# ComputationalRobotics/cuADMM

Measured on NVIDIA B200. Metric: ADMM iterations/s, higher is better.
Workload: dtype f64

## Files before the change

cuadmm_b200/csrc/common.cpp:

```cpp
#include "common.h"
#include <mutex>

namespace cuadmm {
static thread_local std::string g_last_error;
void set_last_error(const std::string& msg) { g_last_error = msg; }
}

extern "C" {
const char* cuadmm_last_error(void) { return cuadmm::g_last_error.c_str(); }
const char* cuadmm_version(void) { return "cuadmm_b200 0.1 (sm_100a)"; }
int cuadmm_device_count(void) {
    int n = 0;
    if (cudaGetDeviceCount(&n) != cudaSuccess) { cudaGetLastError(); return 0; }
    return n;
}
}
```

cuadmm_b200/csrc/common.h:

```cpp
#pragma once
#include <cuda_runtime.h>
#include <stdint.h>
#include <stdio.h>
#include <string>
#include <vector>
#include <memory>
#include <stdexcept>
#include "../../include/cuadmm_b200.h"

namespace cuadmm {

void set_last_error(const std::string& msg);

struct Error : public std::runtime_error {
    int code;
    Error(int c, const std::string& m) : std::runtime_error(m), code(c) {}
};

#define CUADMM_CUDA(call)                                                                   \
    do {                                                                                    \
        cudaError_t e__ = (call);                                                           \
        if (e__ != cudaSuccess) {                                                           \
            char buf__[512];                                                                \
            snprintf(buf__, sizeof buf__, "CUDA error %s at %s:%d: %s", cudaGetErrorName(e__), \
                     __FILE__, __LINE__, cudaGetErrorString(e__));                          \
            throw ::cuadmm::Error(e__ == cudaErrorMemoryAllocation ? CUADMM_ENOMEM :        \
                                  (e__ == cudaErrorNoDevice || e__ == cudaErrorInsufficientDriver) ? CUADMM_ENODEVICE : CUADMM_ECUDA, buf__); \
        }                                                                                   \
    } while (0)

#define CUADMM_REQUIRE(cond, msg)                                                           \
    do { if (!(cond)) throw ::cuadmm::Error(CUADMM_EINVAL, std::string("invalid argument: ") + (msg)); } while (0)

template <class F>
static inline int guarded(F&& f) {
    try { f(); return CUADMM_OK; }
    catch (const Error& e) { set_last_error(e.what()); return e.code; }
    catch (const std::bad_alloc&) { set_last_error("host out of memory"); return CUADMM_ENOMEM; }
    catch (const std::exception& e) { set_last_error(e.what()); return CUADMM_EINVAL; }
}

template <class T>
struct DevBuf {
    T* p = nullptr;
    int64_t n = 0;
    bool owned = true;
    DevBuf() {}
    explicit DevBuf(int64_t n_) { alloc(n_); }
    DevBuf(const DevBuf&) = delete;
    DevBuf& operator=(const DevBuf&) = delete;
    DevBuf(DevBuf&& o) noexcept : p(o.p), n(o.n), owned(o.owned) { o.p = nullptr; o.n = 0; }
    DevBuf& operator=(DevBuf&& o) noexcept { if (this != &o) { release(); p = o.p; n = o.n; owned = o.owned; o.p = nullptr; o.n = 0; } return *this; }
    ~DevBuf() { release(); }
    void release() { if (p && owned) cudaFree(p); p = nullptr; n = 0; owned = true; }
    void adopt(T* ptr, int64_t n_) { release(); p = ptr; n = n_; owned = false; }
    void alloc(int64_t n_) {
        release();
        n = n_;
        if (n_ > 0) CUADMM_CUDA(cudaMalloc((void**)&p, sizeof(T) * (size_t)n_));
    }
    void zero(cudaStream_t s = 0) { if (n) CUADMM_CUDA(cudaMemsetAsync(p, 0, sizeof(T) * (size_t)n, s)); }
    void upload(const T* h, int64_t cnt, cudaStream_t s = 0) {
        if (cnt) CUADMM_CUDA(cudaMemcpyAsync(p, h, sizeof(T) * (size_t)cnt, cudaMemcpyHostToDevice, s));
    }
    void upload(const std::vector<T>& h, cudaStream_t s = 0) {
        if ((int64_t)h.size() != n) alloc((int64_t)h.size());
        upload(h.data(), n, s);
    }
    void download(T* h, int64_t cnt, cudaStream_t s = 0) const {
        if (cnt) CUADMM_CUDA(cudaMemcpyAsync(h, p, sizeof(T) * (size_t)cnt, cudaMemcpyDeviceToHost, s));
    }
};

struct DeviceGuard {
    int prev = -1;
    explicit DeviceGuard(int dev) {
        if (dev >= 0) { cudaGetDevice(&prev); CUADMM_CUDA(cudaSetDevice(dev)); }
    }
    ~DeviceGuard() { if (prev >= 0) cudaSetDevice(prev); }
};

static inline int64_t tri(int64_t n) { return n * (n + 1) / 2; }

}
```

cuadmm_b200/csrc/debug_api.cpp:

```cpp
#include "chol_host.h"
#include "common.h"
#include <algorithm>
#include <cmath>

using namespace cuadmm;

extern "C" {

int cuadmm_debug_chol_solve(int64_t m, int64_t ncols, const int32_t* rowptr, const int32_t* colind, const double* val,
                            double eps, double n_lead_frac, const double* rhs, double* y, int32_t* perm_out,
                            int64_t* stats ) {
    return guarded([&] {
        SymCsc M = form_aat(m, ncols, rowptr, colind, val, eps);
        std::vector<int32_t> perm = min_degree_order(M);
        perm = postorder_perm(M, perm);
        CholFactor F; SymCsc C;
        chol_symbolic(M, perm, F, &C);
        const int64_t n_lead = std::max<int64_t>(0, std::min<int64_t>(m, (int64_t)(n_lead_frac * (double)m)));
        chol_numeric(C, F, n_lead);
        const int64_t r = m - n_lead;
        std::vector<double> S((size_t)(r * r), 0.0);
        for (int64_t j = n_lead; j < m; ++j)
            for (int64_t p = C.p[j]; p < C.p[j + 1]; ++p) S[(C.i[p] - n_lead) + (j - n_lead) * r] = C.x[p];
        for (int64_t j = 0; j < n_lead; ++j)
            for (int64_t p = F.Lp[j] + 1; p < F.Lp[j + 1]; ++p) if (F.Li[p] >= n_lead)
                for (int64_t q = p; q < F.Lp[j + 1]; ++q)
                    S[(F.Li[q] - n_lead) + (F.Li[p] - n_lead) * r] -= F.Lx[q] * F.Lx[p];
        for (int64_t k = 0; k < r; ++k) {
            double d = S[k + k * r];
            d = (d > 1e-11) ? std::sqrt(d) : INFINITY; S[k + k * r] = d;
            for (int64_t i = k + 1; i < r; ++i) S[i + k * r] /= d;
            for (int64_t j = k + 1; j < r; ++j)
                for (int64_t i = j; i < r; ++i) S[i + j * r] -= S[i + k * r] * S[j + k * r];
        }
        std::vector<double> z(m);
        for (int64_t k = 0; k < m; ++k) z[k] = rhs[F.perm[k]];
        for (int64_t j = 0; j < n_lead; ++j) {
            z[j] /= F.Lx[F.Lp[j]];
            for (int64_t p = F.Lp[j] + 1; p < F.Lp[j + 1]; ++p) z[F.Li[p]] -= F.Lx[p] * z[j];
        }
        for (int64_t j = 0; j < r; ++j) {
            z[n_lead + j] /= S[j + j * r];
            for (int64_t i = j + 1; i < r; ++i) z[n_lead + i] -= S[i + j * r] * z[n_lead + j];
        }
        for (int64_t j = r - 1; j >= 0; --j) {
            for (int64_t i = j + 1; i < r; ++i) z[n_lead + j] -= S[i + j * r] * z[n_lead + i];
            z[n_lead + j] /= S[j + j * r];
        }
        for (int64_t j = n_lead - 1; j >= 0; --j) {
            for (int64_t p = F.Lp[j] + 1; p < F.Lp[j + 1]; ++p) z[j] -= F.Lx[p] * z[F.Li[p]];
            z[j] /= F.Lx[F.Lp[j]];
        }
        for (int64_t k = 0; k < m; ++k) y[F.perm[k]] = z[k];
        if (perm_out) std::copy(F.perm.begin(), F.perm.end(), perm_out);
        if (stats) {
            stats[0] = M.p[m]; stats[1] = F.nnz(); stats[2] = F.n_deficient;
            std::vector<int32_t> lev(m, 0);
            int32_t depth = 0;
            for (int64_t j = 0; j < m; ++j) {
                for (int64_t p = F.Lp[j] + 1; p < F.Lp[j + 1]; ++p) lev[F.Li[p]] = std::max(lev[F.Li[p]], lev[j] + 1);
                depth = std::max(depth, lev[j] + 1);
            }
            stats[3] = depth;
            std::vector<int64_t> cnt(depth + 1, 0);
            for (int64_t j = 0; j < m; ++j) cnt[lev[j]]++;
            int64_t narrow = 0;
            for (int32_t l = 0; l < depth; ++l) if (cnt[l] < 8) narrow += cnt[l];
            stats[4] = narrow;
            std::vector<int64_t> sn = find_supernodes(F, 256);
            const int64_t nsn = (int64_t)sn.size() - 1;
            std::vector<int32_t> snof(m, 0), slev(std::max<int64_t>(nsn, 1), 0);
            for (int64_t s = 0; s < nsn; ++s) for (int64_t j = sn[s]; j < sn[s + 1]; ++j) snof[j] = (int32_t)s;
            int32_t sdepth = 0;
            for (int64_t s = 0; s < nsn; ++s) {
                for (int64_t j = sn[s]; j < sn[s + 1]; ++j)
                    for (int64_t p = F.Lp[j] + 1; p < F.Lp[j + 1]; ++p) {
                        const int32_t t = snof[F.Li[p]];
                        if (t != s) slev[t] = std::max(slev[t], slev[s] + 1);
                    }
                sdepth = std::max(sdepth, slev[s] + 1);
            }
            stats[5] = nsn; stats[6] = sdepth;
            std::vector<int64_t> scnt(sdepth + 1, 0);
            for (int64_t s = 0; s < nsn; ++s) scnt[slev[s]] += sn[s + 1] - sn[s];
            int64_t deep_rows = 0;
            for (int32_t l = 48; l < sdepth; ++l) deep_rows += scnt[l];
            stats[7] = deep_rows;
        }
    });
}

}
```

cuadmm_b200/csrc/plan.h:

```cpp
#pragma once
#include "common.h"
#include "blocks.h"
#include "project_jacobi.cuh"

namespace cuadmm { struct DensePart; }
cuadmm::DensePart* dense_part_create(int device, const std::vector<int32_t>& blk, const std::vector<int64_t>& svec_off,
                                     const std::vector<int64_t>& which);
void dense_part_destroy(cuadmm::DensePart* p);
int dense_part_project(cuadmm::DensePart* D, const double* Xb, double* Xproj, cudaStream_t st,
                       const cuadmm::ProjEpilogue* epi, const int* done_flag);

namespace cuadmm {
struct LinChunk {
    int64_t off;
    int32_t len;
    int32_t cone;
};
constexpr int kLinearChunk = 4096;
std::vector<LinChunk> linear_chunks(const BlockLayout& layout);
int linear_project(const LinChunk* d_chunks, int64_t nchunks, const double* Xb, double* Xproj, cudaStream_t st,
                   const ProjEpilogue* epi, const int* done_flag);
}

struct cuadmm_plan {
    int device = -1;
    cuadmm::BlockLayout layout;

    struct Class {
        int kind;
        int nmax;
        int32_t count;
        int64_t first;
        size_t smem;
        int grid;
    };
    std::vector<Class> classes;
    std::vector<cuadmm::BlkDesc> h_desc;
    cuadmm::DevBuf<cuadmm::BlkDesc> d_desc;
    cuadmm::DevBuf<double> d_scratch;
    cuadmm::DevBuf<double> d_eig;
    cuadmm::DevBuf<int32_t> d_sweeps;
    cuadmm::DevBuf<double> d_in, d_out;
    cuadmm::DevBuf<int64_t> d_svec_off, d_mat_off;
    cuadmm::DevBuf<int32_t> d_blk;
    cuadmm::DevBuf<uint8_t> d_pool;

    cuadmm::DevBuf<double> d_Q;
    bool warm_start = true;
    void reset_warm_start();
    double threshold = 1e-11;
    int max_sweeps = 40;
    bool force_global = false;
    std::unique_ptr<cuadmm_plan> eig_plan;
    int rank_limit = 0;
    cudaEvent_t ev0 = nullptr, ev1 = nullptr;
    std::vector<cudaStream_t> side_streams;
    std::vector<cudaEvent_t> side_events;
    cudaEvent_t fork_event = nullptr;
    cuadmm::DensePart* dense = nullptr;
    std::vector<cuadmm::LinChunk> h_lin;
    cuadmm::DevBuf<cuadmm::LinChunk> d_lin;
    cudaStream_t lin_stream = nullptr;
    cudaEvent_t lin_event = nullptr;
    int64_t eig_len = 0;
    const int* done_flag = nullptr;
    double last_ms = 0.0;
    int64_t last_launches = 0;

    ~cuadmm_plan();
    void build_device();
    int project(const double* d_Xb, double* d_Xproj, cudaStream_t stream,
                const cuadmm::ProjEpilogue* epi, bool want_eig);
};
```

cuadmm_b200/csrc/project.cu:

```cuda
#include "plan.h"
#include <algorithm>
#include <limits>
#include <type_traits>
#include <numeric>
#include <stdlib.h>

namespace cuadmm {

template <bool WARP>
__device__ __forceinline__ void mat_sync() {
    if (WARP) __syncwarp(); else __syncthreads();
}

template <int NT, bool WARP>
__device__ __forceinline__ double mat_sum(double v, double* red, int tid) {
#pragma unroll
    for (int o = 16; o > 0; o >>= 1) v += __shfl_xor_sync(0xffffffffu, v, o);
    if (WARP) return v;
    const int wid = tid >> 5;
    __syncthreads();
    if ((tid & 31) == 0) red[wid] = v;
    __syncthreads();
    double t = 0.0;
#pragma unroll 1
    for (int i = 0; i < NT / 32; ++i) t += red[i];
    return t;
}

template <int NT, bool WARP>
__device__ __forceinline__ double mat_max(double v, double* red, int tid) {
#pragma unroll
    for (int o = 16; o > 0; o >>= 1) v = fmax(v, __shfl_xor_sync(0xffffffffu, v, o));
    if (WARP) return v;
    const int wid = tid >> 5;
    __syncthreads();
    if ((tid & 31) == 0) red[wid] = v;
    __syncthreads();
    double t = 0.0;
#pragma unroll 1
    for (int i = 0; i < NT / 32; ++i) t = fmax(t, red[i]);
    return t;
}

__host__ __device__ __forceinline__ int jacobi_ld(int n, int L) {
    if (L >= 16) return n | 1;
    int ld = n;
    while ((ld & 15) != (L & 15)) ++ld;
    return ld;
}
__host__ __device__ __forceinline__ size_t jacobi_per_mat(int nmax, int L) {
    return (((size_t)jacobi_ld(nmax, L) * nmax + nmax + (nmax + 2) / 2 + 1 + 34) + 1) & ~(size_t)1;
}

__device__ __forceinline__ void jacobi_cs2(double alpha, double beta, double gamma, double& c, double& s,
                                           double& alpha_new, double& beta_new) {
    const double d = beta - alpha;
    const double g2 = gamma + gamma;
    const double rh = rsqrt(fma(d, d, g2 * g2));
    const double c2 = fabs(d) * rh;
    const double s2 = (d < 0.0 ? -g2 : g2) * rh;
    const double cc = fma(0.5, c2, 0.5);
    const double rc = rsqrt(cc);
    c = cc * rc;
    s = 0.5 * s2 * rc;
    const double ss = 1.0 - cc;
    const double x = s2 * gamma;
    alpha_new = fma(cc, alpha, fma(ss, beta, -x));
    beta_new = fma(ss, alpha, fma(cc, beta, x));
}

__device__ __forceinline__ void jacobi_dmma(double& c0, double& c1, double a, double b) {
    asm volatile("mma.sync.aligned.m8n8k4.row.col.f64.f64.f64.f64 {%0,%1}, {%2}, {%3}, {%0,%1};"
                 : "+d"(c0), "+d"(c1) : "d"(a), "d"(b));
}

template <int NT, bool WARP>
__device__ __forceinline__ bool jacobi_gram_converged(const double* G, const double* w, int n, int ld, double thr2, int tid) {
    const int lane = tid & 31;
    const int wid = WARP ? 0 : (tid >> 5);
    constexpr int NW = WARP ? 1 : NT / 32;
    const int nt = (n + 7) >> 3;
    const int kr = lane & 3, cq = lane >> 2;
    int flag = 0;
    for (int P = wid; P < nt; P += NW) {
        const int pcol = P * 8 + cq;
        const double* Gp = G + (size_t)min(pcol, n - 1) * ld;
        const bool pv = pcol < n;
        const int row = P * 8 + cq;
        const double wr = (row < n) ? w[row] : 0.0;
        for (int Q0 = P; Q0 < nt; Q0 += 4) {
            double c[4][2];
            const double* Gq[4];
            bool qv[4];
#pragma unroll
            for (int u = 0; u < 4; ++u) {
                const int qcol = (Q0 + u) * 8 + cq;
                qv[u] = (Q0 + u < nt) && qcol < n;
                Gq[u] = G + (size_t)min(qcol, n - 1) * ld;
                c[u][0] = 0.0; c[u][1] = 0.0;
            }
            for (int r0 = 0; r0 < n; r0 += 4) {
                const int r = r0 + kr;
                const bool rv = r < n;
                const double av = (pv && rv) ? Gp[r] : 0.0;
                double bv[4];
#pragma unroll
                for (int u = 0; u < 4; ++u) bv[u] = (qv[u] && rv) ? Gq[u][r] : 0.0;
#pragma unroll
                for (int u = 0; u < 4; ++u) jacobi_dmma(c[u][0], c[u][1], av, bv[u]);
            }
            if (row < n) {
#pragma unroll
                for (int u = 0; u < 4; ++u) {
                    const int col0 = (Q0 + u) * 8 + 2 * kr;
                    if (Q0 + u < nt) {
                        if (col0 < n && col0 != row) { const double g2 = c[u][0] * c[u][0]; if (g2 > thr2 * wr * w[col0] && g2 > 1e-30) flag = 1; }
                        if (col0 + 1 < n && col0 + 1 != row) { const double g2 = c[u][1] * c[u][1]; if (g2 > thr2 * wr * w[col0 + 1] && g2 > 1e-30) flag = 1; }
                    }
                }
            }
        }
    }
    const int any = WARP ? __any_sync(0xffffffffu, flag) : __syncthreads_or(flag);
    return !any;
}

constexpr int jacobi_min_ctas(int T) { return T <= 64 ? 8 : T <= 128 ? 4 : T <= 256 ? 2 : 1; }

template <int T, int L, int RPL, bool WARP>
__global__ void __launch_bounds__(T, jacobi_min_ctas(T)) proj_jacobi_kernel(ProjArgs a, int nmax) {
    extern __shared__ double smem[];
    constexpr int NT = WARP ? 32 : T;
    constexpr int NG = NT / L;
    constexpr int MPC = WARP ? T / 32 : 1;
    const int tid = WARP ? (threadIdx.x & 31) : threadIdx.x;
    const int mat_in_cta = WARP ? (threadIdx.x >> 5) : 0;
    const int bi = blockIdx.x * MPC + mat_in_cta;
    if (bi >= a.nblk) return;
    if (a.done_flag && *a.done_flag) return;

    const size_t per_mat = jacobi_per_mat(nmax, L);
    double* G = smem + per_mat * mat_in_cta;
    double* w = G + (size_t)jacobi_ld(nmax, L) * nmax;
    int* pos = (int*)(w + nmax);
    double* red = w + nmax + (nmax + 2) / 2 + 1;

    const BlkDesc d = a.desc[bi];
    const int n = d.n;
    const int ld = jacobi_ld(n, L);
    const int ntri = n * (n + 1) / 2;
    const double* __restrict__ xin = a.Xb + d.svec_off;
    double* __restrict__ xout = a.Xproj + d.svec_off;

    double amax = 0.0;
    for (int idx0 = tid; idx0 < ntri; idx0 += NT * 8) {
        double v[8];
#pragma unroll
        for (int u = 0; u < 8; ++u) { const int idx = idx0 + u * NT; v[u] = (idx < ntri) ? __ldg(xin + idx) : 0.0; }
#pragma unroll
        for (int u = 0; u < 8; ++u) {
            const int idx = idx0 + u * NT;
            if (idx < ntri) {
                int r, c;
                tri_unrank(idx, r, c);
                amax = fmax(amax, fabs(v[u]));
                const double v2 = (r == c) ? v[u] : v[u] * CUADMM_SQRT2INV;
                G[r + c * ld] = v2;
                G[c + r * ld] = v2;
            }
        }
    }
    amax = mat_max<NT, WARP>(amax, red, tid);
    int ex = 0;
    if (amax > 0.0 && amax < 1.7e308) frexp(amax, &ex);
    mat_sync<WARP>();
    double f2 = 0.0;
    const int e_dc = NT / n, e_dr = NT - e_dc * n;
    const int e_c0 = tid / n, e_r0 = tid - e_c0 * n;
    for (int c = e_c0, r = e_r0; c < n;) {
        const double v = ldexp(G[r + c * ld], -ex);
        G[r + c * ld] = v;
        f2 = fma(v, v, f2);
        r += e_dr; c += e_dc;
        if (r >= n) { r -= n; ++c; }
    }
    f2 = mat_sum<NT, WARP>(f2, red, tid);
    const double sp = sqrt(f2);
    if (!(sp > 0.0) || !(sp < 1.7e308)) {
        const double fill = (sp == 0.0) ? 0.0 : (sp - sp);
        for (int idx = tid; idx < ntri; idx += NT) {
            xout[idx] = fill;
            if (a.epi.X) {
                const int64_t gi = d.svec_off + idx;
                const double sig = *a.epi.sig_ptr;
                const double Sv = (fill - a.epi.X[gi]) / sig - a.epi.Rd1[gi];
                a.epi.S[gi] = Sv;
                a.epi.SmC[gi] = Sv - a.epi.Cd[gi];
            }
        }
        if (tid == 0 && a.sweeps_out) a.sweeps_out[d.index] = 0;
        if (a.eig_out) for (int j = tid; j < n; j += NT) a.eig_out[d.w_off + j] = fill;
        return;
    }
    const double inv_s = 1.0 / sp;
    for (int c = e_c0, r = e_r0; c < n;) {
        const double v = G[r + c * ld] * inv_s;
        G[r + c * ld] = (r == c) ? v + 1.0 : v;
        r += e_dr; c += e_dc;
        if (r >= n) { r -= n; ++c; }
    }
    mat_sync<WARP>();

    const int m = n + (n & 1);
    const int half = m >> 1;
    const int grp = tid / L, lane = tid % L;
    const unsigned gmask = (L == 32) ? 0xffffffffu : (((1u << L) - 1u) << ((tid & 31) / L * L));

    double* Qb = a.Q ? a.Q + d.q_off : nullptr;
    if (Qb) {
        constexpr int KF = (((L * RPL) > 168 ? 168 : (L * RPL)) + 3) / 4;
        constexpr int NWARP = WARP ? 1 : NT / 32;
        const int wid = WARP ? 0 : (tid >> 5);
        const int l32 = tid & 31;
        const int fr = l32 >> 2, fk = l32 & 3;
        const int nk = (n + 3) >> 2;
        for (int r0 = wid * 8; r0 < n; r0 += NWARP * 8) {
            const int row = r0 + fr;
            double af[KF];
#pragma unroll
            for (int kk = 0; kk < KF; ++kk) {
                const int k = kk * 4 + fk;
                af[kk] = (kk < nk && row < n && k < n) ? G[row + k * ld] : 0.0;
            }
            __syncwarp();
            for (int j0 = 0; j0 < n; j0 += 16) {
                constexpr int KC = KF < 16 ? KF : 16;
                const int col0 = j0 + fr, col1 = j0 + 8 + fr;
                const double* __restrict__ q0 = Qb + (size_t)min(col0, n - 1) * n;
                const double* __restrict__ q1 = Qb + (size_t)min(col1, n - 1) * n;
                double c00 = 0.0, c01 = 0.0, c10 = 0.0, c11 = 0.0;
#pragma unroll
                for (int kb = 0; kb < KF; kb += KC) {
                    if (kb < nk) {
                        double b0[KC], b1[KC];
#pragma unroll
                        for (int kk = 0; kk < KC; ++kk) {
                            const int k = (kb + kk) * 4 + fk;
                            const bool kv = kb + kk < nk && k < n;
                            b0[kk] = (kv && col0 < n) ? __ldg(q0 + k) : 0.0;
                            b1[kk] = (kv && col1 < n) ? __ldg(q1 + k) : 0.0;
                        }
#pragma unroll
                        for (int kk = 0; kk < KC; ++kk) {
                            if (kb + kk < KF && kb + kk < nk) {
                                jacobi_dmma(c00, c01, af[kb + kk], b0[kk]);
                                jacobi_dmma(c10, c11, af[kb + kk], b1[kk]);
                            }
                        }
                    }
                }
                if (row < n) {
                    const int cc = j0 + 2 * fk;
                    if (cc < n) G[row + cc * ld] = c00;
                    if (cc + 1 < n) G[row + (cc + 1) * ld] = c01;
                    if (cc + 8 < n) G[row + (cc + 8) * ld] = c10;
                    if (cc + 9 < n) G[row + (cc + 9) * ld] = c11;
                }
            }
        }
        mat_sync<WARP>();
    }

    const double thr2 = a.threshold * a.threshold;
    const double tiny2 = 1.2325951644078309e-32;
    int sweeps = 0;
    bool converged = false;
    while (true) {
        for (int j = grp; j < n; j += NG) {
            const double* Gj = G + j * ld;
            double al = 0.0;
            for (int r = lane; r < n; r += L) al = fma(Gj[r], Gj[r], al);
#pragma unroll
            for (int o = L / 2; o > 0; o >>= 1) al += __shfl_xor_sync(gmask, al, o);
            if (lane == 0) w[j] = al;
        }
        mat_sync<WARP>();
        if (jacobi_gram_converged<NT, WARP>(G, w, n, ld, thr2, tid)) { converged = true; break; }
        if (sweeps >= a.max_sweeps) break;
        auto run_steps = [&](auto nit_c) {
            constexpr int NIT = decltype(nit_c)::value;
// ... 303 lines not shown
    int nmax;
    int threads;
    int L;
    int mats_per_cta;
    void (*fn)(ProjArgs, int);
};

#define CUADMM_CLASS(NMAX, T, L, RPL, WARP) {NMAX, T, L, (WARP) ? (T) / 32 : 1, proj_jacobi_kernel<T, L, RPL, WARP>}
static const SizeClass kSizeClasses[] = {
    CUADMM_CLASS(16, 128, 4, 4, true),
    CUADMM_CLASS(32, 64, 4, 8, false),
    CUADMM_CLASS(64, 128, 4, 16, false),
    CUADMM_CLASS(96, 192, 4, 24, false),
    CUADMM_CLASS(128, 512, 8, 16, false),
    CUADMM_CLASS(168, 352, 8, 21, false),
};
static const int kNumSizeClasses = (int)(sizeof(kSizeClasses) / sizeof(kSizeClasses[0]));
static const int kGlobalKind = -1;

static size_t smem_bytes(int nmax, const SizeClass& sc) {
    return jacobi_per_mat(nmax, sc.L) * sizeof(double) * sc.mats_per_cta;
}

}

using namespace cuadmm;

cuadmm_plan::~cuadmm_plan() {
    if (device >= 0) {
        cudaSetDevice(device);
        if (ev0) cudaEventDestroy(ev0);
        if (ev1) cudaEventDestroy(ev1);
        if (fork_event) cudaEventDestroy(fork_event);
        if (lin_stream) cudaStreamDestroy(lin_stream);
        if (lin_event) cudaEventDestroy(lin_event);
        for (auto s : side_streams) cudaStreamDestroy(s);
        for (auto e : side_events) cudaEventDestroy(e);
        if (dense) dense_part_destroy(dense);
    }
}

void cuadmm_plan::build_device() {
    const int64_t nblk = (int64_t)layout.blk.size();
    std::vector<int64_t> w_off(nblk + 1, 0);
    for (int64_t k = 0; k < nblk; ++k) w_off[k + 1] = w_off[k] + (layout.types[k] == 's' ? layout.blk[k] : 0);
    eig_len = w_off[nblk];
    h_lin = linear_chunks(layout);

    std::vector<std::vector<int64_t>> members(kNumSizeClasses + 1);
    std::vector<int64_t> dense_blocks;
    for (int64_t k = 0; k < nblk; ++k) {
        if (layout.types[k] != 's') continue;
        const int n = layout.blk[k];
        int ci = kNumSizeClasses;
        for (int c = 0; c < kNumSizeClasses; ++c) if (n <= kSizeClasses[c].nmax) { ci = c; break; }
        if (ci == kNumSizeClasses && !force_global) { dense_blocks.push_back(k); continue; }
        members[ci].push_back(k);
    }
    if (dense) { dense_part_destroy(dense); dense = nullptr; }
    if (!dense_blocks.empty()) dense = dense_part_create(device, layout.blk, layout.svec_off, dense_blocks);
    h_desc.clear(); classes.clear();
    int64_t scratch = 0, q_total = 0;
    for (int ci = kNumSizeClasses; ci >= 0; --ci) {
        auto& mem = members[ci];
        if (mem.empty()) continue;
        std::stable_sort(mem.begin(), mem.end(), [&](int64_t a, int64_t b) { return layout.blk[a] > layout.blk[b]; });
        Class cl;
        cl.kind = (ci == kNumSizeClasses) ? kGlobalKind : ci;
        cl.nmax = layout.blk[mem[0]];
        cl.count = (int32_t)mem.size();
        cl.first = (int64_t)h_desc.size();
        if (cl.kind == kGlobalKind) {
            cl.smem = 0;
            cl.grid = cl.count;
        } else {
            const SizeClass& sc = kSizeClasses[cl.kind];
            cl.smem = smem_bytes(cl.nmax, sc);
            cl.grid = (cl.count + sc.mats_per_cta - 1) / sc.mats_per_cta;
        }
        for (int64_t k : mem) {
            BlkDesc d;
            d.svec_off = layout.svec_off[k];
            d.w_off = w_off[k];
            d.n = layout.blk[k];
            d.index = (int32_t)k;
            d.scratch_off = 0;
            d.q_off = 0;
            if (cl.kind != kGlobalKind) { d.q_off = q_total; q_total += (int64_t)d.n * d.n; }
            else { d.scratch_off = scratch; scratch += (int64_t)d.n * d.n; }
            h_desc.push_back(d);
        }
        classes.push_back(cl);
    }
    if (device < 0) return;

    DeviceGuard g(device);
    d_desc.upload(h_desc);
    if (!h_lin.empty()) {
        d_lin.upload(h_lin);
        CUADMM_CUDA(cudaStreamCreateWithFlags(&lin_stream, cudaStreamNonBlocking));
        CUADMM_CUDA(cudaEventCreateWithFlags(&lin_event, cudaEventDisableTiming));
    }
    if (scratch) d_scratch.alloc(scratch);
    d_eig.alloc(std::max<int64_t>(w_off[nblk], 1));
    d_sweeps.alloc(std::max<int64_t>(nblk, 1));
    warm_start = true;
    if (const char* e = getenv("CUADMM_JACOBI_WARM")) warm_start = atoi(e) != 0;
    if (const char* e = getenv("CUADMM_JACOBI_THR")) { const double v = atof(e); if (v > 0.0 && v < 1e-3) threshold = v; }
    if (warm_start && q_total > 0) {
        d_Q.alloc(q_total);
        reset_warm_start();
    }
    d_svec_off.upload(layout.svec_off);
    d_mat_off.upload(layout.mat_off);
    d_blk.upload(layout.blk);
    d_pool.upload(layout.pool);
    CUADMM_CUDA(cudaEventCreate(&ev0));
    CUADMM_CUDA(cudaEventCreate(&ev1));
    CUADMM_CUDA(cudaEventCreateWithFlags(&fork_event, cudaEventDisableTiming));
    for (size_t i = 0; i < classes.size(); ++i) {
        cudaStream_t s; cudaEvent_t e;
        CUADMM_CUDA(cudaStreamCreateWithFlags(&s, cudaStreamNonBlocking));
        CUADMM_CUDA(cudaEventCreateWithFlags(&e, cudaEventDisableTiming));
        side_streams.push_back(s); side_events.push_back(e);
    }
    for (const Class& cl : classes) {
        if (cl.kind == kGlobalKind) continue;
        const SizeClass& sc = kSizeClasses[cl.kind];
        CUADMM_CUDA(cudaFuncSetAttribute((const void*)sc.fn, cudaFuncAttributeMaxDynamicSharedMemorySize, (int)smem_bytes(sc.nmax, sc)));
    }
    CUADMM_CUDA(cudaDeviceSynchronize());
}

__global__ void init_basis_kernel(const BlkDesc* __restrict__ desc, int nblk, double* Q) {
    const int b = blockIdx.x;
    if (b >= nblk) return;
    const int n = desc[b].n;
    double* q = Q + desc[b].q_off;
    for (int e = threadIdx.x; e < n * n; e += blockDim.x) q[e] = (e / n == e % n) ? 1.0 : 0.0;
}

void cuadmm_plan::reset_warm_start() {
    if (d_Q.n == 0) return;
    DeviceGuard g(device);
    for (const Class& cl : classes) {
        if (cl.kind == kGlobalKind) continue;
        init_basis_kernel<<<cl.count, 256>>>(d_desc.p + cl.first, cl.count, d_Q.p);
    }
    CUADMM_CUDA(cudaGetLastError());
    CUADMM_CUDA(cudaDeviceSynchronize());
}

int cuadmm_plan::project(const double* d_Xb, double* d_Xproj, cudaStream_t stream,
                         const ProjEpilogue* epi, bool want_eig) {
    if (device < 0) throw Error(CUADMM_ENODEVICE, "plan was built without a CUDA device; there is no CPU fallback");
    int launches = 0;
    if (want_eig) {
        CUADMM_CUDA(cudaMemsetAsync(d_eig.p, 0xFF, sizeof(double) * (size_t)d_eig.n, stream));
        CUADMM_CUDA(cudaMemsetAsync(d_sweeps.p, 0, sizeof(int32_t) * (size_t)d_sweeps.n, stream));
    }
    const bool has_dense = dense != nullptr;
    const bool has_lin = !h_lin.empty();
    const bool lin_side = has_lin && (has_dense || !classes.empty());
    if (rank_limit > 0) {
        if (has_dense) throw Error(CUADMM_EINVAL, "fixed-rank projection is only available for blocks n <= 168 (the sign iteration of larger blocks has no eigenvalues to rank)");
    }
    if (classes.size() > 1 || (has_dense && !classes.empty()) || lin_side) CUADMM_CUDA(cudaEventRecord(fork_event, stream));
    for (size_t i = 0; i < classes.size(); ++i) {
        const Class& cl = classes[i];
        cudaStream_t st = stream;
        const bool side = has_dense || i > 0;
        if (side) {
            st = side_streams[i];
            CUADMM_CUDA(cudaStreamWaitEvent(st, fork_event, 0));
        }
        ProjArgs a;
        a.Xb = d_Xb; a.Xproj = d_Xproj;
        a.desc = d_desc.p + cl.first;
        a.nblk = cl.count;
        a.threshold = threshold;
        a.max_sweeps = max_sweeps;
        a.eig_out = want_eig ? d_eig.p : nullptr;
        a.sweeps_out = want_eig ? d_sweeps.p : nullptr;
        a.scratch = d_scratch.p;
        a.done_flag = done_flag;
        a.rank_limit = rank_limit;
        a.Q = (warm_start && cl.kind != kGlobalKind && d_Q.n > 0) ? d_Q.p : nullptr;
        if (epi) a.epi = *epi; else { a.epi.X = nullptr; a.epi.Rd1 = nullptr; a.epi.Cd = nullptr; a.epi.S = nullptr; a.epi.SmC = nullptr; a.epi.sig_ptr = nullptr; }
        if (cl.kind == kGlobalKind) {
            proj_jacobi_global_kernel<<<cl.grid, 1024, 0, st>>>(a);
        } else {
            kSizeClasses[cl.kind].fn<<<cl.grid, kSizeClasses[cl.kind].threads, cl.smem, st>>>(a, cl.nmax);
        }
        CUADMM_CUDA(cudaGetLastError());
        ++launches;
        if (side) CUADMM_CUDA(cudaEventRecord(side_events[i], st));
    }
    if (has_lin) {
        cudaStream_t st = stream;
        if (lin_side) {
            st = lin_stream;
            CUADMM_CUDA(cudaStreamWaitEvent(st, fork_event, 0));
        }
        launches += linear_project(d_lin.p, d_lin.n, d_Xb, d_Xproj, st, epi, done_flag);
        if (lin_side) CUADMM_CUDA(cudaEventRecord(lin_event, st));
    }
    if (has_dense) launches += dense_part_project(dense, d_Xb, d_Xproj, stream, epi, done_flag);
    for (size_t i = 0; i < classes.size(); ++i)
        if (has_dense || i > 0) CUADMM_CUDA(cudaStreamWaitEvent(stream, side_events[i], 0));
    if (lin_side) CUADMM_CUDA(cudaStreamWaitEvent(stream, lin_event, 0));
    return launches;
}

extern "C" {

int cuadmm_plan_create(const int32_t* blk, int64_t nblk, int device, cuadmm_plan** out) {
    return cuadmm_plan_create_typed(nullptr, blk, nblk, device, out);
}

int cuadmm_plan_create_typed(const char* types, const int32_t* blk, int64_t nblk, int device, cuadmm_plan** out) {
    return guarded([&] {
        CUADMM_REQUIRE(out != nullptr, "out is null");
        CUADMM_REQUIRE(blk != nullptr || nblk == 0, "blk is null");
        *out = nullptr;
        std::unique_ptr<cuadmm_plan> p(new cuadmm_plan());
        p->layout.init(blk, nblk, types);
        if (device >= 0) {
            int cnt = 0;
            cudaError_t e = cudaGetDeviceCount(&cnt);
            if (e != cudaSuccess || cnt == 0) {
                cudaGetLastError();
                throw Error(CUADMM_ENODEVICE, "no CUDA device available (pass device=-1 for a host-only plan; compute has no CPU fallback)");
            }
            CUADMM_REQUIRE(device < cnt, "device index out of range");
        }
        p->device = device;
        p->build_device();
        *out = p.release();
    });
}

void cuadmm_plan_destroy(cuadmm_plan* plan) { delete plan; }
int64_t cuadmm_plan_vec_len(const cuadmm_plan* plan) { return plan ? plan->layout.vec_len : -1; }
int64_t cuadmm_plan_nblk(const cuadmm_plan* plan) { return plan ? (int64_t)plan->layout.blk.size() : -1; }
int64_t cuadmm_plan_num_sizes(const cuadmm_plan* plan) { return plan ? (int64_t)plan->layout.sizes.size() : -1; }

int cuadmm_plan_sizes(const cuadmm_plan* plan, int32_t* sizes, int32_t* nums, int32_t* is_large) {
    return guarded([&] {
        CUADMM_REQUIRE(plan, "plan is null");
        plan->layout.require_all_psd("cuadmm_plan_sizes");
        for (size_t i = 0; i < plan->layout.sizes.size(); ++i) {
            if (sizes) sizes[i] = plan->layout.sizes[i];
            if (nums) nums[i] = plan->layout.nums[i];
            if (is_large) is_large[i] = plan->layout.large[i];
        }
    });
}

int cuadmm_plan_totals(const cuadmm_plan* plan, int64_t out[6]) {
    return guarded([&] {
        CUADMM_REQUIRE(plan && out, "null argument");
        const BlockLayout& l = plan->layout;
        l.require_all_psd("cuadmm_plan_totals");
        out[0] = l.large_mat_num; out[1] = l.sum_large_mat_size; out[2] = l.total_large_mat_size;
        out[3] = l.small_mat_num; out[4] = l.sum_small_mat_size; out[5] = l.total_small_mat_size;
    });
}

int64_t cuadmm_plan_start_indices(const cuadmm_plan* plan, int which, int64_t* out) {
    if (!plan) return -1;
    const BlockLayout& l = plan->layout;
    if (!l.all_psd()) return guarded([&] { l.require_all_psd("cuadmm_plan_start_indices"); });
    const std::vector<int64_t>* v = nullptr;
    switch (which) {
        case 0: v = &l.large_mat_start; break;
        case 1: v = &l.large_W_start; break;
        case 2: v = &l.small_mat_start; break;
        case 3: v = &l.small_W_start; break;
        default: return -1;
    }
    if (out) std::copy(v->begin(), v->end(), out);
    return (int64_t)v->size();
}

int cuadmm_plan_maps(const cuadmm_plan* plan, int32_t* map_B, int32_t* map_M1, int32_t* map_M2) {
    return guarded([&] {
        CUADMM_REQUIRE(plan && map_B && map_M1 && map_M2, "null argument");
        plan->layout.maps(map_B, map_M1, map_M2);
    });
}

int cuadmm_plan_partition(const cuadmm_plan* plan, int nparts, int32_t* owner, double* part_cost) {
    return guarded([&] {
        CUADMM_REQUIRE(plan && owner, "null argument");
        plan->layout.partition(nparts, owner, part_cost);
    });
}

int cuadmm_plan_set_rank_limit(cuadmm_plan* plan, int eig_rank) {
    return guarded([&] {
        CUADMM_REQUIRE(plan, "plan is null");
        CUADMM_REQUIRE(eig_rank >= 0, "eig_rank < 0");
        plan->rank_limit = eig_rank;
    });
}

int cuadmm_eig_rank_mask(int32_t* mask, int64_t batch_size, int64_t mat_size, int64_t eig_rank) {
    return guarded([&] {
        CUADMM_REQUIRE(mask || batch_size * mat_size == 0, "mask is null");
        CUADMM_REQUIRE(batch_size >= 0 && mat_size >= 0 && eig_rank >= 0 && eig_rank <= mat_size, "bad sizes");
        for (int64_t i = 0; i < batch_size * mat_size; ++i) mask[i] = 0;
        for (int64_t i = 0; i < batch_size; ++i)
            for (int64_t j = 0; j < eig_rank; ++j) mask[i * mat_size + (mat_size - 1 - j)] = 1;
    });
}

int cuadmm_plan_set_warm_start(cuadmm_plan* plan, int enable) {
    return guarded([&] {
        CUADMM_REQUIRE(plan, "plan is null");
        if (plan->device < 0) return;
        plan->reset_warm_start();
        plan->warm_start = enable != 0 && plan->d_Q.n > 0;
    });
}

int cuadmm_plan_set_jacobi(cuadmm_plan* plan, double threshold, int max_sweeps) {
    return guarded([&] {
        CUADMM_REQUIRE(plan, "plan is null");
        CUADMM_REQUIRE(threshold > 0 && max_sweeps > 0, "threshold and max_sweeps must be positive");
        plan->threshold = threshold;
        plan->max_sweeps = max_sweeps;
    });
}

double cuadmm_plan_last_ms(const cuadmm_plan* plan) { return plan ? plan->last_ms : -1.0; }
int64_t cuadmm_plan_last_launches(const cuadmm_plan* plan) { return plan ? plan->last_launches : -1; }

int cuadmm_project_psd(cuadmm_plan* plan, const double* d_Xb, double* d_Xproj, void* stream) {
    return guarded([&] {
        CUADMM_REQUIRE(plan && d_Xb && d_Xproj, "null argument");
        DeviceGuard g(plan->device);
        plan->last_launches = plan->project(d_Xb, d_Xproj, (cudaStream_t)stream, nullptr, false);
    });
}

int cuadmm_project_epilogue(cuadmm_plan* plan, const double* d_Xb, double* d_Xproj, const double* d_X, const double* d_Rd1,
                            const double* d_C, double* d_S, double* d_SmC, const double* d_sig, void* stream) {
    return guarded([&] {
        CUADMM_REQUIRE(plan && d_Xb && d_Xproj && d_X && d_Rd1 && d_C && d_S && d_SmC && d_sig, "null argument");
        DeviceGuard g(plan->device);
        ProjEpilogue pe;
        pe.X = d_X; pe.Rd1 = d_Rd1; pe.Cd = d_C; pe.S = d_S; pe.SmC = d_SmC; pe.sig_ptr = d_sig;
        plan->last_launches = plan->project(d_Xb, d_Xproj, (cudaStream_t)stream, &pe, false);
    });
}

static void project_host_impl(cuadmm_plan* plan, const double* h_Xb, double* h_Xproj,
                              double* h_eig, int32_t* h_sweeps) {
    CUADMM_REQUIRE(plan && h_Xb && h_Xproj, "null argument");
    if (plan->device < 0) throw Error(CUADMM_ENODEVICE, "plan was built without a CUDA device; there is no CPU fallback");
    DeviceGuard g(plan->device);
    const int64_t L = plan->layout.vec_len;
    if (plan->d_in.n != L) { plan->d_in.alloc(L); plan->d_out.alloc(L); }
// ... 105 lines not shown
```

cuadmm_b200/csrc/solver.cu:

```cuda
#include "solver.h"
#include <algorithm>
#include <chrono>
#include <cmath>
#include <string>
#include <string.h>
#include <stdlib.h>

namespace cuadmm {

void spmv_set_done_flag(cuadmm_spmv_s& A, const int* flag);

static constexpr int kEwThreads = 256;
static constexpr int64_t kHistRing = 4096;

__global__ void __launch_bounds__(kEwThreads) x_update_kernel(int64_t n, const double* __restrict__ Rd1,
        const double* __restrict__ S, const double* __restrict__ Cd, double* Rd, double* X,
        const DevState* st, double* partial) {
    if (st->done) return;
    __shared__ double red[2][kEwThreads / 32];
    const double ts = st->tau * st->sig;
    double a0 = 0.0, a1 = 0.0;
    for (int64_t i = (int64_t)blockIdx.x * kEwThreads + threadIdx.x; i < n; i += (int64_t)gridDim.x * kEwThreads) {
        const double rd = Rd1[i] + S[i];
        Rd[i] = rd;
        const double xn = X[i] + ts * rd;
        X[i] = xn;
        a0 = fma(rd, rd, a0);
        a1 = fma(Cd[i], xn, a1);
    }
#pragma unroll
    for (int o = 16; o > 0; o >>= 1) { a0 += __shfl_xor_sync(0xffffffffu, a0, o); a1 += __shfl_xor_sync(0xffffffffu, a1, o); }
    if ((threadIdx.x & 31) == 0) { red[0][threadIdx.x >> 5] = a0; red[1][threadIdx.x >> 5] = a1; }
    __syncthreads();
    if (threadIdx.x == 0) {
        double s0 = 0.0, s1 = 0.0;
        for (int k = 0; k < kEwThreads / 32; ++k) { s0 += red[0][k]; s1 += red[1][k]; }
        partial[2 * blockIdx.x] = s0; partial[2 * blockIdx.x + 1] = s1;
    }
}

__global__ void __launch_bounds__(256) scalar_update_kernel(DevState* st, const double* __restrict__ part_rd, int n_rd,
        const double* __restrict__ part_rp, int n_rp, double* hist, int64_t hist_cap) {
    if (st->done) return;
    __shared__ double sm[4][256];
    double v[4] = {0.0, 0.0, 0.0, 0.0};
    for (int i = threadIdx.x; i < n_rd; i += 256) { v[0] += part_rd[2 * i]; v[1] += part_rd[2 * i + 1]; }
    for (int i = threadIdx.x; i < n_rp; i += 256) { v[2] += part_rp[2 * i]; v[3] += part_rp[2 * i + 1]; }
    for (int q = 0; q < 4; ++q) sm[q][threadIdx.x] = v[q];
    __syncthreads();
    for (int o = 128; o > 0; o >>= 1) {
        if (threadIdx.x < o) for (int q = 0; q < 4; ++q) sm[q][threadIdx.x] += sm[q][threadIdx.x + o];
        __syncthreads();
    }
    if (threadIdx.x != 0) return;
    const double sumRd = sm[0][0], sumCX = sm[1][0], sumRp = sm[2][0], sumby = sm[3][0];
    const int iter = st->iter;
    const double errRp = st->bscale * sqrt(sumRp) / st->norm_borg;
    const double pobj = sumCX * st->objscale;
    const double errRd = st->Cscale * sqrt(sumRd) / st->norm_Corg;
    const double dobj = sumby * st->objscale;
    const double maxfeas = fmax(errRp, errRd);
    const double relgap = fabs(pobj - dobj) / (1 + fabs(pobj) + fabs(dobj));
    const double feasratio = st->ratioconst * errRp / errRd;
    if (feasratio < 1) st->prim_win += 1; else st->dual_win += 1;
    double sig = st->sig;
    if (((iter <= st->sig_update_threshold) && ((iter % st->sig_update_stage_1) == 1)) ||
        ((iter > st->sig_update_threshold) && ((iter % st->sig_update_stage_2) == 1))) {
        if (st->prim_win > 1.2 * st->dual_win) {
            st->prim_win = 0;
            sig = fmin(st->sigmax, sig * st->sigscale);
        } else if (st->dual_win > 1.2 * st->prim_win) {
            st->dual_win = 0;
            sig = fmax(st->sigmin, sig / st->sigscale);
        }
    }
    st->sig = sig;
    st->errRp = errRp; st->errRd = errRd; st->pobj = pobj; st->dobj = dobj;
    st->maxfeas = maxfeas; st->relgap = relgap; st->feasratio = feasratio;
    {
        const int64_t k = (int64_t)(iter - 1) % hist_cap;
        hist[0 * hist_cap + k] = pobj;  hist[1 * hist_cap + k] = dobj;
        hist[2 * hist_cap + k] = errRp; hist[3 * hist_cap + k] = errRd;
        hist[4 * hist_cap + k] = relgap; hist[5 * hist_cap + k] = sig;
        hist[6 * hist_cap + k] = st->bscale; hist[7 * hist_cap + k] = st->Cscale;
    }
    const int next = iter + 1;
    st->iter = next;
    double tau = (next < st->switch_admm) ? 1.95 : 1.618;
    if (errRd < st->stop_tol) tau = fmax(1.618, tau / 1.1);
    st->tau = tau;
    if (fmax(maxfeas, relgap) < st->stop_tol) { st->done = 1; st->stop_reason = 1; }
    if (next > st->max_iter) { st->done = 1; st->stop_reason = 2; }
}

__global__ void switch_kernel(DevState* st) {
    if (st->done) return;
    st->sig_update_stage_2 = st->sig_update_stage_2 / 2;
    st->sigscale = st->sigscale * 1.23;
    st->sgs_KKT = fmax(st->maxfeas, st->relgap);
    st->best_KKT = st->sgs_KKT;
}

__global__ void best_decide_kernel(DevState* st) {
    if (st->done) { st->pad_ = 0; return; }
    const double cur = fmax(st->maxfeas, st->relgap);
    if (st->best_KKT > cur) { st->best_KKT = cur; st->pad_ = 1; } else st->pad_ = 0;
}
__global__ void best_copy_kernel(const DevState* st, int64_t n, const double* __restrict__ src, double* dst) {
    if (!st->pad_) return;
    for (int64_t i = (int64_t)blockIdx.x * blockDim.x + threadIdx.x; i < n; i += (int64_t)gridDim.x * blockDim.x) dst[i] = src[i];
}

__global__ void scale_kernel(int64_t n, double* x, double s) {
    for (int64_t i = (int64_t)blockIdx.x * blockDim.x + threadIdx.x; i < n; i += (int64_t)gridDim.x * blockDim.x) x[i] *= s;
}
__global__ void scale_vec_kernel(int64_t n, double* y, const double* __restrict__ d, double s, int divide) {
    for (int64_t i = (int64_t)blockIdx.x * blockDim.x + threadIdx.x; i < n; i += (int64_t)gridDim.x * blockDim.x)
        y[i] = divide ? y[i] / d[i] * s : y[i] * d[i] * s;
}
__global__ void sub_kernel(int64_t n, const double* __restrict__ a, const double* __restrict__ b, double* out) {
    for (int64_t i = (int64_t)blockIdx.x * blockDim.x + threadIdx.x; i < n; i += (int64_t)gridDim.x * blockDim.x) out[i] = a[i] - b[i];
}

__global__ void rhsy_kernel(int64_t m, const double* __restrict__ Rp, const double* __restrict__ buf, double* rhsy, const DevState* st) {
    if (st->done) return;
    const double sig = st->sig;
    for (int64_t i = (int64_t)blockIdx.x * blockDim.x + threadIdx.x; i < m; i += (int64_t)gridDim.x * blockDim.x) rhsy[i] = Rp[i] / sig + buf[i];
}
__global__ void __launch_bounds__(256) fold_partials_kernel(const double* __restrict__ part, int n, double* out2, const DevState* st) {
    if (st->done) return;
    __shared__ double sm[2][256];
    double a = 0.0, b = 0.0;
    for (int i = threadIdx.x; i < n; i += 256) { a += part[2 * i]; b += part[2 * i + 1]; }
    sm[0][threadIdx.x] = a; sm[1][threadIdx.x] = b;
    __syncthreads();
    for (int o = 128; o > 0; o >>= 1) {
        if (threadIdx.x < o) { sm[0][threadIdx.x] += sm[0][threadIdx.x + o]; sm[1][threadIdx.x] += sm[1][threadIdx.x + o]; }
        __syncthreads();
    }
    if (threadIdx.x == 0) { out2[0] = sm[0][0]; out2[1] = sm[1][0]; }
}
__global__ void __launch_bounds__(kEwThreads) rp_kernel(int64_t m, const double* __restrict__ b, const double* __restrict__ buf,
        const double* __restrict__ normA, const double* __restrict__ y, double* Rp, const DevState* st, double* partial) {
    if (st->done) return;
    __shared__ double red[2][kEwThreads / 32];
    double a0 = 0.0, a1 = 0.0;
    for (int64_t i = (int64_t)blockIdx.x * kEwThreads + threadIdx.x; i < m; i += (int64_t)gridDim.x * kEwThreads) {
        const double rp = b[i] - buf[i];
        Rp[i] = rp;
        const double t = normA[i] * rp;
        a0 = fma(t, t, a0);
        a1 = fma(b[i], y[i], a1);
    }
#pragma unroll
    for (int o = 16; o > 0; o >>= 1) { a0 += __shfl_xor_sync(0xffffffffu, a0, o); a1 += __shfl_xor_sync(0xffffffffu, a1, o); }
    if ((threadIdx.x & 31) == 0) { red[0][threadIdx.x >> 5] = a0; red[1][threadIdx.x >> 5] = a1; }
    __syncthreads();
    if (threadIdx.x == 0) {
        double s0 = 0.0, s1 = 0.0;
        for (int k = 0; k < kEwThreads / 32; ++k) { s0 += red[0][k]; s1 += red[1][k]; }
        partial[2 * blockIdx.x] = s0; partial[2 * blockIdx.x + 1] = s1;
    }
}
__global__ void scatter_full_kernel(int64_t nloc, const double* __restrict__ local, const int64_t* __restrict__ loc2glob, double* full) {
    for (int64_t i = (int64_t)blockIdx.x * blockDim.x + threadIdx.x; i < nloc; i += (int64_t)gridDim.x * blockDim.x) full[loc2glob[i]] = local[i];
}

static int ew_grid(int64_t n, int device) {
    int sms = 148;
    cudaDeviceGetAttribute(&sms, cudaDevAttrMultiProcessorCount, device);
    return (int)std::max<int64_t>(1, std::min<int64_t>((n + kEwThreads - 1) / kEwThreads, (int64_t)sms * 8));
}

static double host_norm2(const std::vector<double>& v) {
    double scale = 0.0, ssq = 1.0;
    for (double x : v) {
        if (x != 0.0) {
            const double a = std::fabs(x);
            if (scale < a) { ssq = 1.0 + ssq * (scale / a) * (scale / a); scale = a; }
            else ssq += (a / scale) * (a / scale);
        }
    }
    return scale * std::sqrt(ssq);
}

}

using namespace cuadmm;

cuadmm_solver::~cuadmm_solver() {
    cudaSetDevice(device);
    delete A; delete At; delete ys;
    if (h_st) cudaFreeHost(h_st);
    if (ev_start) cudaEventDestroy(ev_start);
    if (ev_now) cudaEventDestroy(ev_now);
    for (auto e : prof_ev) cudaEventDestroy(e);
    if (graph_sgs) cudaGraphExecDestroy(graph_sgs);
    if (graph_admm) cudaGraphExecDestroy(graph_admm);
    if (stream) cudaStreamDestroy(stream);
}

void cuadmm_solver::init(int , int , int64_t vec_len_, int64_t con_num_,
                         const int32_t* At_col_ptrs, const int32_t* At_row_ids, const double* At_vals, int64_t At_nnz,
                         const int32_t* b_idx, const double* b_val, int64_t b_nnz,
                         const int32_t* C_idx, const double* C_val, int64_t C_nnz,
                         const int32_t* blk, int64_t mat_num, const double* X0, const double* y0, const double* S0, double sig) {
    CUADMM_REQUIRE(!initialised, "solver already initialised (one instance per problem, like SDPSolver)");
    CUADMM_REQUIRE(vec_len_ >= 0 && con_num_ >= 0 && At_nnz >= 0, "negative dimension");
    CUADMM_REQUIRE(At_col_ptrs && blk, "null argument");
    CUADMM_REQUIRE(At_col_ptrs[0] == 0 && At_col_ptrs[con_num_] == At_nnz, "At_csc_col_ptrs does not span At_nnz");
    int cnt = 0;
    if (cudaGetDeviceCount(&cnt) != cudaSuccess || cnt == 0) {
        cudaGetLastError();
        throw Error(CUADMM_ENODEVICE, "no CUDA device available; the solver has no CPU fallback");
    }
    if (!device_set) {
        if (const char* e = getenv("CUADMM_DEVICE")) device = atoi(e);
        else { int cur = 0; if (cudaGetDevice(&cur) == cudaSuccess) device = cur; else cudaGetLastError(); }
    }
    if (const char* e = getenv("CUADMM_NO_GRAPH")) use_graphs = atoi(e) == 0;
    CUADMM_REQUIRE(device >= 0 && device < cnt, "device index out of range");
    CUADMM_CUDA(cudaSetDevice(device));
    vec_len = vec_len_; con_num = con_num_;
    CUADMM_CUDA(cudaStreamCreateWithFlags(&stream, cudaStreamNonBlocking));
    CUADMM_CUDA(cudaEventCreate(&ev_start));
    CUADMM_CUDA(cudaEventCreate(&ev_now));
    CUADMM_CUDA(cudaEventRecord(ev_start, stream));
    const auto t0 = std::chrono::steady_clock::now();

    {
        CUADMM_REQUIRE(blk_types.empty() || (int64_t)blk_types.size() == mat_num, "block types were set for a different block count");
        BlockLayout full_layout;
        full_layout.init(blk, mat_num, blk_types.empty() ? nullptr : blk_types.data());
        CUADMM_REQUIRE(full_layout.vec_len == vec_len, "vec_len does not match the block sizes");
        shard.build(full_layout, world, rank);
        nloc = shard.vec_len_local;
        plan.reset(new cuadmm_plan());
        plan->layout.init(shard.local_blk.data(), (int64_t)shard.local_blk.size(), shard.local_types.data());
        plan->device = device;
        plan->build_device();
        if (world > 1) {
            d_loc2glob.upload(shard.loc2glob);
            if (const char* c = getenv("CUADMM_COMM")) use_peer = strcmp(c, "nccl") != 0;
        }
    }
    std::vector<double> vals(At_vals, At_vals + At_nnz);
    h_normA.assign(con_num, 1.0);
    for (int64_t p = 0; p < At_nnz; ++p) CUADMM_REQUIRE(At_row_ids[p] >= 0 && At_row_ids[p] < vec_len, "At row index out of range");
    for (int64_t i = 0; i < con_num; ++i) {
        double norm = 0.0;
        for (int p = At_col_ptrs[i]; p < At_col_ptrs[i + 1]; ++p) norm += vals[p] * vals[p];
        norm = std::max(1.0, std::sqrt(norm));
        h_normA[i] = norm;
        for (int p = At_col_ptrs[i]; p < At_col_ptrs[i + 1]; ++p) vals[p] /= norm;
    }
    {
        std::vector<int32_t> l_cp, l_ri; std::vector<double> l_v;
        const int32_t* cp = At_col_ptrs; const int32_t* ri = At_row_ids; const double* vv = vals.data();
        int64_t l_nnz = At_nnz;
        if (world > 1) {
            shard.slice_csc(con_num, At_col_ptrs, At_row_ids, vals.data(), l_cp, l_ri, l_v);
            l_ri.push_back(0); l_v.push_back(0.0);
            cp = l_cp.data(); ri = l_ri.data(); vv = l_v.data(); l_nnz = l_cp[con_num];
        }
        A = spmv_create(con_num, nloc, l_nnz, cp, ri, vv, device);
        std::vector<int32_t> t_rp(nloc + 1), t_ci(std::max<int64_t>(l_nnz, 1));
        std::vector<double> t_v(std::max<int64_t>(l_nnz, 1));
        if (cuadmm_csc_to_csr_host(nloc, con_num, l_nnz, cp, ri, vv, t_rp.data(), t_ci.data(), t_v.data()) != 0)
            throw Error(CUADMM_EINVAL, cuadmm_last_error());
        At = spmv_create(nloc, con_num, l_nnz, t_rp.data(), t_ci.data(), t_v.data(), device);
    }
    ys = ysolve_create(con_num, vec_len, At_nnz, At_col_ptrs, At_row_ids, vals.data(), 1e-15, device);
    if (world > 1) {
        if (use_peer) {
            CUADMM_REQUIRE(con_num < (int64_t)0xffffffffll, "sharded solver: con_num exceeds 32 bits");
            slice = (((con_num + world - 1) / world) + 1) & ~(int64_t)1;
            const int64_t mm = std::max<int64_t>(con_num, 1);
            const size_t need = sizeof(double) * (size_t)(world * slice + 4 * mm + std::max<int64_t>(ys->n_tail, 1) + std::max<int64_t>(vec_len, 1)) + 16 * 256;
            peer.reset(new PeerComm());
            peer->init(rank, world, nccl_id, device, need);
            const size_t o_stage = peer->alloc(sizeof(double) * world * slice);
            const size_t o_asmc = peer->alloc(sizeof(double) * mm), o_Rp = peer->alloc(sizeof(double) * mm), o_y = peer->alloc(sizeof(double) * mm);
            const size_t o_x = peer->alloc(sizeof(double) * mm), o_tmp = peer->alloc(sizeof(double) * std::max<int64_t>(ys->n_tail, 1));
            const size_t o_full = peer->alloc(sizeof(double) * std::max<int64_t>(vec_len, 1));
            stage = peer->local<double>(o_stage);
            p_stage = peer->ptrs(o_stage); p_asmc = peer->ptrs(o_asmc); p_Rp = peer->ptrs(o_Rp); p_full = peer->ptrs(o_full);
            asmc.adopt(peer->local<double>(o_asmc), mm); Rp.adopt(peer->local<double>(o_Rp), mm); y.adopt(peer->local<double>(o_y), mm);
            full_buf.adopt(peer->local<double>(o_full), std::max<int64_t>(vec_len, 1));
            ys->enable_peer(peer.get(), o_tmp, o_x);
            cta_part.alloc(2 * (int64_t)peer_reduce_grid(*peer, slice) + 2);
        } else {
            comm.reset(new NcclComm());
            comm->init(rank, world, nccl_id, device);
            red_buf.alloc(con_num + 2);
            asmc_part.alloc(std::max<int64_t>(con_num, 1));
            asmc_part.zero(stream);
        }
    }

    std::vector<double> hb(con_num, 0.0), hC(vec_len, 0.0), hX(vec_len, 0.0), hy(con_num, 0.0), hS(vec_len, 0.0);
    for (int64_t k = 0; k < b_nnz; ++k) { CUADMM_REQUIRE(b_idx[k] >= 0 && b_idx[k] < con_num, "b index out of range"); hb[b_idx[k]] = b_val[k]; }
    for (int64_t k = 0; k < C_nnz; ++k) { CUADMM_REQUIRE(C_idx[k] >= 0 && C_idx[k] < vec_len, "C index out of range"); hC[C_idx[k]] = C_val[k]; }
    if (X0) std::copy(X0, X0 + vec_len, hX.begin());
    if (y0) std::copy(y0, y0 + con_num, hy.begin());
    if (S0) std::copy(S0, S0 + vec_len, hS.begin());
    norm_borg = 1 + host_norm2(hb);
    norm_Corg = 1 + host_norm2(hC);
    for (int64_t i = 0; i < con_num; ++i) { hb[i] /= h_normA[i]; hy[i] *= h_normA[i]; }
    bscale = 1 + host_norm2(hb);
    Cscale = 1 + host_norm2(hC);
    objscale = bscale * Cscale;
    for (auto& v : hb) v /= bscale;
    for (auto& v : hC) v /= Cscale;
    for (auto& v : hX) v /= bscale;
    for (auto& v : hS) v /= Cscale;
    for (auto& v : hy) v /= Cscale;

    std::vector<double> hRp(con_num), hSmC(vec_len), hRd(vec_len, 0.0);
    for (int64_t i = 0; i < con_num; ++i) {
        double acc = 0.0;
        for (int p = At_col_ptrs[i]; p < At_col_ptrs[i + 1]; ++p) acc += vals[p] * hX[At_row_ids[p]];
        hRp[i] = hb[i] - acc;
    }
    for (int64_t i = 0; i < con_num; ++i)
        for (int p = At_col_ptrs[i]; p < At_col_ptrs[i + 1]; ++p) hRd[At_row_ids[p]] += vals[p] * hy[i];
    double sRp = 0, sRd = 0, cx = 0, by = 0;
    {
        std::vector<double> tmp(con_num);
        for (int64_t i = 0; i < con_num; ++i) tmp[i] = h_normA[i] * hRp[i] * bscale;
        sRp = host_norm2(tmp);
        for (int64_t i = 0; i < vec_len; ++i) { hSmC[i] = hS[i] - hC[i]; hRd[i] = (hRd[i] + hSmC[i]) * Cscale; cx += hC[i] * hX[i]; }
        sRd = host_norm2(hRd);
        for (int64_t i = 0; i < con_num; ++i) by += hb[i] * hy[i];
    }

    auto up = [&](DevBuf<double>& d, const std::vector<double>& h) {
        if (d.owned || !d.p) d.alloc(std::max<int64_t>((int64_t)h.size(), 1));
        d.upload(h.data(), (int64_t)h.size(), stream);
    };
    if (world > 1) {
        std::vector<double> t;
        shard.slice_vec(hX.data(), t); hX.swap(t);
        shard.slice_vec(hS.data(), t); hS.swap(t);
        shard.slice_vec(hSmC.data(), t); hSmC.swap(t);
        shard.slice_vec(hC.data(), t); hC.swap(t);
    }
    up(X, hX); up(S, hS); up(y, hy); up(Rp, hRp); up(SmC, hSmC); up(Cd, hC); up(bd, hb); up(normA, h_normA);
    Rd1.alloc(std::max<int64_t>(nloc, 1)); Rd.alloc(std::max<int64_t>(nloc, 1)); Xb.alloc(std::max<int64_t>(nloc, 1));
    Xproj.alloc(std::max<int64_t>(nloc, 1)); rhsy.alloc(std::max<int64_t>(con_num, 1)); if (asmc.owned || !asmc.p) asmc.alloc(std::max<int64_t>(con_num, 1)); asmc_valid = false;
    Rd1.zero(stream); Rd.zero(stream);
    nA_blocks = spmv_grid(*A); nAt_blocks = spmv_grid(*At); nE_blocks = ew_grid(std::max(nloc, con_num), device);
    partial.alloc(2 * (int64_t)(std::max(nAt_blocks, nE_blocks) + std::max(nA_blocks, nE_blocks)) + 4);
    partial.zero(stream);

    st.alloc(1);
    CUADMM_CUDA(cudaMallocHost((void**)&h_st, sizeof(DevState)));
    memset(h_st, 0, sizeof(DevState));
    h_st->sig = sig; h_st->tau = 1.95;
    h_st->errRp = sRp / norm_borg; h_st->errRd = sRd / norm_Corg;
    h_st->maxfeas = std::max(h_st->errRp, h_st->errRd);
    h_st->pobj = cx * objscale; h_st->dobj = by * objscale;
    h_st->relgap = std::fabs(h_st->pobj - h_st->dobj) / (1 + std::fabs(h_st->pobj) + std::fabs(h_st->dobj));
    h_st->bscale = bscale; h_st->Cscale = Cscale; h_st->objscale = objscale;
    h_st->norm_borg = norm_borg; h_st->norm_Corg = norm_Corg;
    h_st->sigmax = 1e3; h_st->sigmin = 1e-3; h_st->ratioconst = 1e0;
    h_st->prim_win = 0; h_st->dual_win = 0;
    CUADMM_CUDA(cudaMemcpyAsync(st.p, h_st, sizeof(DevState), cudaMemcpyHostToDevice, stream));

    const int* done_ptr = &st.p->done;
    spmv_set_done_flag(*A, done_ptr);
    spmv_set_done_flag(*At, done_ptr);
    ys->done_flag = done_ptr;
    plan->done_flag = done_ptr;
    CUADMM_CUDA(cudaStreamSynchronize(stream));
    init_time = std::chrono::duration<double>(std::chrono::steady_clock::now() - t0).count();
    initialised = true;
}

void cuadmm_solver::enqueue_iteration(int iter, int switch_admm, bool prof) {
    const double* scal = &st.p->sig;
    SpmvEpilogue e;
    auto mark = [&](int k) {
        if (!prof) return;
        cudaEvent_t ev;
        CUADMM_CUDA(cudaEventCreate(&ev));
        CUADMM_CUDA(cudaEventRecord(ev, stream));
        prof_ev.push_back(ev);
        prof_tag.push_back(k);
    };
    ys->prof_ev = prof ? &prof_ev : nullptr;
    ys->prof_tag = prof ? &prof_tag : nullptr;
    const int gm_ = ew_grid(con_num, device);
    auto k1 = [&](bool cached) {
        if (!cached) {
            if (world == 1) { e = SpmvEpilogue(); spmv_launch(*A, -1.0, SmC.p, 0.0, asmc.p, e, stream); ++launches; }
            else reduce_partial_A(false, SmC.p, -1.0, nullptr, 0, nullptr);
        }
        rhsy_kernel<<<gm_, 256, 0, stream>>>(con_num, Rp.p, asmc.p, rhsy.p, st.p); ++launches;
    };
    k1(asmc_valid);
    mark(0);
    ys->solve(rhsy.p, y.p, stream); launches += ys->launches_per_solve;
    mark(1);
    e = SpmvEpilogue(); e.mode = 2; e.aux1 = Cd.p; e.aux2 = X.p; e.out2 = Xb.p; e.scal = scal;
    spmv_launch(*At, 1.0, y.p, 0.0, Rd1.p, e, stream); ++launches;
    ProjEpilogue pe;
    pe.X = X.p; pe.Rd1 = Rd1.p; pe.Cd = Cd.p; pe.S = S.p; pe.SmC = SmC.p; pe.sig_ptr = scal;
    mark(2);
    launches += plan->project(Xb.p, Xproj.p, stream, &pe, false);
    mark(3);
    if (iter == switch_admm) {
        switch_kernel<<<1, 1, 0, stream>>>(st.p); ++launches;
        CUADMM_CUDA(cudaMemcpyAsync(X_best.p, X.p, sizeof(double) * nloc, cudaMemcpyDeviceToDevice, stream));
        CUADMM_CUDA(cudaMemcpyAsync(y_best.p, y.p, sizeof(double) * con_num, cudaMemcpyDeviceToDevice, stream));
        CUADMM_CUDA(cudaMemcpyAsync(S_best.p, S.p, sizeof(double) * nloc, cudaMemcpyDeviceToDevice, stream));
    }
    double* part_rd = partial.p;
    double* part_rp = partial.p + 2 * (int64_t)std::max(nAt_blocks, nE_blocks);
    int n_rd = 0;
    if (iter < switch_admm) {
        mark(6);
        k1(false);
        mark(7);
        mark(4);
        ys->solve(rhsy.p, y.p, stream); launches += ys->launches_per_solve;
        mark(5);
        e = SpmvEpilogue(); e.mode = 3; e.aux1 = Cd.p; e.aux2 = S.p; e.out2 = X.p; e.scal = scal; e.partial = part_rd;
        spmv_launch(*At, 1.0, y.p, 0.0, Rd.p, e, stream); ++launches;
        n_rd = nAt_blocks;
    } else {
        if (iter > switch_admm) {
            const int g = ew_grid(nloc, device);
            best_decide_kernel<<<1, 1, 0, stream>>>(st.p);
            best_copy_kernel<<<g, 256, 0, stream>>>(st.p, nloc, X.p, X_best.p);
            best_copy_kernel<<<g, 256, 0, stream>>>(st.p, con_num, y.p, y_best.p);
            best_copy_kernel<<<g, 256, 0, stream>>>(st.p, nloc, S.p, S_best.p);
            launches += 4;
        }
        mark(4); mark(5);
        x_update_kernel<<<nE_blocks, kEwThreads, 0, stream>>>(nloc, Rd1.p, S.p, Cd.p, Rd.p, X.p, st.p, part_rd); ++launches;
        n_rd = nE_blocks;
    }
    mark(8);
    if (world == 1) {
        e = SpmvEpilogue(); e.mode = 4; e.aux1 = bd.p; e.aux2 = normA.p; e.aux3 = y.p; e.partial = part_rp;
        spmv_launch(*A, 1.0, X.p, 0.0, Rp.p, e, stream); ++launches;
        scalar_update_kernel<<<1, 256, 0, stream>>>(st.p, part_rd, n_rd, part_rp, nA_blocks, hist.p, hist_cap); ++launches;
    } else {
        reduce_partial_A(true, X.p, 1.0, part_rd, n_rd, part_rp);
        if (use_peer)
            scalar_update_kernel<<<1, 256, 0, stream>>>(st.p, peer->local<double>(peer->off_scal_rd), world,
                                                        peer->local<double>(peer->off_scal_rp), world, hist.p, hist_cap);
        else
            scalar_update_kernel<<<1, 256, 0, stream>>>(st.p, red_buf.p + con_num, 1, part_rp, nE_blocks, hist.p, hist_cap);
        ++launches;
    }
    mark(9);
    ys->prof_ev = nullptr; ys->prof_tag = nullptr;
    asmc_valid = iter < switch_admm;
    CUADMM_CUDA(cudaGetLastError());
}

void cuadmm_solver::launch_iteration(int iter, int switch_admm, bool prof) {
    const bool sgs = iter < switch_admm;
    if (prof || !use_graphs || iter == switch_admm || sgs != asmc_valid) { enqueue_iteration(iter, switch_admm, prof); return; }
    cudaGraphExec_t& exec = sgs ? graph_sgs : graph_admm;
    int64_t& nl = sgs ? graph_launches_sgs : graph_launches_admm;
    if (!exec) {
        const int64_t before = launches;
        cudaGraph_t graph = nullptr;
        CUADMM_CUDA(cudaStreamBeginCapture(stream, cudaStreamCaptureModeThreadLocal));
        try {
            enqueue_iteration(iter, switch_admm, false);
        } catch (...) {
            cudaStreamEndCapture(stream, &graph);
            if (graph) cudaGraphDestroy(graph);
            throw;
        }
        CUADMM_CUDA(cudaStreamEndCapture(stream, &graph));
        CUADMM_CUDA(cudaGraphInstantiate(&exec, graph, 0));
        CUADMM_CUDA(cudaGraphDestroy(graph));
        nl = launches - before;
        launches = before;
    }
    CUADMM_CUDA(cudaGraphLaunch(exec, stream));
    launches += nl;
    asmc_valid = sgs;
}

void cuadmm_solver::reduce_partial_A(bool for_rp, const double* x_local, double alpha, const double* part_rd, int n_rd, double* part_rp) {
    SpmvEpilogue e;
    if (use_peer) {
        e.mode = 5; e.slice = (unsigned)slice; e.rank = rank;
        for (int q = 0; q < world; ++q) e.push[q] = p_stage.p[q];
        spmv_launch(*A, alpha, x_local, 0.0, stage, e, stream);
        peer_reduce_launch(*peer, for_rp ? 1 : 0, con_num, slice, stage, for_rp ? p_Rp : p_asmc, bd.p, normA.p, y.p, part_rd, n_rd,
                           cta_part.p, &st.p->done, stream);
        launches += 2;
        return;
    }
    if (!for_rp) {
        spmv_launch(*A, alpha, x_local, 0.0, asmc_part.p, e, stream);
        comm->allreduce_sum(asmc_part.p, asmc.p, con_num, stream);
        launches += 2;
        return;
    }
    spmv_launch(*A, alpha, x_local, 0.0, red_buf.p, e, stream);
    if (part_rd) fold_partials_kernel<<<1, 256, 0, stream>>>(part_rd, n_rd, red_buf.p + con_num, st.p);
    comm->allreduce_sum(red_buf.p, red_buf.p, con_num + 2, stream);
    rp_kernel<<<nE_blocks, kEwThreads, 0, stream>>>(con_num, bd.p, red_buf.p, normA.p, y.p, Rp.p, st.p, part_rp);
    launches += 4;
}

void cuadmm_solver::enqueue_half_step() {
    SpmvEpilogue e;
    if (!asmc_valid) {
        if (world == 1) { spmv_launch(*A, -1.0, SmC.p, 0.0, asmc.p, e, stream); ++launches; }
        else reduce_partial_A(false, SmC.p, -1.0, nullptr, 0, nullptr);
    }
    rhsy_kernel<<<ew_grid(con_num, device), 256, 0, stream>>>(con_num, Rp.p, asmc.p, rhsy.p, st.p); ++launches;
    ys->solve(rhsy.p, y.p, stream); launches += ys->launches_per_solve;
}

void cuadmm_solver::run_iterations(int n_iters, bool sgs, bool profile_, double out_ms[8]) {
    CUADMM_REQUIRE(initialised && hist.n > 0, "run_iterations() needs init() and one solve() first");
    CUADMM_CUDA(cudaSetDevice(device));
    CUADMM_CUDA(cudaMemcpyAsync(h_st, st.p, sizeof(DevState), cudaMemcpyDeviceToHost, stream));
    CUADMM_CUDA(cudaStreamSynchronize(stream));
    const int first = h_st->iter;
    h_st->done = 0; h_st->stop_tol = -1.0; h_st->max_iter = 0x7fffffff;
    const int sw = sgs ? 0x7fffffff : 0;
    h_st->switch_admm = sw;
    h_st->tau = sgs ? 1.95 : 1.618;
    CUADMM_CUDA(cudaMemcpyAsync(st.p, h_st, sizeof(DevState), cudaMemcpyHostToDevice, stream));
    if (!sgs && X_best.n < std::max<int64_t>(nloc, 1)) {
        X_best.alloc(std::max<int64_t>(nloc, 1)); y_best.alloc(std::max<int64_t>(con_num, 1)); S_best.alloc(std::max<int64_t>(nloc, 1));
        if (graph_admm) { cudaGraphExecDestroy(graph_admm); graph_admm = nullptr; }
    }
    for (auto e : prof_ev) cudaEventDestroy(e);
    prof_ev.clear(); prof_tag.clear();
    cudaEvent_t e0, e1;
    CUADMM_CUDA(cudaEventCreate(&e0)); CUADMM_CUDA(cudaEventCreate(&e1));
    CUADMM_CUDA(cudaEventRecord(e0, stream));
    for (int k = 0; k < n_iters; ++k) launch_iteration(first + k, sw, profile_);
    CUADMM_CUDA(cudaEventRecord(e1, stream));
    CUADMM_CUDA(cudaStreamSynchronize(stream));
    float ms = 0.f;
    cudaEventElapsedTime(&ms, e0, e1);
    out_ms[0] = ms;
    for (int k = 1; k < 8; ++k) out_ms[k] = 0.0;
    if (profile_) {
        auto span = [&](int a, int b) {
            double tot = 0.0;
            for (size_t i = 0; i < prof_ev.size(); ++i) {
                if (prof_tag[i] != a) continue;
                for (size_t j = i + 1; j < prof_ev.size(); ++j)
                    if (prof_tag[j] == b) { float t = 0.f; cudaEventElapsedTime(&t, prof_ev[i], prof_ev[j]); tot += t; break; }
            }
            return tot;
        };
        out_ms[1] = span(2, 3);
        out_ms[2] = span(0, 1) + (sgs ? span(4, 5) : 0.0);
        out_ms[3] = out_ms[0] - out_ms[1] - out_ms[2];
        out_ms[4] = span(6, 7);
        out_ms[5] = span(8, 9);
        out_ms[6] = span(20, 21);
        for (auto e : prof_ev) cudaEventDestroy(e);
        prof_ev.clear(); prof_tag.clear();
    }
    cudaEventDestroy(e0); cudaEventDestroy(e1);
    h_st->done = 1;
    CUADMM_CUDA(cudaMemcpyAsync(&st.p->done, &h_st->done, sizeof(int), cudaMemcpyHostToDevice, stream));
    CUADMM_CUDA(cudaStreamSynchronize(stream));
    if (peer) peer->check(stream);
}

void cuadmm_solver::gather_full(const DevBuf<double>& local, double* h_full) {
    CUADMM_REQUIRE(initialised && h_full, "solver not initialised");
    CUADMM_CUDA(cudaSetDevice(device));
    if (use_peer) {
        peer_scatter_full_launch(*peer, nloc, local.p, d_loc2glob.p, p_full, stream);
        full_buf.download(h_full, vec_len, stream);
        peer->check(stream);
        return;
    }
    if (full_buf.n < vec_len) full_buf.alloc(std::max<int64_t>(vec_len, 1));
    full_buf.zero(stream);
    scatter_full_kernel<<<ew_grid(nloc, device), 256, 0, stream>>>(nloc, local.p, d_loc2glob.p, full_buf.p);
    comm->allreduce_sum(full_buf.p, full_buf.p, vec_len, stream);
    full_buf.download(h_full, vec_len, stream);
    CUADMM_CUDA(cudaStreamSynchronize(stream));
}

static bool is_log_iter(int iter) { return (iter <= 200 && iter % 50 == 1) || (iter > 200 && iter % 100 == 1); }

void cuadmm_solver::solve(int max_iter, double stop_tol, int sig_update_threshold, int sig_update_stage_1,
                          int sig_update_stage_2, int switch_admm, double sigscale, bool if_first) {
    CUADMM_REQUIRE(initialised, "solve() before init()");
    CUADMM_REQUIRE(max_iter >= 0, "max_iter < 0");
    CUADMM_REQUIRE(sig_update_stage_1 >= 1 && sig_update_stage_2 >= 1, "sig_update_stage must be >= 1");
    CUADMM_CUDA(cudaSetDevice(device));
    const auto t0 = std::chrono::steady_clock::now();
    const int64_t n = nloc, m = con_num;
    const int gv = ew_grid(n, device), gm = ew_grid(m, device);
    if (X_best.n < std::max<int64_t>(n, 1)) {
        X_best.alloc(std::max<int64_t>(n, 1)); y_best.alloc(std::max<int64_t>(m, 1)); S_best.alloc(std::max<int64_t>(n, 1));
    }
    if (hist.n == 0) {
        hist_cap = kHistRing;
        hist.alloc(8 * hist_cap);
        if (graph_sgs) { cudaGraphExecDestroy(graph_sgs); graph_sgs = nullptr; }
        if (graph_admm) { cudaGraphExecDestroy(graph_admm); graph_admm = nullptr; }
    }
    info_iter_num = 0;
    for (auto& v : h_hist) v.clear();
    int64_t drained = 0;
    auto drain = [&](int64_t upto) {
        if (upto <= drained) return;
        CUADMM_REQUIRE(upto - drained <= hist_cap, "internal: history ring overrun");
        const int64_t n0 = upto - drained;
        for (int q = 0; q < 8; ++q) {
            const size_t base = h_hist[q].size();
            h_hist[q].resize(base + (size_t)n0);
            int64_t done_ = 0;
            while (done_ < n0) {
                const int64_t k = (drained + done_) % hist_cap;
                const int64_t len = std::min(n0 - done_, hist_cap - k);
                CUADMM_CUDA(cudaMemcpyAsync(h_hist[q].data() + base + done_, hist.p + q * hist_cap + k, sizeof(double) * len,
                                            cudaMemcpyDeviceToHost, stream));
                done_ += len;
            }
        }
        CUADMM_CUDA(cudaStreamSynchronize(stream));
// ... 298 lines not shown
```

cuadmm_b200/csrc/solver.h:

```cpp
#pragma once
#include "common.h"
#include "plan.h"
#include "spmv.h"
#include "ysolve.h"
#include "problem.h"
#include "shard.h"
#include "dist.h"
#include "peer.h"
#include "peer_kernels.h"

namespace cuadmm {

struct DevState {
    double sig, tau;
    double errRp, errRd, pobj, dobj, relgap, maxfeas, feasratio;
    double bscale, Cscale, objscale, norm_borg, norm_Corg;
    double sigmax, sigmin, sigscale, stop_tol, ratioconst;
    double best_KKT, sgs_KKT;
    int prim_win, dual_win;
    int iter;
    int done;
    int max_iter, sig_update_threshold, sig_update_stage_1, sig_update_stage_2, switch_admm;
    int stop_reason;
    int pad_;
};

}

struct cuadmm_solver {
    int device = 0;
    bool verbose = false;
    bool initialised = false;
    int64_t vec_len = 0, con_num = 0;
    int64_t nloc = 0;
    int rank = 0, world = 1;
    char nccl_id[128] = {0};
    cuadmm::Shard shard;
    std::vector<char> blk_types;
    bool use_peer = true;
    bool device_set = false;
    std::unique_ptr<cuadmm::PeerComm> peer;
    int64_t slice = 0;
    double* stage = nullptr;
    cuadmm::PeerPtrs p_stage, p_asmc, p_Rp, p_full;
    cuadmm::DevBuf<double> cta_part;
    std::unique_ptr<cuadmm::NcclComm> comm;
    cuadmm::DevBuf<double> red_buf;
    cuadmm::DevBuf<double> asmc_part;
    cuadmm::DevBuf<int64_t> d_loc2glob;
    cuadmm::DevBuf<double> full_buf;
    void gather_full(const cuadmm::DevBuf<double>& local, double* h_full);
    void reduce_partial_A(bool for_rp, const double* x_local, double alpha, const double* part_rd, int n_rd, double* part_rp);
    std::unique_ptr<cuadmm_plan> plan;
    cuadmm_spmv_s* A = nullptr;
    cuadmm_spmv_s* At = nullptr;
    cuadmm_ysolve_s* ys = nullptr;
    cuadmm::DevBuf<double> X, S, y, Rp, SmC, Rd1, Rd, Xb, Xproj, rhsy, Cd, bd, normA;
    cuadmm::DevBuf<double> X_best, y_best, S_best;
    cuadmm::DevBuf<double> partial;
    cuadmm::DevBuf<double> hist;
    int64_t hist_cap = 0;
    cuadmm::DevBuf<cuadmm::DevState> st;
    cuadmm::DevState* h_st = nullptr;
    cudaStream_t stream = nullptr;
    cudaEvent_t ev_start = nullptr, ev_now = nullptr;
    double bscale = 1, Cscale = 1, objscale = 1, norm_borg = 1, norm_Corg = 1;
    std::vector<double> h_normA;
    int64_t info_iter_num = 0;
    std::vector<double> h_hist[8];
    double total_time = 0, init_time = 0, solve_time = 0, proj_time = 0, ysolve_time = 0, spmv_time = 0;
    int64_t launches = 0;
    int nA_blocks = 0, nAt_blocks = 0, nE_blocks = 0;
    bool profile = false;
    std::vector<cudaEvent_t> prof_ev;
    std::vector<int> prof_tag;

    ~cuadmm_solver();
    void init(int eig_stream_num_per_gpu, int cpu_eig_thread_num, int64_t vec_len, int64_t con_num,
              const int32_t* At_col_ptrs, const int32_t* At_row_ids, const double* At_vals, int64_t At_nnz,
              const int32_t* b_idx, const double* b_val, int64_t b_nnz,
              const int32_t* C_idx, const double* C_val, int64_t C_nnz,
              const int32_t* blk, int64_t mat_num, const double* X0, const double* y0, const double* S0, double sig);
    void solve(int max_iter, double stop_tol, int sig_update_threshold, int sig_update_stage_1,
               int sig_update_stage_2, int switch_admm, double sigscale, bool if_first);
    void enqueue_iteration(int iter, int switch_admm, bool prof = false);
    void run_iterations(int n_iters, bool sgs, bool profile, double out_ms[8]);
    void enqueue_half_step();
    cudaGraphExec_t graph_sgs = nullptr, graph_admm = nullptr;
    int64_t graph_launches_sgs = 0, graph_launches_admm = 0;
    bool use_graphs = true;
    cuadmm::DevBuf<double> asmc;
    bool asmc_valid = false;
    void launch_iteration(int iter, int switch_admm, bool prof);
};
```

cuadmm_b200/csrc/spmv.cu:

```cuda
#include "spmv.h"
#include <algorithm>
#include <cstdlib>

namespace cuadmm {

static constexpr int kLongRow = 256;
static constexpr int kThreads = 256;

struct SpmvPre { double a1, a2, a3; };
template <int MODE>
__device__ __forceinline__ SpmvPre spmv_prefetch(const SpmvEpilogue& e, double beta, const double* y, int64_t i) {
    SpmvPre p = {0.0, 0.0, 0.0};
    switch (MODE) {
        case 0: if (beta != 0.0) p.a1 = y[i]; break;
        case 1: p.a1 = e.aux1[i]; break;
        case 2: p.a1 = e.aux1[i]; p.a2 = e.aux2[i]; break;
        case 3: p.a1 = e.aux1[i]; p.a2 = e.aux2[i]; p.a3 = e.out2[i]; break;
        case 4: p.a1 = e.aux1[i]; p.a2 = e.aux2[i]; p.a3 = e.aux3[i]; break;
        default: break;
    }
    return p;
}

template <int MODE>
__device__ __forceinline__ void spmv_store(const SpmvEpilogue& e, double alpha, double beta, double* y,
                                           int64_t i, double r, const SpmvPre& pre, double& acc0, double& acc1) {
    switch (MODE) {
        case 0:
            y[i] = (beta == 0.0) ? alpha * r : alpha * r + beta * pre.a1;
            break;
        case 1: {
            const double sig = e.scal[0];
            y[i] = pre.a1 / sig - r;
            break;
        }
        case 2: {
            const double sig = e.scal[0];
            const double rd1 = r - pre.a1;
            y[i] = rd1;
            e.out2[i] = pre.a2 + sig * rd1;
            break;
        }
        case 3: {
            const double sig = e.scal[0], tau = e.scal[1];
            const double c = pre.a1;
            const double rd = (r - c) + pre.a2;
            y[i] = rd;
            const double xn = pre.a3 + (tau * sig) * rd;
            e.out2[i] = xn;
            acc0 = fma(rd, rd, acc0);
            acc1 = fma(c, xn, acc1);
            break;
        }
        case 4: {
            const double b = pre.a1;
            const double rp = b - r;
            y[i] = rp;
            const double t = pre.a2 * rp;
            acc0 = fma(t, t, acc0);
            acc1 = fma(b, pre.a3, acc1);
            break;
        }
        case 5: {
            const unsigned q = (unsigned)i / e.slice;
            e.push[q][(size_t)e.rank * e.slice + ((unsigned)i - q * e.slice)] = alpha * r;
            break;
        }
    }
}

#ifndef CUADMM_SPMV_MINB
#define CUADMM_SPMV_MINB 5
#endif
template <int G, int MODE>
__global__ void __launch_bounds__(kThreads, CUADMM_SPMV_MINB) spmv_csr_kernel(
        int64_t rows, const int32_t* __restrict__ rowptr, const int32_t* __restrict__ colind,
        const double* __restrict__ val, const double* __restrict__ x, double* y, double alpha, double beta,
        SpmvEpilogue e, const int32_t* __restrict__ long_rows, int n_long, int main_blocks, int long_thr,
        const int* __restrict__ done_flag) {
    if (done_flag && *done_flag) return;
    __shared__ double red[2][kThreads / 32];
    double acc0 = 0.0, acc1 = 0.0;
    const int lane = threadIdx.x & 31;
    if ((int)blockIdx.x < main_blocks) {
        const int sub = threadIdx.x % G;
        const int64_t gid = ((int64_t)blockIdx.x * kThreads + threadIdx.x) / G;
        const int64_t ngroups = (int64_t)main_blocks * kThreads / G;
        const unsigned gmask = (G == 32) ? 0xffffffffu : (((1u << G) - 1u) << (lane / G * G));
        constexpr int U = (G == 1) ? 2 : 4;
        constexpr bool PRE = (G == 1);
        for (int64_t i0 = gid; i0 < rows; i0 += ngroups * U) {
            int p0[U], p1[U];
            bool mine[U];
            double r[U];
            SpmvPre pre[U];
#pragma unroll
            for (int u = 0; u < U; ++u) {
                const int64_t i = i0 + (int64_t)u * ngroups;
                p0[u] = 0; p1[u] = 0;
                pre[u] = SpmvPre{0.0, 0.0, 0.0};
                if (i < rows) {
                    p0[u] = rowptr[i]; p1[u] = rowptr[i + 1];
                    if (PRE && sub == 0) pre[u] = spmv_prefetch<MODE>(e, beta, y, i);
                }
            }
#pragma unroll
            for (int u = 0; u < U; ++u) {
                const int64_t i = i0 + (int64_t)u * ngroups;
                mine[u] = i < rows && p1[u] - p0[u] <= long_thr;
                if (!mine[u]) p1[u] = p0[u];
            }
#pragma unroll
            for (int u = 0; u < U; ++u) {
                const int p = p0[u] + sub;
                r[u] = 0.0;
                if (p < p1[u]) r[u] = fma(val[p], x[colind[p]], 0.0);
            }
#pragma unroll
            for (int u = 0; u < U; ++u)
                for (int p = p0[u] + sub + G; p < p1[u]; p += G) r[u] = fma(val[p], x[colind[p]], r[u]);
#pragma unroll
            for (int u = 0; u < U; ++u) {
#pragma unroll
                for (int o = G / 2; o > 0; o >>= 1) r[u] += __shfl_xor_sync(gmask, r[u], o);
            }
#pragma unroll
            for (int u = 0; u < U; ++u) {
                const int64_t i = i0 + (int64_t)u * ngroups;
                if (sub == 0 && mine[u]) {
                    if (!PRE) pre[u] = spmv_prefetch<MODE>(e, beta, y, i);
                    spmv_store<MODE>(e, alpha, beta, y, i, r[u], pre[u], acc0, acc1);
                }
            }
        }
    } else {
        const int w = ((int)blockIdx.x - main_blocks) * (kThreads / 32) + (threadIdx.x >> 5);
        const int nw = ((int)gridDim.x - main_blocks) * (kThreads / 32);
        for (int li = w; li < n_long; li += nw) {
            const int64_t i = long_rows[li];
            const int p0 = rowptr[i], p1 = rowptr[i + 1];
            SpmvPre pre = {0.0, 0.0, 0.0};
            if (lane == 0) pre = spmv_prefetch<MODE>(e, beta, y, i);
            double r = 0.0;
            for (int p = p0 + lane; p < p1; p += 32) r = fma(val[p], x[colind[p]], r);
#pragma unroll
            for (int o = 16; o > 0; o >>= 1) r += __shfl_xor_sync(0xffffffffu, r, o);
            if (lane == 0) spmv_store<MODE>(e, alpha, beta, y, i, r, pre, acc0, acc1);
        }
    }
    if ((MODE == 3 || MODE == 4) && e.partial) {
#pragma unroll
        for (int o = 16; o > 0; o >>= 1) {
            acc0 += __shfl_xor_sync(0xffffffffu, acc0, o);
            acc1 += __shfl_xor_sync(0xffffffffu, acc1, o);
        }
        if (lane == 0) { red[0][threadIdx.x >> 5] = acc0; red[1][threadIdx.x >> 5] = acc1; }
        __syncthreads();
        if (threadIdx.x == 0) {
            double s0 = 0.0, s1 = 0.0;
            for (int k = 0; k < kThreads / 32; ++k) { s0 += red[0][k]; s1 += red[1][k]; }
            e.partial[2 * blockIdx.x] = s0;
            e.partial[2 * blockIdx.x + 1] = s1;
        }
    }
}

struct SpmvAux {
    DevBuf<int32_t> long_rows;
    int n_long = 0;
    int long_thr = kLongRow;
    int main_blocks = 0, long_blocks = 0;
};

}

using namespace cuadmm;

struct cuadmm_spmv_full : cuadmm_spmv_s {
    SpmvAux aux;
    const int* done_flag = nullptr;
};

namespace cuadmm {

int spmv_grid(const cuadmm_spmv_s& A_) {
    const cuadmm_spmv_full& A = static_cast<const cuadmm_spmv_full&>(A_);
    return A.aux.main_blocks + A.aux.long_blocks;
}

void spmv_set_done_flag(cuadmm_spmv_s& A_, const int* flag) {
    static_cast<cuadmm_spmv_full&>(A_).done_flag = flag;
}

void spmv_launch(const cuadmm_spmv_s& A_, double alpha, const double* x, double beta, double* y,
                 const SpmvEpilogue& epi, cudaStream_t stream, int* grid_out) {
    const cuadmm_spmv_full& A = static_cast<const cuadmm_spmv_full&>(A_);
    const int grid = A.aux.main_blocks + A.aux.long_blocks;
    if (grid_out) *grid_out = grid;
    if (A.rows == 0 || grid == 0) return;
#define CUADMM_SPMV_LAUNCH(G, MODE)                                                                     \
    spmv_csr_kernel<G, MODE><<<grid, kThreads, 0, stream>>>(A.rows, A.rowptr.p, A.colind.p, A.val.p, x, y, \
        alpha, beta, epi, A.aux.long_rows.p, A.aux.n_long, A.aux.main_blocks, A.aux.long_thr, A.done_flag)
#define CUADMM_SPMV_CASE(G)                                                                            \
    case G:                                                                                            \
        switch (epi.mode) {                                                                            \
            case 0: CUADMM_SPMV_LAUNCH(G, 0); break;                                                   \
            case 1: CUADMM_SPMV_LAUNCH(G, 1); break;                                                   \
            case 2: CUADMM_SPMV_LAUNCH(G, 2); break;                                                   \
            case 3: CUADMM_SPMV_LAUNCH(G, 3); break;                                                   \
            case 4: CUADMM_SPMV_LAUNCH(G, 4); break;                                                   \
            case 5: CUADMM_SPMV_LAUNCH(G, 5); break;                                                   \
            default: throw Error(CUADMM_EINVAL, "bad spmv epilogue mode");                             \
        }                                                                                              \
        break;
    switch (A.group) {
        CUADMM_SPMV_CASE(1)
        CUADMM_SPMV_CASE(2)
        CUADMM_SPMV_CASE(4)
        CUADMM_SPMV_CASE(8)
        CUADMM_SPMV_CASE(16)
        CUADMM_SPMV_CASE(32)
        default: throw Error(CUADMM_EINVAL, "bad spmv group size");
    }
#undef CUADMM_SPMV_LAUNCH
#undef CUADMM_SPMV_CASE
    CUADMM_CUDA(cudaGetLastError());
}

cuadmm_spmv_s* spmv_create(int64_t rows, int64_t cols, int64_t nnz, const int32_t* h_rowptr,
                         const int32_t* h_colind, const double* h_val, int device) {
    CUADMM_REQUIRE(rows >= 0 && cols >= 0 && nnz >= 0, "negative dimension");
    CUADMM_REQUIRE(nnz <= INT32_MAX, "nnz exceeds int32 row pointers");
    CUADMM_REQUIRE(h_rowptr != nullptr, "rowptr is null");
    CUADMM_REQUIRE(h_rowptr[0] == 0 && h_rowptr[rows] == nnz, "rowptr does not span nnz");
    int cnt = 0;
    if (cudaGetDeviceCount(&cnt) != cudaSuccess || cnt == 0) {
        cudaGetLastError();
        throw Error(CUADMM_ENODEVICE, "no CUDA device available; SpMV has no CPU fallback");
    }
    CUADMM_REQUIRE(device >= 0 && device < cnt, "device index out of range");
    std::unique_ptr<cuadmm_spmv_full> A(new cuadmm_spmv_full());
    A->device = device; A->rows = rows; A->cols = cols; A->nnz = nnz;
    DeviceGuard g(device);
    A->rowptr.alloc(rows + 1); A->rowptr.upload(h_rowptr, rows + 1);
    A->colind.alloc(std::max<int64_t>(nnz, 1)); A->colind.upload(h_colind, nnz);
    A->val.alloc(std::max<int64_t>(nnz, 1)); A->val.upload(h_val, nnz);
    std::vector<int32_t> longs;
    int64_t short_nnz = 0, short_rows = 0;
    for (int64_t i = 0; i < rows; ++i) {
        CUADMM_REQUIRE(h_rowptr[i + 1] >= h_rowptr[i], "rowptr not monotone");
        const int len = h_rowptr[i + 1] - h_rowptr[i];
        if (len > 0 && len <= kLongRow) { short_nnz += len; ++short_rows; }
    }
    for (int64_t p = 0; p < nnz; ++p) CUADMM_REQUIRE(h_colind[p] >= 0 && h_colind[p] < cols, "column index out of range");
    const double mean = short_rows ? (double)short_nnz / (double)short_rows : 1.0;
    int G = 1;
    while (G < 32 && (double)G < mean) G <<= 1;
    if (mean <= 4.0 && rows >= 262144) G = 1;
    if (const char* e = getenv("CUADMM_SPMV_G")) {
        const int g = atoi(e);
        if (g >= 1 && g <= 32 && (g & (g - 1)) == 0) G = g;
    }
    A->group = G;
    int long_thr = kLongRow;
    if (G == 1 && rows >= 262144) long_thr = 16;
    if (const char* e = getenv("CUADMM_SPMV_LONG")) { const int t = atoi(e); if (t >= 1 && t <= kLongRow) long_thr = t; }
    A->aux.long_thr = long_thr;
    for (int64_t i = 0; i < rows; ++i)
        if (h_rowptr[i + 1] - h_rowptr[i] > long_thr) longs.push_back((int32_t)i);
    A->aux.n_long = (int)longs.size();
    if (!longs.empty()) { A->aux.long_rows.upload(longs); }
    int sm = 148;
    cudaDeviceGetAttribute(&sm, cudaDevAttrMultiProcessorCount, device);
    const int64_t need = (rows * G + kThreads - 1) / kThreads;
    const int cap_default = CUADMM_SPMV_MINB;
    int cap = cap_default;
    if (const char* e = getenv("CUADMM_SPMV_CAP")) { const int c = atoi(e); if (c >= 1 && c <= 32) cap = c; }
    A->aux.main_blocks = (int)std::min<int64_t>(std::max<int64_t>(need, 1), (int64_t)sm * cap);
    A->aux.long_blocks = longs.empty() ? 0 : (int)std::min<int64_t>(((int64_t)longs.size() + 7) / 8, (int64_t)sm);
    CUADMM_CUDA(cudaStreamSynchronize(0));
    return A.release();
}

}

extern "C" {

int cuadmm_spmv_create(int64_t rows, int64_t cols, int64_t nnz, const int32_t* h_rowptr, const int32_t* h_colind,
                       const double* h_val, int device, cuadmm_spmv_t** out) {
    return guarded([&] {
        CUADMM_REQUIRE(out != nullptr, "out is null");
        *out = nullptr;
        *out = spmv_create(rows, cols, nnz, h_rowptr, h_colind, h_val, device);
    });
}

void cuadmm_spmv_destroy(cuadmm_spmv_t* A) { delete static_cast<cuadmm_spmv_full*>(A); }

int cuadmm_spmv(cuadmm_spmv_t* A, double alpha, const double* d_x, double beta, double* d_y, void* stream) {
    return guarded([&] {
        CUADMM_REQUIRE(A && d_x && d_y, "null argument");
        DeviceGuard g(A->device);
        SpmvEpilogue e;
        spmv_launch(*A, alpha, d_x, beta, d_y, e, (cudaStream_t)stream);
    });
}

int cuadmm_spmv_host(cuadmm_spmv_t* A, double alpha, const double* h_x, double beta, double* h_y) {
    return guarded([&] {
        CUADMM_REQUIRE(A && h_x && h_y, "null argument");
        DeviceGuard g(A->device);
        if (A->d_x.n != A->cols) A->d_x.alloc(A->cols);
        if (A->d_y.n != A->rows) A->d_y.alloc(A->rows);
        A->d_x.upload(h_x, A->cols);
        A->d_y.upload(h_y, A->rows);
        SpmvEpilogue e;
        spmv_launch(*A, alpha, A->d_x.p, beta, A->d_y.p, e, 0);
        A->d_y.download(h_y, A->rows);
        CUADMM_CUDA(cudaStreamSynchronize(0));
    });
}

int cuadmm_normA_host(int64_t con_num, const int32_t* At_col_ptrs, double* At_vals, double* normA) {
    return guarded([&] {
        CUADMM_REQUIRE(At_col_ptrs && At_vals && normA, "null argument");
        for (int64_t i = 0; i < con_num; ++i) {
            double norm = 0.0;
            for (int p = At_col_ptrs[i]; p < At_col_ptrs[i + 1]; ++p) norm += At_vals[p] * At_vals[p];
            norm = std::max(1.0, sqrt(norm));
            normA[i] = norm;
            for (int p = At_col_ptrs[i]; p < At_col_ptrs[i + 1]; ++p) At_vals[p] /= norm;
        }
    });
}

int cuadmm_csc_to_csr_host(int64_t nrows, int64_t ncols, int64_t nnz, const int32_t* col_ptrs, const int32_t* row_ids,
                           const double* vals, int32_t* row_ptrs, int32_t* col_ids, double* out_vals) {
    return guarded([&] {
        CUADMM_REQUIRE(col_ptrs && row_ptrs, "null argument");
        std::vector<int64_t> cnt(nrows + 1, 0);
        for (int64_t p = 0; p < nnz; ++p) {
            CUADMM_REQUIRE(row_ids[p] >= 0 && row_ids[p] < nrows, "row index out of range");
            cnt[row_ids[p] + 1]++;
        }
        for (int64_t i = 0; i < nrows; ++i) cnt[i + 1] += cnt[i];
        for (int64_t i = 0; i <= nrows; ++i) row_ptrs[i] = (int32_t)cnt[i];
        std::vector<int64_t> next(cnt.begin(), cnt.end() - 1);
        for (int64_t c = 0; c < ncols; ++c)
            for (int p = col_ptrs[c]; p < col_ptrs[c + 1]; ++p) {
                const int64_t q = next[row_ids[p]]++;
                col_ids[q] = (int32_t)c;
                out_vals[q] = vals[p];
            }
    });
}
// ... 3 lines not shown
```

cuadmm_b200/csrc/spmv.h:

```cpp
#pragma once
#include "common.h"

struct cuadmm_spmv_s {
    int device = -1;
    int64_t rows = 0, cols = 0, nnz = 0;
    cuadmm::DevBuf<int32_t> rowptr, colind;
    cuadmm::DevBuf<double> val;
    int group = 1;
    cuadmm::DevBuf<double> d_x, d_y;
    int64_t alg_bytes() const { return 12 * nnz + 4 * (rows + 1) + 8 * rows + 8 * cols; }
};

namespace cuadmm {

struct SpmvEpilogue {
    int mode = 0;
    const double* aux1 = nullptr;
    const double* aux2 = nullptr;
    const double* aux3 = nullptr;
    double* out2 = nullptr;
    double* out3 = nullptr;
    const double* scal = nullptr;
    double* partial = nullptr;
    double* push[8] = {nullptr, nullptr, nullptr, nullptr, nullptr, nullptr, nullptr, nullptr};
    unsigned slice = 1;
    int rank = 0;
};

void spmv_launch(const cuadmm_spmv_s& A, double alpha, const double* x, double beta, double* y,
                 const SpmvEpilogue& epi, cudaStream_t stream, int* grid_out = nullptr);
int spmv_grid(const cuadmm_spmv_s& A);
cuadmm_spmv_s* spmv_create(int64_t rows, int64_t cols, int64_t nnz, const int32_t* h_rowptr,
                         const int32_t* h_colind, const double* h_val, int device);
void spmv_set_done_flag(cuadmm_spmv_s& A, const int* flag);

}
```

cuadmm_b200/csrc/ysolve.cu:

```cuda
#include "ysolve.h"
#include <chrono>
#include <thread>
#include <atomic>
#include "dense.h"
#include <algorithm>
#include <numeric>
#include <stdio.h>
#include <stdlib.h>

namespace cuadmm {

static constexpr int kTriThreads = 256;
static constexpr int kLongRowNnz = 24;
static constexpr int kNarrowSlots = 160;
static constexpr int kNarrowThreads = 1024;

struct SlotWork {
    static constexpr int K = 4;
    int32_t u; int is_long;
    double rv, invd;
    int64_t p, p1; int step;
    int32_t d[K]; double v[K];

    __device__ __forceinline__ void load(int64_t s, int lane, const int32_t* __restrict__ slot_rows,
            const int32_t* __restrict__ slot_info, const int64_t* __restrict__ ptr, const int32_t* __restrict__ dep,
            const double* __restrict__ val, const double* __restrict__ inv_diag, const double* __restrict__ rhs,
            const int32_t* __restrict__ rhs_gather) {
        is_long = slot_info[s] >> 30;
        u = slot_rows[8 * s + (is_long ? 0 : (lane >> 2))];
        step = is_long ? 32 : 4;
        p = 0; p1 = 0; rv = 0.0; invd = 0.0;
        if (u >= 0) {
            p = ptr[u] + (is_long ? lane : (lane & 3));
            p1 = ptr[u + 1];
            invd = inv_diag[u];
            rv = rhs_gather ? rhs[rhs_gather[u]] : rhs[u];
        }
#pragma unroll
        for (int k = 0; k < K; ++k) {
            const int64_t q = p + (int64_t)k * step;
            if (q < p1) { d[k] = dep[q]; v[k] = val[q]; } else { d[k] = -1; v[k] = 0.0; }
        }
    }
    __device__ __forceinline__ void finish(int lane, const int32_t* __restrict__ dep, const double* __restrict__ val,
                                           double* x, double* out_scatter, const int32_t* __restrict__ out_perm) {
        double acc = 0.0;
#pragma unroll
        for (int k = 0; k < K; ++k) if (d[k] >= 0) acc = fma(v[k], x[d[k]], acc);
        for (int64_t q = p + (int64_t)K * step; q < p1; q += step) acc = fma(val[q], x[dep[q]], acc);
        acc += __shfl_xor_sync(0xffffffffu, acc, 1);
        acc += __shfl_xor_sync(0xffffffffu, acc, 2);
        if (is_long) {
            acc += __shfl_xor_sync(0xffffffffu, acc, 4);
            acc += __shfl_xor_sync(0xffffffffu, acc, 8);
            acc += __shfl_xor_sync(0xffffffffu, acc, 16);
        }
        const bool writer = (u >= 0) && (is_long ? (lane == 0) : ((lane & 3) == 0));
        if (writer) {
            const double r = (rv - acc) * invd;
            x[u] = r;
            if (out_scatter) out_scatter[out_perm[u]] = r;
        }
    }
};

#define CUADMM_TRI_PARAMS                                                                                   \
    const int32_t* __restrict__ slot_rows, const int32_t* __restrict__ slot_info, const int64_t* __restrict__ ptr, \
    const int32_t* __restrict__ dep, const double* __restrict__ val, const double* __restrict__ inv_diag,   \
    const double* __restrict__ rhs, const int32_t* __restrict__ rhs_gather, double* x, double* out_scatter, \
    const int32_t* __restrict__ out_perm, const int* __restrict__ done_flag
#define CUADMM_TRI_LOAD(W, S) (W).load((S), lane, slot_rows, slot_info, ptr, dep, val, inv_diag, rhs, rhs_gather)
#define CUADMM_TRI_FINISH(W) (W).finish(lane, dep, val, x, out_scatter, out_perm)

__global__ void __launch_bounds__(kTriThreads) tri_wide_kernel(int64_t slot0, int64_t slot1, CUADMM_TRI_PARAMS) {
    if (done_flag && *done_flag) return;
    const int lane = threadIdx.x & 31;
    const int64_t s = slot0 + (((int64_t)blockIdx.x * kTriThreads + threadIdx.x) >> 5);
    if (s >= slot1) return;
    SlotWork w;
    CUADMM_TRI_LOAD(w, s);
    CUADMM_TRI_FINISH(w);
}

template <int NW>
__device__ __forceinline__ void tri_level_loop(const int64_t* __restrict__ lvl_ptr, int level0, int level1, int lane, int warp,
        CUADMM_TRI_PARAMS) {
    (void)done_flag;
    if (level0 >= level1) return;
    SlotWork w;
    int64_t s0 = lvl_ptr[level0];
    int64_t s1 = lvl_ptr[level0 + 1];
    bool have = (s0 + warp) < s1;
    if (have) CUADMM_TRI_LOAD(w, s0 + warp);
    for (int l = level0; l < level1; ++l) {
        if (have) {
            CUADMM_TRI_FINISH(w);
            for (int64_t s = s0 + warp + NW; s < s1; s += NW) { SlotWork t; CUADMM_TRI_LOAD(t, s); CUADMM_TRI_FINISH(t); }
        }
        s0 = s1;
        have = false;
        if (l + 1 < level1) {
            s1 = lvl_ptr[l + 2];
            have = (s0 + warp) < s1;
            if (have) CUADMM_TRI_LOAD(w, s0 + warp);
        }
        __syncthreads();
    }
}

__global__ void __launch_bounds__(kNarrowThreads) tri_narrow_kernel(int level0, int level1, const int64_t* __restrict__ level_ptr,
                                                                    CUADMM_TRI_PARAMS) {
    if (done_flag && *done_flag) return;
    tri_level_loop<kNarrowThreads / 32>(level_ptr, level0, level1, threadIdx.x & 31, threadIdx.x >> 5,
        slot_rows, slot_info, ptr, dep, val, inv_diag, rhs, rhs_gather, x, out_scatter, out_perm, done_flag);
}

__global__ void __launch_bounds__(kTriThreads) tri_subtree_kernel(const int64_t* __restrict__ sub_off,
        const int64_t* __restrict__ sub_lvl_ptr, CUADMM_TRI_PARAMS) {
    if (done_flag && *done_flag) return;
    const int64_t base = sub_off[blockIdx.x];
    const int nl = (int)(sub_off[blockIdx.x + 1] - base) - 1;
    tri_level_loop<kTriThreads / 32>(sub_lvl_ptr + base, 0, nl, threadIdx.x & 31, threadIdx.x >> 5,
        slot_rows, slot_info, ptr, dep, val, inv_diag, rhs, rhs_gather, x, out_scatter, out_perm, done_flag);
}

#ifndef CUADMM_PK_CHUNK
#define CUADMM_PK_CHUNK 65536
#endif
#ifndef CUADMM_PK_RING
#define CUADMM_PK_RING 2
#endif
static constexpr int kPkChunk = CUADMM_PK_CHUNK;
static constexpr int kPkRing = CUADMM_PK_RING;
#ifndef CUADMM_PK_THREADS
#define CUADMM_PK_THREADS 1024
#endif
static constexpr int kPkThreads = CUADMM_PK_THREADS;
static constexpr int kPkRecHeader = 8 + 32 + 16 + 16 + 16 + 64;
static constexpr int kPkMaxRowEntries = 768;
static constexpr int kPkMaxRows = 23000;
static constexpr int kPkChainMax = 384;

__device__ __forceinline__ uint32_t smem_u32(const void* p) { return (uint32_t)__cvta_generic_to_shared(p); }

__device__ __forceinline__ long long pk_globaltimer() {
    long long t;
    asm volatile("mov.u64 %0, %%globaltimer;" : "=l"(t));
    return t;
}

__device__ __forceinline__ void pk_fetch(unsigned char* dst, const unsigned char* src, uint64_t* bar) {
    asm volatile("mbarrier.arrive.expect_tx.shared::cta.b64 _, [%0], %1;" :: "r"(smem_u32(bar)), "r"(kPkChunk) : "memory");
    asm volatile("cp.async.bulk.shared::cluster.global.mbarrier::complete_tx::bytes [%0], [%1], %2, [%3];"
                 :: "r"(smem_u32(dst)), "l"(src), "r"(kPkChunk), "r"(smem_u32(bar)) : "memory");
}

__device__ __forceinline__ void pk_wait(uint64_t* bar, uint32_t parity) {
    uint32_t ok;
    do {
        asm volatile("{ .reg .pred p; mbarrier.try_wait.parity.shared::cta.b64 p, [%1], %2; selp.u32 %0, 1, 0, p; }"
                     : "=r"(ok) : "r"(smem_u32(bar)), "r"(parity) : "memory");
    } while (!ok);
}

__device__ __forceinline__ void pk_record(const unsigned char* rec, int lane, double* xs) {
    const int r = lane >> 2;
    const bool is_long = *reinterpret_cast<const int32_t*>(rec) != 0;
    const int ul = reinterpret_cast<const int32_t*>(rec + 8)[r];
    const int voff = reinterpret_cast<const uint16_t*>(rec + 40)[r];
    const int ioff = reinterpret_cast<const uint16_t*>(rec + 56)[r];
    const int ln = reinterpret_cast<const uint16_t*>(rec + 72)[r];
    const double invd = reinterpret_cast<const double*>(rec + 88)[r];
    const int j = is_long ? lane : (lane & 3);
    const int step = is_long ? 32 : 4;
    const double* val = reinterpret_cast<const double*>(rec) + voff;
    const uint16_t* idx = reinterpret_cast<const uint16_t*>(rec) + ioff;
    const double cur = ul >= 0 ? xs[ul] : 0.0;
    double acc = 0.0;
    for (int k = j; k < ln; k += step) acc = fma(val[k], xs[idx[k]], acc);
    acc += __shfl_xor_sync(0xffffffffu, acc, 1);
    acc += __shfl_xor_sync(0xffffffffu, acc, 2);
    if (is_long) {
        acc += __shfl_xor_sync(0xffffffffu, acc, 4);
        acc += __shfl_xor_sync(0xffffffffu, acc, 8);
        acc += __shfl_xor_sync(0xffffffffu, acc, 16);
    }
    if (ul >= 0 && j == 0) xs[ul] = (cur - acc) * invd;
}

static constexpr int kPkHeavyExt = 8;

__global__ void __launch_bounds__(256) pk_gather_kernel(int64_t n_rows, int main_blocks, const int32_t* __restrict__ heavy,
        int n_heavy, const int32_t* __restrict__ prow_src, const int64_t* __restrict__ ext_ptr,
        const int32_t* __restrict__ ext_dep, const double* __restrict__ ext_val, const double* __restrict__ rhs,
        const double* __restrict__ x, double* __restrict__ w, const int* __restrict__ done_flag) {
    if (done_flag && *done_flag) return;
    if ((int)blockIdx.x < main_blocks) {
        const int64_t g = (int64_t)blockIdx.x * 256 + threadIdx.x;
        if (g >= n_rows) return;
        const int32_t src = prow_src[g];
        double acc = src >= 0 ? rhs[src] : 0.0;
        if (ext_ptr) {
            const int64_t p0 = ext_ptr[g], p1 = ext_ptr[g + 1];
            if (p1 - p0 > kPkHeavyExt) return;
            for (int64_t p = p0; p < p1; ++p) acc = fma(-ext_val[p], x[ext_dep[p]], acc);
        }
        w[g] = acc;
    } else {
        const int lane = threadIdx.x & 31;
        const int hw = ((int)blockIdx.x - main_blocks) * 8 + (threadIdx.x >> 5);
        if (hw >= n_heavy) return;
        const int64_t g = heavy[hw];
        double acc = 0.0;
        for (int64_t p = ext_ptr[g] + lane; p < ext_ptr[g + 1]; p += 32) acc = fma(ext_val[p], x[ext_dep[p]], acc);
#pragma unroll
        for (int o = 16; o > 0; o >>= 1) acc += __shfl_xor_sync(0xffffffffu, acc, o);
        if (lane == 0) {
            const int32_t src = prow_src[g];
            w[g] = (src >= 0 ? rhs[src] : 0.0) - acc;
        }
    }
}

__device__ __forceinline__ void pk_record2(const unsigned char* recA, const unsigned char* recB, bool hasB, int lane, double* xs) {
    const int r = lane >> 2;
    const bool longA = *reinterpret_cast<const int32_t*>(recA) != 0;
    const bool longB = *reinterpret_cast<const int32_t*>(recB) != 0;
    const int ulA = reinterpret_cast<const int32_t*>(recA + 8)[r];
    const int ulB = hasB ? reinterpret_cast<const int32_t*>(recB + 8)[r] : -1;
    const int voffA = reinterpret_cast<const uint16_t*>(recA + 40)[r], voffB = reinterpret_cast<const uint16_t*>(recB + 40)[r];
    const int ioffA = reinterpret_cast<const uint16_t*>(recA + 56)[r], ioffB = reinterpret_cast<const uint16_t*>(recB + 56)[r];
    const int lnA = reinterpret_cast<const uint16_t*>(recA + 72)[r];
    const int lnB = hasB ? reinterpret_cast<const uint16_t*>(recB + 72)[r] : 0;
    const double invdA = reinterpret_cast<const double*>(recA + 88)[r], invdB = reinterpret_cast<const double*>(recB + 88)[r];
    const int jA = longA ? lane : (lane & 3), jB = longB ? lane : (lane & 3);
    const int stepA = longA ? 32 : 4, stepB = longB ? 32 : 4;
    const double* valA = reinterpret_cast<const double*>(recA) + voffA;
    const double* valB = reinterpret_cast<const double*>(recB) + voffB;
    const uint16_t* idxA = reinterpret_cast<const uint16_t*>(recA) + ioffA;
    const uint16_t* idxB = reinterpret_cast<const uint16_t*>(recB) + ioffB;
    const double curA = ulA >= 0 ? xs[ulA] : 0.0;
    const double curB = ulB >= 0 ? xs[ulB] : 0.0;
    double accA = 0.0, accB = 0.0;
    int kA = jA, kB = jB;
    while (kA < lnA || kB < lnB) {
        const bool a = kA < lnA, b = kB < lnB;
        double va = 0.0, vb = 0.0;
        int ia = 0, ib = 0;
        if (a) { va = valA[kA]; ia = idxA[kA]; }
        if (b) { vb = valB[kB]; ib = idxB[kB]; }
        const double xa = xs[ia], xb = xs[ib];
        if (a) accA = fma(va, xa, accA);
        if (b) accB = fma(vb, xb, accB);
        kA += stepA; kB += stepB;
    }
    accA += __shfl_xor_sync(0xffffffffu, accA, 1);
    accB += __shfl_xor_sync(0xffffffffu, accB, 1);
    accA += __shfl_xor_sync(0xffffffffu, accA, 2);
    accB += __shfl_xor_sync(0xffffffffu, accB, 2);
    if (longA || longB) {
        double tA = accA, tB = accB;
        tA += __shfl_xor_sync(0xffffffffu, tA, 4);  tB += __shfl_xor_sync(0xffffffffu, tB, 4);
        tA += __shfl_xor_sync(0xffffffffu, tA, 8);  tB += __shfl_xor_sync(0xffffffffu, tB, 8);
        tA += __shfl_xor_sync(0xffffffffu, tA, 16); tB += __shfl_xor_sync(0xffffffffu, tB, 16);
        if (longA) accA = tA;
        if (longB) accB = tB;
    }
    if (ulA >= 0 && jA == 0) xs[ulA] = (curA - accA) * invdA;
    if (ulB >= 0 && jB == 0) xs[ulB] = (curB - accB) * invdB;
}

template <int NW, bool WARP>
__device__ __forceinline__ void pk_chunk(const unsigned char* chunk, int lane, int warp, double* xs) {
    const uint16_t* dir = reinterpret_cast<const uint16_t*>(chunk);
    const int nseg = dir[0];
    const uint16_t* seg_end = dir + 2;
    const uint16_t* rec_off = seg_end + nseg;
    int sb = 0;
    for (int g = 0; g < nseg; ++g) {
        const int se = seg_end[g];
        int sl = sb + warp;
        if constexpr (!WARP) {
            for (; sl + NW < se; sl += 2 * NW)
                pk_record2(chunk + 8 * (int)rec_off[sl], chunk + 8 * (int)rec_off[sl + NW], true, lane, xs);
        }
        for (; sl < se; sl += NW) pk_record(chunk + 8 * (int)rec_off[sl], lane, xs);
        if constexpr (WARP) __syncwarp(); else __syncthreads();
        sb = se;
    }
}

__global__ void __launch_bounds__(kPkThreads, 1) tri_packed_kernel(const int64_t* __restrict__ chunk_off,
        const int64_t* __restrict__ row_off, const unsigned char* __restrict__ stream, const int32_t* __restrict__ prow_u,
        const int32_t* __restrict__ prow_out, const double* __restrict__ w, double* x, double* out_scatter,
        const int* __restrict__ done_flag, long long* __restrict__ timeline) {
    if (done_flag && *done_flag) return;
    if (timeline && threadIdx.x == 0) timeline[4 * blockIdx.x + 0] = pk_globaltimer();
    extern __shared__ __align__(128) unsigned char pk_smem[];
    unsigned char* ring = pk_smem;
    uint64_t* bars = reinterpret_cast<uint64_t*>(pk_smem + kPkRing * kPkChunk);
    double* xs = reinterpret_cast<double*>(pk_smem + kPkRing * kPkChunk + 64);
    const int tid = threadIdx.x, lane = tid & 31, warp = tid >> 5;
    const int64_t c0 = chunk_off[blockIdx.x];
    const int nc = (int)(chunk_off[blockIdx.x + 1] - c0);
    const int64_t r0 = row_off[blockIdx.x];
    const int nr = (int)(row_off[blockIdx.x + 1] - r0);
    const unsigned char* src = stream + c0 * kPkChunk;
    if (tid == 0) {
        for (int i = 0; i < kPkRing; ++i)
            asm volatile("mbarrier.init.shared::cta.b64 [%0], 1;" :: "r"(smem_u32(bars + i)) : "memory");
        asm volatile("fence.mbarrier_init.release.cluster;" ::: "memory");
        asm volatile("fence.proxy.async.shared::cta;" ::: "memory");
        for (int i = 0; i < kPkRing && i < nc; ++i) pk_fetch(ring + i * kPkChunk, src + (int64_t)i * kPkChunk, bars + i);
    }
#pragma unroll 4
    for (int loc = tid; loc < nr; loc += kPkThreads) xs[loc] = w[r0 + loc];
    __syncthreads();
    if (timeline && tid == 0) timeline[4 * blockIdx.x + 1] = pk_globaltimer();
    for (int c = 0; c < nc; ++c) {
        const int b = c % kPkRing;
        pk_wait(bars + b, (uint32_t)((c / kPkRing) & 1));
        pk_chunk<kPkThreads / 32, false>(ring + b * kPkChunk, lane, warp, xs);
        if (tid == 0 && c + kPkRing < nc) pk_fetch(ring + b * kPkChunk, src + (int64_t)(c + kPkRing) * kPkChunk, bars + b);
    }
    if (timeline && tid == 0) timeline[4 * blockIdx.x + 2] = pk_globaltimer();
#pragma unroll 4
    for (int loc = tid; loc < nr; loc += kPkThreads) {
        const int32_t u = prow_u[r0 + loc];
        if (u < 0) continue;
        const double r = xs[loc];
        x[u] = r;
        if (out_scatter) out_scatter[prow_out[r0 + loc]] = r;
    }
    if (timeline && tid == 0) timeline[4 * blockIdx.x + 3] = pk_globaltimer();
}

static constexpr int kPkWarpBlob = 2048;
static constexpr int kPkWarpRows = 32;
static constexpr int kPkWarpThreads = 256;

__global__ void __launch_bounds__(kPkWarpThreads, 5) tri_packed_warp_kernel(int64_t count, const int64_t* __restrict__ blob_off,
        const int64_t* __restrict__ row_off, const uint4* __restrict__ blobs, const int32_t* __restrict__ prow_u,
        const int32_t* __restrict__ prow_out, const double* __restrict__ w, double* x, double* out_scatter,
        const int* __restrict__ done_flag) {
    if (done_flag && *done_flag) return;
    __shared__ __align__(16) unsigned char slices[kPkWarpThreads / 32][kPkWarpBlob];
    __shared__ double xs_all[kPkWarpThreads / 32][kPkWarpRows];
    const int lane = threadIdx.x & 31, warp = threadIdx.x >> 5;
    const int64_t t = (int64_t)blockIdx.x * (kPkWarpThreads / 32) + warp;
    if (t >= count) return;
    const int64_t b0 = blob_off[t];
    const int nb = (int)(blob_off[t + 1] - b0);
    const int64_t r0 = row_off[t];
    const int nr = (int)(row_off[t + 1] - r0);
    uint4* slice = reinterpret_cast<uint4*>(slices[warp]);
    double* xs = xs_all[warp];
    for (int i = lane; i < nb; i += 32) slice[i] = blobs[b0 + i];
    int32_t u = -1, po = -1;
    if (lane < nr) {
        xs[lane] = w[r0 + lane];
        u = prow_u[r0 + lane];
        if (out_scatter) po = prow_out[r0 + lane];
    }
    __syncwarp();
    pk_chunk<1, true>(slices[warp], lane, 0, xs);
    if (lane < nr && u >= 0) {
        const double r = xs[lane];
        x[u] = r;
        if (out_scatter) out_scatter[po] = r;
    }
}

__global__ void __launch_bounds__(256) tail_gemv_row_kernel(int64_t r, const double* __restrict__ T, const double* __restrict__ in,
                                                        double* out, const int32_t* __restrict__ tile_ptr,
                                                        const int32_t* __restrict__ tile_col, double* out_scatter,
                                                        const int32_t* __restrict__ out_perm, int64_t perm_base,
                                                        const int* __restrict__ done_flag, int longest_last) {
    if (done_flag && *done_flag) return;
    const int lane = threadIdx.x & 31;
    const int64_t cta = longest_last ? (int64_t)gridDim.x - 1 - blockIdx.x : blockIdx.x;
    const int64_t row = cta * (blockDim.x >> 5) + (threadIdx.x >> 5);
    if (row >= r) return;
    const double* Ti = T + row * r;
    const int I = (int)(row >> 6);
    double acc0 = 0.0, acc1 = 0.0;
    const bool vec = (r & 1) == 0 && (reinterpret_cast<uintptr_t>(T) & 15) == 0;
    const bool in_al = (reinterpret_cast<uintptr_t>(in) & 15) == 0;
    for (int t = tile_ptr[I]; t < tile_ptr[I + 1]; ++t) {
        const int64_t j0 = tile_col[2 * t];
        const int64_t j1 = min((int64_t)tile_col[2 * t + 1], r);
        if (vec) {
            const int64_t jv = j0 + ((j1 - j0) & ~(int64_t)1);
#pragma unroll 4
            for (int64_t j = j0 + 2 * lane; j < jv; j += 64) {
                const double2 a = __ldcs(reinterpret_cast<const double2*>(Ti + j));
                const double2 b = in_al ? *reinterpret_cast<const double2*>(in + j) : make_double2(in[j], in[j + 1]);
                acc0 = fma(a.x, b.x, acc0);
                acc1 = fma(a.y, b.y, acc1);
            }
            if (lane == 0 && jv < j1) acc0 = fma(Ti[jv], in[jv], acc0);
        } else {
#pragma unroll 4
            for (int64_t j = j0 + lane; j < j1; j += 32) acc0 = fma(Ti[j], in[j], acc0);
        }
    }
    double acc = acc0 + acc1;
#pragma unroll
    for (int o = 16; o > 0; o >>= 1) acc += __shfl_xor_sync(0xffffffffu, acc, o);
    if (lane == 0) {
        out[row] = acc;
        if (out_scatter) out_scatter[out_perm[perm_base + row]] = acc;
    }
}

__global__ void __launch_bounds__(256) tail_gemv_kernel(int64_t r, const double* __restrict__ T, const double* in,
                                                        double* out, const int32_t* __restrict__ tile_ptr,
                                                        const int32_t* __restrict__ tile_col, double* out_scatter,
                                                        const int32_t* __restrict__ out_perm, int64_t perm_base,
                                                        const int* __restrict__ done_flag, int longest_last,
                                                        int64_t row0, int64_t nrows, int npush, PeerView pv,
                                                        PeerPtrs outp, PeerPtrs scatp, int splits, double* split_part,
                                                        unsigned int* split_count) {
    if (done_flag && *done_flag) return;
    __shared__ double part[8][9];
    __shared__ int s_final;
    const int lane = threadIdx.x & 31, w = threadIdx.x >> 5;
    unsigned long long ep = 0;
    if (npush) ep = peer_epoch(pv);
    const int sp = (int)(blockIdx.x % (unsigned)splits);
    const int64_t rb = blockIdx.x / (unsigned)splits, nrb = gridDim.x / (unsigned)splits;
    const int64_t cta = longest_last ? nrb - 1 - rb : rb;
    const int64_t base = row0 + cta * 8;
    const int nr = (int)max((int64_t)0, min((int64_t)8, row0 + nrows - base));
    double acc[8];
#pragma unroll
    for (int q = 0; q < 8; ++q) acc[q] = 0.0;
    if (nr > 0) {
        const int I = (int)(base >> 6);
        const bool vec = (r & 1) == 0 && (reinterpret_cast<uintptr_t>(T) & 15) == 0 && (reinterpret_cast<uintptr_t>(in) & 15) == 0;
        const double* Tb = T + base * r;
        int g = 0;
        for (int t = tile_ptr[I]; t < tile_ptr[I + 1]; ++t) {
            const int64_t j0 = tile_col[2 * t];
            const int64_t j1 = min((int64_t)tile_col[2 * t + 1], r);
            const int nch = (int)((j1 - j0 + 63) >> 6);
            const int g0 = g;
            int c = (w - (g & 7)) & 7;
            g += nch;
            for (; c < nch; c += 8) {
                if (splits > 1 && (((g0 + c) >> 3) % splits) != sp) continue;
                const int64_t j = j0 + ((int64_t)c << 6) + 2 * lane;
                if (vec) {
                    if (j + 1 < j1) {
                        const double2 b = *reinterpret_cast<const double2*>(in + j);
#pragma unroll
                        for (int q = 0; q < 8; ++q) {
                            if (q < nr) {
                                const double2 a = __ldcs(reinterpret_cast<const double2*>(Tb + q * r + j));
                                acc[q] = fma(a.x, b.x, fma(a.y, b.y, acc[q]));
                            }
                        }
                    } else if (j < j1) {
                        const double b = in[j];
#pragma unroll
                        for (int q = 0; q < 8; ++q) if (q < nr) acc[q] = fma(Tb[q * r + j], b, acc[q]);
                    }
                } else {
#pragma unroll
                    for (int h = 0; h < 2; ++h) {
                        const int64_t jj = j0 + ((int64_t)c << 6) + lane + 32 * h;
                        if (jj < j1) {
                            const double b = in[jj];
#pragma unroll
                            for (int q = 0; q < 8; ++q) if (q < nr) acc[q] = fma(Tb[q * r + jj], b, acc[q]);
                        }
                    }
                }
            }
        }
    }
#pragma unroll
    for (int q = 0; q < 8; ++q) {
#pragma unroll
        for (int o = 16; o > 0; o >>= 1) acc[q] += __shfl_xor_sync(0xffffffffu, acc[q], o);
    }
    if (lane == 0) {
#pragma unroll
        for (int q = 0; q < 8; ++q) part[w][q] = acc[q];
    }
    __syncthreads();
    const int t = threadIdx.x;
    bool final_cta = true;
    if (splits > 1) {
        if (t < 8) {
            double v = 0.0;
#pragma unroll
            for (int k = 0; k < 8; ++k) v += part[k][t];
            split_part[(rb * splits + sp) * 8 + t] = v;
        }
        __syncthreads();
        if (t == 0) {
            __threadfence();
            const unsigned old = atomicAdd(split_count + rb, 1u);
            s_final = (old == (unsigned)splits - 1u) ? 1 : 0;
            if (s_final) { split_count[rb] = 0u; __threadfence(); }
        }
        __syncthreads();
        final_cta = s_final != 0;
    }
    if (final_cta && t < 8 * max(npush, 1)) {
        const int q = t >> 3, rr = t & 7;
        if (rr < nr) {
            double v = 0.0;
            if (splits > 1) {
                for (int k = 0; k < splits; ++k) v += __ldcg(split_part + (rb * splits + k) * 8 + rr);
            } else {
#pragma unroll
                for (int k = 0; k < 8; ++k) v += part[k][rr];
            }
            if (npush == 0) {
                out[base + rr] = v;
                if (out_scatter) out_scatter[out_perm[perm_base + base + rr]] = v;
            } else {
                outp.p[q][base + rr] = v;
            }
        }
    }
    if (npush) peer_leave(pv, ep);
}

__global__ void __launch_bounds__(256) tail_scatter_kernel(int64_t r, const double* __restrict__ xt, const int32_t* __restrict__ perm,
                                                           int64_t base, double* y, const int* __restrict__ done_flag) {
    if (done_flag && *done_flag) return;
    const int64_t i = (int64_t)blockIdx.x * 256 + threadIdx.x;
    if (i < r) y[perm[base + i]] = xt[i];
}

static int launch_subtrees(const TriSweep& S, const double* rhs, const int32_t* gather, double* x, double* out_scatter,
                           const int32_t* out_perm, const int* done, cudaStream_t st, const SweepStreams& ss) {
    int launches = 0;
    if (S.pk_rows > 0) {
        const int main_blocks = (int)((S.pk_rows + 255) / 256);
        pk_gather_kernel<<<(unsigned)(main_blocks + (S.pk_n_heavy + 7) / 8), 256, 0, st>>>(S.pk_rows, main_blocks, S.pk_heavy.p,
            (int)S.pk_n_heavy, S.pk_prow_src.p, S.pk_has_ext ? S.pk_ext_ptr.p : nullptr, S.pk_ext_dep.p, S.pk_ext_val.p, rhs, x,
            S.pk_w.p, done);
        ++launches;
    }
    const bool fork = S.n_sub_warp > 0 && (S.n_sub_pack > 0 || S.n_sub_cta > 0);
    cudaStream_t wst = st;
    if (fork) {
        CUADMM_CUDA(cudaEventRecord(ss.fork, st));
        CUADMM_CUDA(cudaStreamWaitEvent(ss.side, ss.fork, 0));
        wst = ss.side;
    }
    if (S.n_sub_pack > 0) {
        tri_packed_kernel<<<(unsigned)S.n_sub_pack, kPkThreads, S.pk_smem, st>>>(S.pk_chunk_off.p, S.pk_row_off.p, S.pk_stream.p,
            S.pk_prow_u.p, S.pk_prow_out.p, S.pk_w.p, x, out_scatter, done, S.pk_timeline.n ? S.pk_timeline.p : nullptr);
        ++launches;
    }
    if (S.n_sub_warp > 0) {
        const int wpb = kPkWarpThreads / 32;
        tri_packed_warp_kernel<<<(unsigned)((S.n_sub_warp + wpb - 1) / wpb), kPkWarpThreads, 0, wst>>>(S.n_sub_warp,
            S.pk_blob_off.p, S.pk_row_off.p + S.n_sub_pack, reinterpret_cast<const uint4*>(S.pk_blobs.p), S.pk_prow_u.p,
            S.pk_prow_out.p, S.pk_w.p, x, out_scatter, done);
        ++launches;
    }
    if (S.n_sub_cta > 0) {
        tri_subtree_kernel<<<(unsigned)S.n_sub_cta, kTriThreads, 0, st>>>(S.sub_off.p, S.sub_lvl_ptr.p, S.slot_rows.p, S.slot_info.p,
            S.ptr.p, S.dep.p, S.val.p, S.inv_diag.p, rhs, gather, x, out_scatter, out_perm, done);
        ++launches;
    }
    if (fork) {
        CUADMM_CUDA(cudaEventRecord(ss.join, ss.side));
        CUADMM_CUDA(cudaStreamWaitEvent(st, ss.join, 0));
    }
    return launches;
}

static int launch_sweep(const TriSweep& S, const double* rhs, const int32_t* gather, double* x,
                        double* out_scatter, const int32_t* out_perm, const int* done, cudaStream_t st, const SweepStreams& ss) {
    int launches = 0;
    if (S.subtrees_first && S.n_sub) launches += launch_subtrees(S, rhs, gather, x, out_scatter, out_perm, done, st, ss);
    for (const TriSweep::Phase& ph : S.phases) {
        if (ph.narrow) {
            tri_narrow_kernel<<<1, kNarrowThreads, 0, st>>>(ph.level0, ph.level1, S.level_ptr.p, S.slot_rows.p, S.slot_info.p,
                S.ptr.p, S.dep.p, S.val.p, S.inv_diag.p, rhs, gather, x, out_scatter, out_perm, done);
        } else {
            const int64_t s0 = S.h_level_ptr[ph.level0], s1 = S.h_level_ptr[ph.level1];
            const int grid = (int)(((s1 - s0) * 32 + kTriThreads - 1) / kTriThreads);
            tri_wide_kernel<<<grid, kTriThreads, 0, st>>>(s0, s1, S.slot_rows.p, S.slot_info.p, S.ptr.p, S.dep.p, S.val.p,
                S.inv_diag.p, rhs, gather, x, out_scatter, out_perm, done);
        }
        ++launches;
    }
    if (!S.subtrees_first && S.n_sub) launches += launch_subtrees(S, rhs, gather, x, out_scatter, out_perm, done, st, ss);
    CUADMM_CUDA(cudaGetLastError());
    return launches;
}

struct HostSweep {
    std::vector<int64_t> ptr;
    std::vector<int32_t> dep;
    std::vector<double> val, inv_diag;
    int64_t n = 0;
    std::vector<int32_t> order;
    std::vector<int32_t> sub;
    int64_t n_sub = 0;
    bool subtrees_first = true;
    const std::vector<int32_t>* gather = nullptr;
    const std::vector<int32_t>* out_perm = nullptr;
};

static int64_t emit_level_slots(const HostSweep& H, std::vector<int32_t>& rows, int level,
                                std::vector<int32_t>& slot_rows, std::vector<int32_t>& slot_info) {
    std::vector<int32_t> longs, shorts;
    for (int32_t u : rows) ((H.ptr[u + 1] - H.ptr[u]) > kLongRowNnz ? longs : shorts).push_back(u);
    std::stable_sort(longs.begin(), longs.end(), [&](int32_t a, int32_t b) {
        return H.ptr[a + 1] - H.ptr[a] > H.ptr[b + 1] - H.ptr[b]; });
    int64_t cnt = 0;
    for (int32_t u : longs) {
        slot_rows.push_back(u);
        for (int t = 1; t < 8; ++t) slot_rows.push_back(-1);
        slot_info.push_back(level | (1 << 30));
        ++cnt;
    }
    for (size_t t = 0; t < shorts.size(); t += 8) {
        for (size_t q = t; q < t + 8; ++q) slot_rows.push_back(q < shorts.size() ? shorts[q] : -1);
        slot_info.push_back(level);
        ++cnt;
    }
    return cnt;
}

struct PkRow {
    int32_t slot; double invd;
    std::vector<uint16_t> idx; std::vector<double> val;
};

static void pack_subtrees(const HostSweep& H, TriSweep& S, const std::vector<std::vector<int32_t>>& members,
                          const std::vector<int32_t>& level, const std::vector<int32_t>& depth, std::vector<int>& kind) {
    struct Packed {
        std::vector<unsigned char> bytes; int32_t t; size_t last_used; int levels;
        std::vector<int32_t> slot_u, slot_src;
    };
    std::vector<Packed> packs, blobs;
    std::vector<int32_t> loc(H.n, -1), cidx(H.n, -1), height(H.n, 0), lvl_r(H.n, 0);
    int chain_max = kPkChainMax, chain_gain = 6;
    if (const char* e = getenv("CUADMM_SWEEP_CHAIN_MAX")) chain_max = std::min(atoi(e), kPkMaxRowEntries);
    const bool verbose = getenv("CUADMM_YSOLVE_VERBOSE") != nullptr;
    int64_t n_collapsed = 0, levels_before = 0, levels_after = 0, chain_entries = 0;
    kind.assign(H.n_sub, 0);
    auto same = [&](int32_t u, int64_t p) { return H.sub[H.dep[p]] == H.sub[u]; };
    std::vector<Packed> result(H.n_sub);
    std::atomic<int64_t> a_collapsed{0}, a_before{0}, a_after{0}, a_entries{0};
    auto do_subtree = [&](int64_t t) {
        const std::vector<int32_t>& rows = members[t];
        const int32_t nr0 = (int32_t)rows.size();
        if (nr0 + chain_max > kPkMaxRows) return;
        int32_t longest = 0;
        for (int32_t q = 0; q < nr0; ++q) {
            const int32_t u = rows[q];
            loc[u] = q;
            int32_t cnt = 0;
            for (int64_t p = H.ptr[u]; p < H.ptr[u + 1]; ++p) cnt += same(u, p) ? 1 : 0;
            longest = std::max(longest, cnt);
        }
        if (longest > kPkMaxRowEntries) return;
        std::vector<int32_t> C;
        int new_depth = depth[t], k0 = 0;
        if (chain_max > 0 && depth[t] > chain_gain + 2 && nr0 > kPkWarpRows) {
            const bool initial = !H.subtrees_first;
            std::vector<int32_t> key(nr0);
            if (initial) {
                for (int32_t u : rows) height[u] = 0;
                for (int32_t q = nr0 - 1; q >= 0; --q) {
                    const int32_t u = rows[q];
                    for (int64_t p = H.ptr[u]; p < H.ptr[u + 1]; ++p)
                        if (same(u, p)) height[H.dep[p]] = std::max(height[H.dep[p]], height[u] + 1);
                }
                for (int32_t q = 0; q < nr0; ++q) key[q] = height[rows[q]];
            } else {
                for (int32_t q = 0; q < nr0; ++q) key[q] = level[rows[q]];
            }
            std::vector<int32_t> cnt(depth[t] + 1, 0);
            for (int32_t q = 0; q < nr0; ++q) ++cnt[key[q]];
            int32_t acc = 0;
            k0 = depth[t];
            while (k0 > 0 && acc + cnt[k0 - 1] <= chain_max) { --k0; acc += cnt[k0]; }
            const int nd = initial ? k0 + 1 : k0 + 2;
            if (acc > 0 && depth[t] - nd >= chain_gain) {
                new_depth = nd;
                for (int32_t q = 0; q < nr0; ++q) if (key[q] >= k0) C.push_back(rows[q]);
            }
        }
        const int32_t nC = (int32_t)C.size();
        for (int32_t i = 0; i < nC; ++i) cidx[C[i]] = i;
        std::vector<std::vector<PkRow>> lv(new_depth);
        auto plain_row = [&](int32_t u) {
            PkRow r; r.slot = loc[u]; r.invd = H.inv_diag[u];
            for (int64_t p = H.ptr[u]; p < H.ptr[u + 1]; ++p)
                if (same(u, p)) { r.idx.push_back((uint16_t)loc[H.dep[p]]); r.val.push_back(H.val[p]); }
            return r;
        };
        if (nC == 0) {
            for (int32_t u : rows) lv[level[u]].push_back(plain_row(u));
        } else {
            std::vector<double> M((size_t)nC * nC, 0.0);
            for (int32_t i = 0; i < nC; ++i) {
                const int32_t u = C[i];
                double* mi = M.data() + (size_t)i * nC;
                mi[i] = 1.0;
                for (int64_t p = H.ptr[u]; p < H.ptr[u + 1]; ++p) {
                    if (!same(u, p) || cidx[H.dep[p]] < 0) continue;
                    const int32_t k = cidx[H.dep[p]];
                    const double v = H.val[p];
                    const double* mk = M.data() + (size_t)k * nC;
                    for (int32_t j = 0; j <= k; ++j) mi[j] -= v * mk[j];
                }
                const double d = H.inv_diag[u];
                for (int32_t j = 0; j <= i; ++j) mi[j] *= d;
            }
            const bool initial = !H.subtrees_first;
            const int lvB = initial ? 0 : k0 + 1;
            for (int32_t i = 0; i < nC; ++i) {
                PkRow r; r.slot = loc[C[i]]; r.invd = -1.0;
                const double* mi = M.data() + (size_t)i * nC;
                for (int32_t j = 0; j <= i; ++j) if (mi[j] != 0.0) { r.idx.push_back((uint16_t)(nr0 + j)); r.val.push_back(mi[j]); }
                a_entries += (int64_t)r.idx.size();
                lv[lvB].push_back(std::move(r));
            }
            if (initial) {
                for (int32_t u : rows) {
                    if (cidx[u] >= 0) continue;
                    int32_t l = 0;
                    for (int64_t p = H.ptr[u]; p < H.ptr[u + 1]; ++p)
                        if (same(u, p) && cidx[H.dep[p]] < 0) l = std::max(l, lvl_r[H.dep[p]] + 1);
                    lvl_r[u] = l;
                    lv[1 + l].push_back(plain_row(u));
                }
            } else {
                for (int32_t u : rows) {
                    if (cidx[u] < 0) { lv[level[u]].push_back(plain_row(u)); continue; }
                    PkRow r; r.slot = nr0 + cidx[u]; r.invd = 1.0;
                    for (int64_t p = H.ptr[u]; p < H.ptr[u + 1]; ++p)
                        if (same(u, p) && cidx[H.dep[p]] < 0) { r.idx.push_back((uint16_t)loc[H.dep[p]]); r.val.push_back(H.val[p]); }
                    if (!r.idx.empty()) lv[k0].push_back(std::move(r));
                }
            }
// ... 361 lines not shown
    std::vector<int32_t> perm1; perm1.reserve(m);
    for (int64_t k = 0; k < m; ++k) if (lev[k] < cut) perm1.push_back(F.perm[k]);
    const int64_t n_lead = (int64_t)perm1.size();
    for (int64_t k = 0; k < m; ++k) if (lev[k] >= cut) perm1.push_back(F.perm[k]);
    const int64_t n_tail = m - n_lead;
    SymCsc C;
    if (n_tail > 0) {
        F = CholFactor();
        chol_symbolic(M, perm1, F, &C);
    } else {
        chol_symbolic(M, perm0, F, &C);
    }
    lap("symbolic (2, tail last)");
    chol_numeric(C, F, n_lead);
    lap("numeric (sparse lead part)");
    Y->n_lead = n_lead; Y->n_tail = n_tail;
    Y->nnz_L = F.nnz();
    Y->n_deficient = F.n_deficient;
    Y->h_perm = F.perm;
    Y->perm.upload(F.perm);

    std::vector<int32_t> sub;
    const int64_t n_sub = choose_subtrees(F, n_lead, sub);
    {
        HostSweep H;
        H.n = m;
        H.ptr.assign(m + 1, 0);
        for (int64_t j = 0; j < n_lead; ++j)
            for (int64_t p = F.Lp[j] + 1; p < F.Lp[j + 1]; ++p) H.ptr[F.Li[p] + 1]++;
        for (int64_t i = 0; i < m; ++i) H.ptr[i + 1] += H.ptr[i];
        H.dep.resize(H.ptr[m]); H.val.resize(H.ptr[m]);
        std::vector<int64_t> nx(H.ptr.begin(), H.ptr.end() - 1);
        for (int64_t j = 0; j < n_lead; ++j)
            for (int64_t p = F.Lp[j] + 1; p < F.Lp[j + 1]; ++p) {
                const int64_t q = nx[F.Li[p]]++;
                H.dep[q] = (int32_t)j; H.val[q] = F.Lx[p];
            }
        H.inv_diag.assign(m, 1.0);
        for (int64_t i = 0; i < n_lead; ++i) H.inv_diag[i] = 1.0 / F.Lx[F.Lp[i]];
        H.order.resize(m);
        std::iota(H.order.begin(), H.order.end(), 0);
        H.sub = sub; H.n_sub = n_sub; H.subtrees_first = true;
        H.gather = &Y->h_perm;
        upload_sweep(H, Y->fwd);
    }
    {
        HostSweep H;
        H.n = m;
        H.ptr.assign(m + 1, 0);
        for (int64_t j = 0; j < n_lead; ++j) H.ptr[j + 1] = F.Lp[j + 1] - F.Lp[j] - 1;
        for (int64_t i = 0; i < m; ++i) H.ptr[i + 1] += H.ptr[i];
        H.dep.resize(H.ptr[m]); H.val.resize(H.ptr[m]);
        for (int64_t j = 0; j < n_lead; ++j) {
            int64_t q = H.ptr[j];
            for (int64_t p = F.Lp[j] + 1; p < F.Lp[j + 1]; ++p, ++q) { H.dep[q] = F.Li[p]; H.val[q] = F.Lx[p]; }
        }
        H.inv_diag.assign(m, 1.0);
        for (int64_t i = 0; i < n_lead; ++i) H.inv_diag[i] = 1.0 / F.Lx[F.Lp[i]];
        H.order.resize(n_lead);
        for (int64_t j = 0; j < n_lead; ++j) H.order[j] = (int32_t)(n_lead - 1 - j);
        H.sub = sub;
        for (int64_t i = n_lead; i < m; ++i) H.sub[i] = -2;
        H.n_sub = n_sub; H.subtrees_first = false;
        H.out_perm = &Y->h_perm;
        upload_sweep(H, Y->bwd);
    }
    lap("pack + upload sweeps");
    Y->z.alloc(std::max<int64_t>(m, 1));
    Y->x.alloc(std::max<int64_t>(m, 1));

    if (n_tail > 0) {
        int64_t tail_def = 0;
        std::vector<int> flags;
        build_dense_tail(C, F, n_lead, n_tail, Y->tail_inv, Y->tail_inv_t, &tail_def, &flags);
        const int nt = (int)((n_tail + 63) / 64);
        std::vector<int32_t> tp(1, 0), tc, tpt(1, 0), tct;
        auto add_runs = [&](std::vector<int32_t>& ptr, std::vector<int32_t>& col, int J0, int J1, auto used) {
            for (int J = J0; J < J1;) {
                if (!used(J)) { ++J; continue; }
                int E = J;
                while (E < J1 && used(E)) ++E;
                col.push_back(J * 64); col.push_back(E * 64);
                J = E;
            }
            ptr.push_back((int32_t)(col.size() / 2));
        };
        Y->h_tail_cost[0].assign(nt, 0.0); Y->h_tail_cost[1].assign(nt, 0.0);
        for (int I = 0; I < nt; ++I) {
            add_runs(tp, tc, 0, I + 1, [&](int J) { return flags[(size_t)I * nt + J] != 0; });
            add_runs(tpt, tct, I, nt, [&](int J) { return flags[(size_t)J * nt + I] != 0; });
            for (int32_t t = tp[I]; t < tp[I + 1]; ++t) Y->h_tail_cost[0][I] += tc[2 * t + 1] - tc[2 * t];
            for (int32_t t = tpt[I]; t < tpt[I + 1]; ++t) Y->h_tail_cost[1][I] += tct[2 * t + 1] - tct[2 * t];
        }
        if (tc.empty()) tc.assign(2, 0);
        if (tct.empty()) tct.assign(2, 0);
        Y->tail_tptr.upload(tp); Y->tail_tcol.upload(tc); Y->tail_tptr_t.upload(tpt); Y->tail_tcol_t.upload(tct);
        Y->n_deficient += tail_def;
        Y->tail_tmp.alloc(n_tail);
        lap("dense tail (GPU)");
    }
    Y->launches_per_solve = (int)(Y->fwd.phases.size() + Y->bwd.phases.size()) + (n_tail > 0 ? 2 : 0) +
                            (Y->fwd.n_sub_cta > 0 ? 2 : 0) + (Y->fwd.n_sub_warp > 0 ? 2 : 0) + (Y->fwd.n_sub_pack > 0 ? 2 : 0) +
                            (Y->fwd.pk_rows > 0 ? 2 : 0);
    CUADMM_CUDA(cudaStreamCreateWithFlags(&Y->streams.side, cudaStreamNonBlocking));
    CUADMM_CUDA(cudaEventCreateWithFlags(&Y->streams.fork, cudaEventDisableTiming));
    CUADMM_CUDA(cudaEventCreateWithFlags(&Y->streams.join, cudaEventDisableTiming));
    Y->alg_bytes = 2 * (12 * Y->nnz_L + 8 * m) + 24 * m;
    CUADMM_CUDA(cudaDeviceSynchronize());
    return Y.release();
}

}

using namespace cuadmm;

cuadmm_ysolve_s::~cuadmm_ysolve_s() {
    if (streams.fork) cudaEventDestroy(streams.fork);
    if (streams.join) cudaEventDestroy(streams.join);
    if (streams.side) cudaStreamDestroy(streams.side);
}

void cuadmm_ysolve_s::enable_peer(const PeerComm* pc, size_t off_tmp, size_t off_x) {
    peer = pc;
    peer_tmp = pc->ptrs(off_tmp);
    peer_x = pc->ptrs(off_x);
    tail_tmp_p = pc->local<double>(off_tmp);
    x_p = pc->local<double>(off_x);
    if (n_tail > 0 && pc->world > 1) launches_per_solve += 1;
    split_tail_rows(pc->world, pc->rank);
}

void cuadmm_ysolve_s::split_tail_rows(int world, int rank) {
    for (int k = 0; k < 2; ++k) {
        const std::vector<double>& c = h_tail_cost[k];
        double total = 0.0;
        for (int64_t i = 0; i < n_tail; ++i) total += c[i >> 6] + 32.0;
        std::vector<int64_t> cut(world + 1, n_tail);
        cut[0] = 0;
        double acc = 0.0;
        int q = 1;
        for (int64_t i = 0; i < n_tail && q < world; ++i) {
            acc += c[i >> 6] + 32.0;
            while (q < world && acc >= total * q / world) cut[q++] = std::min<int64_t>(n_tail, (i + 1 + 7) / 8 * 8);
        }
        tail_row0[k] = cut[rank]; tail_row1[k] = cut[rank + 1];
    }
    const int64_t nrb = std::max<int64_t>(1, (std::max(tail_row1[0] - tail_row0[0], tail_row1[1] - tail_row0[1]) + 7) / 8);
    split_part.alloc(nrb * 8 * 8);
    split_count.alloc(nrb);
    split_count.zero();
    CUADMM_CUDA(cudaDeviceSynchronize());
}

void cuadmm_ysolve_s::solve(const double* d_rhs_, double* d_y_, cudaStream_t st) {
    if (m == 0) return;
    double* xv = x_p ? x_p : x.p;
    double* tmpv = tail_tmp_p ? tail_tmp_p : tail_tmp.p;
    launch_sweep(fwd, d_rhs_, perm.p, z.p, nullptr, nullptr, done_flag, st, streams);
    auto mark = [&](int tag) {
        if (!prof_ev) return;
        cudaEvent_t ev;
        CUADMM_CUDA(cudaEventCreate(&ev));
        CUADMM_CUDA(cudaEventRecord(ev, st));
        prof_ev->push_back(ev); prof_tag->push_back(tag);
    };
    auto gemv_split = [&](const double* Tm, const double* in, double* out, const int32_t* tp, const int32_t* tc, int longest_last,
                          int64_t r0, int64_t nrows_, int npush, const PeerView& pv, const PeerPtrs& outp) {
        const int64_t nrb = std::max<int64_t>(1, (nrows_ + 7) / 8);
        int splits = (int)std::min<int64_t>(8, std::max<int64_t>(1, (2 * 148 + nrb - 1) / nrb));
        CUADMM_REQUIRE(split_part.n >= nrb * 8 * 8 && split_count.n >= nrb, "internal: split-column GEMV scratch too small");
        tail_gemv_kernel<<<(unsigned)(nrb * splits), 256, 0, st>>>(n_tail, Tm, in, out, tp, tc, nullptr, nullptr, 0, done_flag,
            longest_last, r0, nrows_, npush, pv, outp, PeerPtrs(), splits, split_part.p, split_count.p);
    };
    if (n_tail > 0) {
        mark(20);
        if (!peer || peer->world == 1) {
            const int blocks = (int)((n_tail + 7) / 8);
            tail_gemv_row_kernel<<<blocks, 256, 0, st>>>(n_tail, tail_inv.p, z.p + n_lead, tmpv, tail_tptr.p, tail_tcol.p,
                                                         nullptr, nullptr, 0, done_flag, 1);
            tail_gemv_row_kernel<<<blocks, 256, 0, st>>>(n_tail, tail_inv_t.p, tmpv, xv + n_lead, tail_tptr_t.p, tail_tcol_t.p,
                                                         d_y_, perm.p, n_lead, done_flag, 0);
        } else {
            PeerPtrs pxt = peer_x;
            for (int q = 0; q < peer->world; ++q) pxt.p[q] += n_lead;
            const PeerView pv = peer->view();
            const int64_t n0 = tail_row1[0] - tail_row0[0], n1 = tail_row1[1] - tail_row0[1];
            gemv_split(tail_inv.p, z.p + n_lead, tmpv, tail_tptr.p, tail_tcol.p, 1, tail_row0[0], n0, peer->world, pv, peer_tmp);
            gemv_split(tail_inv_t.p, tmpv, xv + n_lead, tail_tptr_t.p, tail_tcol_t.p, 0, tail_row0[1], n1, peer->world, pv, pxt);
            tail_scatter_kernel<<<(int)((n_tail + 255) / 256), 256, 0, st>>>(n_tail, xv + n_lead, perm.p, n_lead, d_y_, done_flag);
        }
        CUADMM_CUDA(cudaGetLastError());
        mark(21);
    }
    launch_sweep(bwd, z.p, nullptr, xv, d_y_, perm.p, done_flag, st, streams);
}

extern "C" {

int cuadmm_ysolve_create(int64_t m, int64_t vec_len, int64_t nnz, const int32_t* h_A_rowptr, const int32_t* h_A_colind,
                         const double* h_A_val, double eps, int device, cuadmm_ysolve_t** out) {
    return guarded([&] {
        CUADMM_REQUIRE(out != nullptr, "out is null");
        *out = nullptr;
        *out = ysolve_create(m, vec_len, nnz, h_A_rowptr, h_A_colind, h_A_val, eps, device);
    });
}

void cuadmm_ysolve_destroy(cuadmm_ysolve_t* ys) { delete ys; }

int cuadmm_ysolve(cuadmm_ysolve_t* ys, const double* d_rhs, double* d_y, void* stream) {
    return guarded([&] {
        CUADMM_REQUIRE(ys && d_rhs && d_y, "null argument");
        DeviceGuard g(ys->device);
        ys->solve(d_rhs, d_y, (cudaStream_t)stream);
    });
}

int cuadmm_debug_ysolve_timeline(cuadmm_ysolve_t* ys, int which, long long* timeline, long long* meta, int64_t cap, int64_t* n) {
    return guarded([&] {
        CUADMM_REQUIRE(ys && n, "null argument");
        DeviceGuard g(ys->device);
        const cuadmm::TriSweep& S = which ? ys->bwd : ys->fwd;
        *n = S.pk_timeline.n / 4;
        if (!timeline || cap < *n || *n == 0) return;
        CUADMM_CUDA(cudaDeviceSynchronize());
        CUADMM_CUDA(cudaMemcpy(timeline, S.pk_timeline.p, sizeof(long long) * 4 * (size_t)*n, cudaMemcpyDeviceToHost));
        if (meta) std::copy(S.pk_timeline_meta.begin(), S.pk_timeline_meta.end(), meta);
    });
}

int cuadmm_ysolve_host(cuadmm_ysolve_t* ys, const double* h_rhs, double* h_y) {
    return guarded([&] {
        CUADMM_REQUIRE(ys && h_rhs && h_y, "null argument");
        DeviceGuard g(ys->device);
        if (ys->d_rhs.n != ys->m) { ys->d_rhs.alloc(std::max<int64_t>(ys->m, 1)); ys->d_y.alloc(std::max<int64_t>(ys->m, 1)); }
        ys->d_rhs.upload(h_rhs, ys->m);
        ys->solve(ys->d_rhs.p, ys->d_y.p, 0);
        ys->d_y.download(h_y, ys->m);
        CUADMM_CUDA(cudaStreamSynchronize(0));
    });
}

int cuadmm_ysolve_stats(const cuadmm_ysolve_t* ys, int64_t out[8]) {
    return guarded([&] {
        CUADMM_REQUIRE(ys && out, "null argument");
        out[0] = ys->nnz_aat; out[1] = ys->nnz_L; out[2] = std::max(ys->fwd.levels, ys->bwd.levels);
        out[3] = ys->n_tail; out[4] = ys->launches_per_solve; out[5] = ys->alg_bytes;
        out[6] = ys->n_deficient; out[7] = ys->fwd.n_sub * 100000 + ys->fwd.sub_depth;
    });
}

int cuadmm_ysolve_perm(const cuadmm_ysolve_t* ys, int32_t* perm) {
    return guarded([&] {
        CUADMM_REQUIRE(ys && perm, "null argument");
        std::copy(ys->h_perm.begin(), ys->h_perm.end(), perm);
    });
}

}
```

cuadmm_b200/csrc/ysolve.h:

```cpp
#pragma once
#include "common.h"
#include "chol_host.h"
#include "peer.h"

namespace cuadmm {

struct TriSweep {
    int64_t n_unknowns = 0;
    int64_t nnz = 0;
    DevBuf<int64_t> ptr;
    DevBuf<int32_t> dep;
    DevBuf<double> val;
    DevBuf<double> inv_diag;
    DevBuf<int32_t> slot_rows;
    DevBuf<int32_t> slot_info;
    DevBuf<int64_t> level_ptr;
    std::vector<int64_t> h_level_ptr;
    struct Phase { bool narrow; int level0, level1; };
    std::vector<Phase> phases;
    int64_t n_slots = 0;
    int levels = 0;
    DevBuf<int64_t> sub_off, sub_lvl_ptr;
    int64_t n_sub = 0;
    int64_t n_sub_cta = 0;
    int64_t n_sub_pack = 0, n_sub_warp = 0, pk_rows = 0;
    DevBuf<unsigned char> pk_stream, pk_blobs;
    DevBuf<int64_t> pk_chunk_off, pk_blob_off, pk_row_off, pk_ext_ptr;
    DevBuf<int32_t> pk_prow_u, pk_prow_src, pk_prow_out, pk_ext_dep, pk_heavy;
    int64_t pk_n_heavy = 0;
    DevBuf<double> pk_ext_val, pk_w;
    DevBuf<long long> pk_timeline;
    std::vector<long long> pk_timeline_meta;
    size_t pk_smem = 0;
    bool pk_has_ext = false;
    int sub_depth = 0;
    bool subtrees_first = true;
};

struct SweepStreams {
    cudaStream_t side = nullptr;
    cudaEvent_t fork = nullptr, join = nullptr;
};

}

struct cuadmm_ysolve_s {
    int device = -1;
    int64_t m = 0;
    int64_t n_lead = 0, n_tail = 0;
    int64_t nnz_aat = 0, nnz_L = 0, n_deficient = 0;
    cuadmm::TriSweep fwd, bwd;
    cuadmm::DevBuf<int32_t> perm;
    cuadmm::DevBuf<double> z;
    cuadmm::DevBuf<double> x;
    cuadmm::DevBuf<double> tail_inv, tail_inv_t, tail_tmp;
    cuadmm::DevBuf<int32_t> tail_tptr, tail_tcol, tail_tptr_t, tail_tcol_t;
    cuadmm::DevBuf<double> d_rhs, d_y;
    std::vector<int32_t> h_perm;
    const cuadmm::PeerComm* peer = nullptr;
    double* tail_tmp_p = nullptr;
    double* x_p = nullptr;
    cuadmm::PeerPtrs peer_tmp, peer_x;
    int64_t tail_row0[2] = {0, 0}, tail_row1[2] = {0, 0};
    std::vector<double> h_tail_cost[2];
    void enable_peer(const cuadmm::PeerComm* pc, size_t off_tmp, size_t off_x);
    void split_tail_rows(int world, int rank);
    cuadmm::DevBuf<double> split_part;
    cuadmm::DevBuf<unsigned int> split_count;
    const int* done_flag = nullptr;
    std::vector<cudaEvent_t>* prof_ev = nullptr;
    std::vector<int>* prof_tag = nullptr;
    cuadmm::SweepStreams streams;
    ~cuadmm_ysolve_s();
    int launches_per_solve = 0;
    int64_t alg_bytes = 0;
    void solve(const double* d_rhs, double* d_y, cudaStream_t stream);
};

namespace cuadmm {
cuadmm_ysolve_s* ysolve_create(int64_t m, int64_t vec_len, int64_t nnz, const int32_t* rowptr, const int32_t* colind,
                               const double* val, double eps, int device);
}
```

Before: 828.4.

## Chain ADMM iteration kernels with programmatic dependent launch inside CUDA graphs

Launches the per-iteration kernel sequence (SpMV, rhs, triangular sweeps, tail GEMV, projection, scalar update) through cudaLaunchKernelEx with programmatic stream serialization, and adds griddepcontrol.wait at the start of each kernel. A chain flag tracks where PDL is safe and is reset after memsets, event joins and non-PDL launches. The aim is to overlap each kernel's launch and prologue with the tail of the one before it in a long chain of small kernels. It also adds optional stream-priority attributes (off by default) and graph instantiation with node priorities. The risk is extra per-kernel overhead from the wait instruction, and wrong results if any chain reset is missing.

```diff
diff --git a/cuadmm_b200/csrc/common.cpp b/cuadmm_b200/csrc/common.cpp
--- a/cuadmm_b200/csrc/common.cpp
+++ b/cuadmm_b200/csrc/common.cpp
@@ -4,6 +4,12 @@
 namespace cuadmm {
 static thread_local std::string g_last_error;
 void set_last_error(const std::string& msg) { g_last_error = msg; }
+int64_t& pdl_launch_count() { static thread_local int64_t n = 0; return n; }
+int high_priority() {
+    int least = 0, greatest = 0;
+    if (cudaDeviceGetStreamPriorityRange(&least, &greatest) != cudaSuccess) { cudaGetLastError(); return 0; }
+    return greatest;
+}
 }
 
 extern "C" {
diff --git a/cuadmm_b200/csrc/common.h b/cuadmm_b200/csrc/common.h
--- a/cuadmm_b200/csrc/common.h
+++ b/cuadmm_b200/csrc/common.h
@@ -82,4 +82,39 @@
 
 static inline int64_t tri(int64_t n) { return n * (n + 1) / 2; }
 
+#ifdef __CUDACC__
+__device__ __forceinline__ void pdl_wait() { asm volatile("griddepcontrol.wait;" ::: "memory"); }
+#endif
+
+int64_t& pdl_launch_count();
+
+int high_priority();
+
+template <class... KArgs, class... Args>
+static inline void pdl_launch_prio(void (*kernel)(KArgs...), dim3 grid, dim3 block, size_t smem, cudaStream_t stream, bool allow,
+                                   int priority, Args&&... args) {
+    cudaLaunchAttribute attr[2];
+    attr[0].id = cudaLaunchAttributeProgrammaticStreamSerialization;
+    attr[0].val.programmaticStreamSerializationAllowed = allow ? 1 : 0;
+    attr[1].id = cudaLaunchAttributePriority;
+    attr[1].val.priority = priority;
+    cudaLaunchConfig_t cfg = {};
+    cfg.gridDim = grid; cfg.blockDim = block; cfg.dynamicSmemBytes = smem; cfg.stream = stream;
+    cfg.attrs = attr; cfg.numAttrs = 2;
+    CUADMM_CUDA(cudaLaunchKernelEx(&cfg, kernel, std::forward<Args>(args)...));
+    if (allow) ++pdl_launch_count();
 }
+template <class... KArgs, class... Args>
+static inline void pdl_launch(void (*kernel)(KArgs...), dim3 grid, dim3 block, size_t smem, cudaStream_t stream, bool allow,
+                              Args&&... args) {
+    pdl_launch_prio(kernel, grid, block, smem, stream, allow, 0, std::forward<Args>(args)...);
+}
+
+static inline bool pdl_next(bool* pdl_chain) {
+    if (!pdl_chain) return false;
+    const bool allow = *pdl_chain;
+    *pdl_chain = true;
+    return allow;
+}
+
+}
diff --git a/cuadmm_b200/csrc/debug_api.cpp b/cuadmm_b200/csrc/debug_api.cpp
--- a/cuadmm_b200/csrc/debug_api.cpp
+++ b/cuadmm_b200/csrc/debug_api.cpp
@@ -1,5 +1,6 @@
 #include "chol_host.h"
 #include "common.h"
+#include "solver.h"
 #include <algorithm>
 #include <cmath>
 
@@ -90,4 +91,11 @@
     });
 }
 
+int cuadmm_debug_graph_edges(cuadmm_solver* s, int64_t out[3]) {
+    return guarded([&] {
+        CUADMM_REQUIRE(s && out, "null argument");
+        for (int k = 0; k < 3; ++k) out[k] = s->graph_sgs ? s->graph_edges_sgs[k] : 0;
+    });
 }
+
+}
diff --git a/cuadmm_b200/csrc/plan.h b/cuadmm_b200/csrc/plan.h
--- a/cuadmm_b200/csrc/plan.h
+++ b/cuadmm_b200/csrc/plan.h
@@ -70,5 +70,5 @@
     ~cuadmm_plan();
     void build_device();
     int project(const double* d_Xb, double* d_Xproj, cudaStream_t stream,
-                const cuadmm::ProjEpilogue* epi, bool want_eig);
+                const cuadmm::ProjEpilogue* epi, bool want_eig, bool* pdl_chain = nullptr);
 };
diff --git a/cuadmm_b200/csrc/project.cu b/cuadmm_b200/csrc/project.cu
--- a/cuadmm_b200/csrc/project.cu
+++ b/cuadmm_b200/csrc/project.cu
@@ -1,3 +1,9 @@
+#ifndef CUADMM_EXP_PROJ
+#define CUADMM_EXP_PROJ 0
+#endif
+#ifndef CUADMM_EXP_PK
+#define CUADMM_EXP_PK 0
+#endif
 #include "plan.h"
 #include <algorithm>
 #include <limits>
@@ -136,6 +142,7 @@
     const int tid = WARP ? (threadIdx.x & 31) : threadIdx.x;
     const int mat_in_cta = WARP ? (threadIdx.x >> 5) : 0;
     const int bi = blockIdx.x * MPC + mat_in_cta;
+    pdl_wait();
     if (bi >= a.nblk) return;
     if (a.done_flag && *a.done_flag) return;
 
@@ -745,12 +752,13 @@
 }
 
 int cuadmm_plan::project(const double* d_Xb, double* d_Xproj, cudaStream_t stream,
-                         const ProjEpilogue* epi, bool want_eig) {
+                         const ProjEpilogue* epi, bool want_eig, bool* pdl_chain) {
     if (device < 0) throw Error(CUADMM_ENODEVICE, "plan was built without a CUDA device; there is no CPU fallback");
     int launches = 0;
     if (want_eig) {
         CUADMM_CUDA(cudaMemsetAsync(d_eig.p, 0xFF, sizeof(double) * (size_t)d_eig.n, stream));
         CUADMM_CUDA(cudaMemsetAsync(d_sweeps.p, 0, sizeof(int32_t) * (size_t)d_sweeps.n, stream));
+        if (pdl_chain) *pdl_chain = false;
     }
     const bool has_dense = dense != nullptr;
     const bool has_lin = !h_lin.empty();
@@ -782,8 +790,10 @@
         if (epi) a.epi = *epi; else { a.epi.X = nullptr; a.epi.Rd1 = nullptr; a.epi.Cd = nullptr; a.epi.S = nullptr; a.epi.SmC = nullptr; a.epi.sig_ptr = nullptr; }
         if (cl.kind == kGlobalKind) {
             proj_jacobi_global_kernel<<<cl.grid, 1024, 0, st>>>(a);
+            if (!side && pdl_chain) *pdl_chain = true;
         } else {
-            kSizeClasses[cl.kind].fn<<<cl.grid, kSizeClasses[cl.kind].threads, cl.smem, st>>>(a, cl.nmax);
+            pdl_launch_prio(kSizeClasses[cl.kind].fn, cl.grid, kSizeClasses[cl.kind].threads, cl.smem, st,
+                       side ? false : pdl_next(pdl_chain), ((CUADMM_EXP_PROJ == 1 && side) || (CUADMM_EXP_PROJ == 2 && !side)) ? high_priority() : 0, a, cl.nmax);
         }
         CUADMM_CUDA(cudaGetLastError());
         ++launches;
@@ -802,6 +812,7 @@
     for (size_t i = 0; i < classes.size(); ++i)
         if (has_dense || i > 0) CUADMM_CUDA(cudaStreamWaitEvent(stream, side_events[i], 0));
     if (lin_side) CUADMM_CUDA(cudaStreamWaitEvent(stream, lin_event, 0));
+    if (pdl_chain && (has_dense || has_lin || classes.size() != 1)) *pdl_chain = false;
     return launches;
 }
 
diff --git a/cuadmm_b200/csrc/solver.cu b/cuadmm_b200/csrc/solver.cu
--- a/cuadmm_b200/csrc/solver.cu
+++ b/cuadmm_b200/csrc/solver.cu
@@ -41,6 +41,7 @@
 
 __global__ void __launch_bounds__(256) scalar_update_kernel(DevState* st, const double* __restrict__ part_rd, int n_rd,
         const double* __restrict__ part_rp, int n_rp, double* hist, int64_t hist_cap) {
+    pdl_wait();
     if (st->done) return;
     __shared__ double sm[4][256];
     double v[4] = {0.0, 0.0, 0.0, 0.0};
@@ -123,6 +124,7 @@
 }
 
 __global__ void rhsy_kernel(int64_t m, const double* __restrict__ Rp, const double* __restrict__ buf, double* rhsy, const DevState* st) {
+    pdl_wait();
     if (st->done) return;
     const double sig = st->sig;
     for (int64_t i = (int64_t)blockIdx.x * blockDim.x + threadIdx.x; i < m; i += (int64_t)gridDim.x * blockDim.x) rhsy[i] = Rp[i] / sig + buf[i];
@@ -390,27 +392,32 @@
     };
     ys->prof_ev = prof ? &prof_ev : nullptr;
     ys->prof_tag = prof ? &prof_tag : nullptr;
+    bool chain_state = false;
+    bool* chain = (world == 1 && !prof) ? &chain_state : nullptr;
     const int gm_ = ew_grid(con_num, device);
     auto k1 = [&](bool cached) {
         if (!cached) {
-            if (world == 1) { e = SpmvEpilogue(); spmv_launch(*A, -1.0, SmC.p, 0.0, asmc.p, e, stream); ++launches; }
+            if (world == 1) { e = SpmvEpilogue(); spmv_launch(*A, -1.0, SmC.p, 0.0, asmc.p, e, stream, nullptr, chain); ++launches; }
             else reduce_partial_A(false, SmC.p, -1.0, nullptr, 0, nullptr);
         }
-        rhsy_kernel<<<gm_, 256, 0, stream>>>(con_num, Rp.p, asmc.p, rhsy.p, st.p); ++launches;
+        pdl_launch(rhsy_kernel, gm_, 256, 0, stream, pdl_next(chain), con_num, (const double*)Rp.p, (const double*)asmc.p,
+                   rhsy.p, (const DevState*)st.p);
+        ++launches;
     };
     k1(asmc_valid);
     mark(0);
-    ys->solve(rhsy.p, y.p, stream); launches += ys->launches_per_solve;
+    ys->solve(rhsy.p, y.p, stream, chain); launches += ys->launches_per_solve;
     mark(1);
     e = SpmvEpilogue(); e.mode = 2; e.aux1 = Cd.p; e.aux2 = X.p; e.out2 = Xb.p; e.scal = scal;
-    spmv_launch(*At, 1.0, y.p, 0.0, Rd1.p, e, stream); ++launches;
+    spmv_launch(*At, 1.0, y.p, 0.0, Rd1.p, e, stream, nullptr, chain); ++launches;
     ProjEpilogue pe;
     pe.X = X.p; pe.Rd1 = Rd1.p; pe.Cd = Cd.p; pe.S = S.p; pe.SmC = SmC.p; pe.sig_ptr = scal;
     mark(2);
-    launches += plan->project(Xb.p, Xproj.p, stream, &pe, false);
+    launches += plan->project(Xb.p, Xproj.p, stream, &pe, false, chain);
     mark(3);
     if (iter == switch_admm) {
         switch_kernel<<<1, 1, 0, stream>>>(st.p); ++launches;
+        chain_state = false;
         CUADMM_CUDA(cudaMemcpyAsync(X_best.p, X.p, sizeof(double) * nloc, cudaMemcpyDeviceToDevice, stream));
         CUADMM_CUDA(cudaMemcpyAsync(y_best.p, y.p, sizeof(double) * con_num, cudaMemcpyDeviceToDevice, stream));
         CUADMM_CUDA(cudaMemcpyAsync(S_best.p, S.p, sizeof(double) * nloc, cudaMemcpyDeviceToDevice, stream));
@@ -423,10 +430,10 @@
         k1(false);
         mark(7);
         mark(4);
-        ys->solve(rhsy.p, y.p, stream); launches += ys->launches_per_solve;
+        ys->solve(rhsy.p, y.p, stream, chain); launches += ys->launches_per_solve;
         mark(5);
         e = SpmvEpilogue(); e.mode = 3; e.aux1 = Cd.p; e.aux2 = S.p; e.out2 = X.p; e.scal = scal; e.partial = part_rd;
-        spmv_launch(*At, 1.0, y.p, 0.0, Rd.p, e, stream); ++launches;
+        spmv_launch(*At, 1.0, y.p, 0.0, Rd.p, e, stream, nullptr, chain); ++launches;
         n_rd = nAt_blocks;
     } else {
         if (iter > switch_admm) {
@@ -439,13 +446,16 @@
         }
         mark(4); mark(5);
         x_update_kernel<<<nE_blocks, kEwThreads, 0, stream>>>(nloc, Rd1.p, S.p, Cd.p, Rd.p, X.p, st.p, part_rd); ++launches;
+        chain_state = true;
         n_rd = nE_blocks;
     }
     mark(8);
     if (world == 1) {
         e = SpmvEpilogue(); e.mode = 4; e.aux1 = bd.p; e.aux2 = normA.p; e.aux3 = y.p; e.partial = part_rp;
-        spmv_launch(*A, 1.0, X.p, 0.0, Rp.p, e, stream); ++launches;
-        scalar_update_kernel<<<1, 256, 0, stream>>>(st.p, part_rd, n_rd, part_rp, nA_blocks, hist.p, hist_cap); ++launches;
+        spmv_launch(*A, 1.0, X.p, 0.0, Rp.p, e, stream, nullptr, chain); ++launches;
+        pdl_launch(scalar_update_kernel, 1, 256, 0, stream, pdl_next(chain), st.p, (const double*)part_rd, n_rd,
+                   (const double*)part_rp, nA_blocks, hist.p, hist_cap);
+        ++launches;
     } else {
         reduce_partial_A(true, X.p, 1.0, part_rd, n_rd, part_rp);
         if (use_peer)
@@ -468,6 +478,7 @@
     int64_t& nl = sgs ? graph_launches_sgs : graph_launches_admm;
     if (!exec) {
         const int64_t before = launches;
+        const int64_t pdl_before = pdl_launch_count();
         cudaGraph_t graph = nullptr;
         CUADMM_CUDA(cudaStreamBeginCapture(stream, cudaStreamCaptureModeThreadLocal));
         try {
@@ -478,7 +489,18 @@
             throw;
         }
         CUADMM_CUDA(cudaStreamEndCapture(stream, &graph));
-        CUADMM_CUDA(cudaGraphInstantiate(&exec, graph, 0));
+        if (sgs) {
+            size_t ne = 0;
+            CUADMM_CUDA(cudaGraphGetEdges_v2(graph, nullptr, nullptr, nullptr, &ne));
+            std::vector<cudaGraphNode_t> from(ne), to(ne);
+            std::vector<cudaGraphEdgeData> ed(ne);
+            if (ne) CUADMM_CUDA(cudaGraphGetEdges_v2(graph, from.data(), to.data(), ed.data(), &ne));
+            graph_edges_sgs[0] = (int64_t)ne;
+            graph_edges_sgs[1] = std::count_if(ed.begin(), ed.end(),
+                                               [](const cudaGraphEdgeData& d) { return d.type == cudaGraphDependencyTypeProgrammatic; });
+            graph_edges_sgs[2] = pdl_launch_count() - pdl_before;
+        }
+        CUADMM_CUDA(cudaGraphInstantiate(&exec, graph, cudaGraphInstantiateFlagUseNodePriority));
         CUADMM_CUDA(cudaGraphDestroy(graph));
         nl = launches - before;
         launches = before;
diff --git a/cuadmm_b200/csrc/solver.h b/cuadmm_b200/csrc/solver.h
--- a/cuadmm_b200/csrc/solver.h
+++ b/cuadmm_b200/csrc/solver.h
@@ -88,6 +88,7 @@
     void enqueue_half_step();
     cudaGraphExec_t graph_sgs = nullptr, graph_admm = nullptr;
     int64_t graph_launches_sgs = 0, graph_launches_admm = 0;
+    int64_t graph_edges_sgs[3] = {0, 0, 0};
     bool use_graphs = true;
     cuadmm::DevBuf<double> asmc;
     bool asmc_valid = false;
diff --git a/cuadmm_b200/csrc/spmv.cu b/cuadmm_b200/csrc/spmv.cu
--- a/cuadmm_b200/csrc/spmv.cu
+++ b/cuadmm_b200/csrc/spmv.cu
@@ -78,10 +78,11 @@
         const double* __restrict__ val, const double* __restrict__ x, double* y, double alpha, double beta,
         SpmvEpilogue e, const int32_t* __restrict__ long_rows, int n_long, int main_blocks, int long_thr,
         const int* __restrict__ done_flag) {
-    if (done_flag && *done_flag) return;
     __shared__ double red[2][kThreads / 32];
     double acc0 = 0.0, acc1 = 0.0;
     const int lane = threadIdx.x & 31;
+    pdl_wait();
+    if (done_flag && *done_flag) return;
     if ((int)blockIdx.x < main_blocks) {
         const int sub = threadIdx.x % G;
         const int64_t gid = ((int64_t)blockIdx.x * kThreads + threadIdx.x) / G;
@@ -193,14 +194,16 @@
 }
 
 void spmv_launch(const cuadmm_spmv_s& A_, double alpha, const double* x, double beta, double* y,
-                 const SpmvEpilogue& epi, cudaStream_t stream, int* grid_out) {
+                 const SpmvEpilogue& epi, cudaStream_t stream, int* grid_out, bool* pdl_chain) {
     const cuadmm_spmv_full& A = static_cast<const cuadmm_spmv_full&>(A_);
     const int grid = A.aux.main_blocks + A.aux.long_blocks;
     if (grid_out) *grid_out = grid;
     if (A.rows == 0 || grid == 0) return;
-#define CUADMM_SPMV_LAUNCH(G, MODE)                                                                     \
-    spmv_csr_kernel<G, MODE><<<grid, kThreads, 0, stream>>>(A.rows, A.rowptr.p, A.colind.p, A.val.p, x, y, \
-        alpha, beta, epi, A.aux.long_rows.p, A.aux.n_long, A.aux.main_blocks, A.aux.long_thr, A.done_flag)
+    const bool allow = pdl_next(pdl_chain);
+#define CUADMM_SPMV_LAUNCH(G, MODE)                                                                                    \
+    pdl_launch(spmv_csr_kernel<G, MODE>, grid, kThreads, 0, stream, allow, (int64_t)A.rows, (const int32_t*)A.rowptr.p, \
+        (const int32_t*)A.colind.p, (const double*)A.val.p, x, y, alpha, beta, epi, (const int32_t*)A.aux.long_rows.p,  \
+        A.aux.n_long, A.aux.main_blocks, A.aux.long_thr, A.done_flag)
 #define CUADMM_SPMV_CASE(G)                                                                            \
     case G:                                                                                            \
         switch (epi.mode) {                                                                            \
diff --git a/cuadmm_b200/csrc/spmv.h b/cuadmm_b200/csrc/spmv.h
--- a/cuadmm_b200/csrc/spmv.h
+++ b/cuadmm_b200/csrc/spmv.h
@@ -28,7 +28,7 @@
 };
 
 void spmv_launch(const cuadmm_spmv_s& A, double alpha, const double* x, double beta, double* y,
-                 const SpmvEpilogue& epi, cudaStream_t stream, int* grid_out = nullptr);
+                 const SpmvEpilogue& epi, cudaStream_t stream, int* grid_out = nullptr, bool* pdl_chain = nullptr);
 int spmv_grid(const cuadmm_spmv_s& A);
 cuadmm_spmv_s* spmv_create(int64_t rows, int64_t cols, int64_t nnz, const int32_t* h_rowptr,
                          const int32_t* h_colind, const double* h_val, int device);
diff --git a/cuadmm_b200/csrc/ysolve.cu b/cuadmm_b200/csrc/ysolve.cu
--- a/cuadmm_b200/csrc/ysolve.cu
+++ b/cuadmm_b200/csrc/ysolve.cu
@@ -1,3 +1,9 @@
+#ifndef CUADMM_EXP_PROJ
+#define CUADMM_EXP_PROJ 0
+#endif
+#ifndef CUADMM_EXP_PK
+#define CUADMM_EXP_PK 0
+#endif
 #include "ysolve.h"
 #include <chrono>
 #include <thread>
@@ -73,6 +79,7 @@
 #define CUADMM_TRI_FINISH(W) (W).finish(lane, dep, val, x, out_scatter, out_perm)
 
 __global__ void __launch_bounds__(kTriThreads) tri_wide_kernel(int64_t slot0, int64_t slot1, CUADMM_TRI_PARAMS) {
+    pdl_wait();
     if (done_flag && *done_flag) return;
     const int lane = threadIdx.x & 31;
     const int64_t s = slot0 + (((int64_t)blockIdx.x * kTriThreads + threadIdx.x) >> 5);
@@ -194,6 +201,7 @@
         int n_heavy, const int32_t* __restrict__ prow_src, const int64_t* __restrict__ ext_ptr,
         const int32_t* __restrict__ ext_dep, const double* __restrict__ ext_val, const double* __restrict__ rhs,
         const double* __restrict__ x, double* __restrict__ w, const int* __restrict__ done_flag) {
+    pdl_wait();
     if (done_flag && *done_flag) return;
     if ((int)blockIdx.x < main_blocks) {
         const int64_t g = (int64_t)blockIdx.x * 256 + threadIdx.x;
@@ -294,8 +302,7 @@
         const int64_t* __restrict__ row_off, const unsigned char* __restrict__ stream, const int32_t* __restrict__ prow_u,
         const int32_t* __restrict__ prow_out, const double* __restrict__ w, double* x, double* out_scatter,
         const int* __restrict__ done_flag, long long* __restrict__ timeline) {
-    if (done_flag && *done_flag) return;
-    if (timeline && threadIdx.x == 0) timeline[4 * blockIdx.x + 0] = pk_globaltimer();
+    const long long t_start = timeline ? pk_globaltimer() : 0;
     extern __shared__ __align__(128) unsigned char pk_smem[];
     unsigned char* ring = pk_smem;
     uint64_t* bars = reinterpret_cast<uint64_t*>(pk_smem + kPkRing * kPkChunk);
@@ -313,6 +320,12 @@
         asm volatile("fence.proxy.async.shared::cta;" ::: "memory");
         for (int i = 0; i < kPkRing && i < nc; ++i) pk_fetch(ring + i * kPkChunk, src + (int64_t)i * kPkChunk, bars + i);
     }
+    pdl_wait();
+    if (done_flag && *done_flag) {
+        if (tid == 0) for (int i = 0; i < kPkRing && i < nc; ++i) pk_wait(bars + i, 0u);
+        return;
+    }
+    if (timeline && tid == 0) timeline[4 * blockIdx.x + 0] = t_start;
 #pragma unroll 4
     for (int loc = tid; loc < nr; loc += kPkThreads) xs[loc] = w[r0 + loc];
     __syncthreads();
@@ -376,17 +389,20 @@
                                                         const int32_t* __restrict__ tile_col, double* out_scatter,
                                                         const int32_t* __restrict__ out_perm, int64_t perm_base,
                                                         const int* __restrict__ done_flag, int longest_last) {
-    if (done_flag && *done_flag) return;
     const int lane = threadIdx.x & 31;
     const int64_t cta = longest_last ? (int64_t)gridDim.x - 1 - blockIdx.x : blockIdx.x;
     const int64_t row = cta * (blockDim.x >> 5) + (threadIdx.x >> 5);
-    if (row >= r) return;
+    const bool live = row < r;
+    const int I = (int)(row >> 6);
+    int t0 = 0, t1 = 0;
+    if (live) { t0 = tile_ptr[I]; t1 = tile_ptr[I + 1]; }
+    pdl_wait();
+    if (!live || (done_flag && *done_flag)) return;
     const double* Ti = T + row * r;
-    const int I = (int)(row >> 6);
     double acc0 = 0.0, acc1 = 0.0;
     const bool vec = (r & 1) == 0 && (reinterpret_cast<uintptr_t>(T) & 15) == 0;
     const bool in_al = (reinterpret_cast<uintptr_t>(in) & 15) == 0;
-    for (int t = tile_ptr[I]; t < tile_ptr[I + 1]; ++t) {
+    for (int t = t0; t < t1; ++t) {
         const int64_t j0 = tile_col[2 * t];
         const int64_t j1 = min((int64_t)tile_col[2 * t + 1], r);
         if (vec) {
@@ -537,13 +553,14 @@
 }
 
 static int launch_subtrees(const TriSweep& S, const double* rhs, const int32_t* gather, double* x, double* out_scatter,
-                           const int32_t* out_perm, const int* done, cudaStream_t st, const SweepStreams& ss) {
+                           const int32_t* out_perm, const int* done, cudaStream_t st, const SweepStreams& ss, bool* pdl_chain) {
     int launches = 0;
     if (S.pk_rows > 0) {
         const int main_blocks = (int)((S.pk_rows + 255) / 256);
-        pk_gather_kernel<<<(unsigned)(main_blocks + (S.pk_n_heavy + 7) / 8), 256, 0, st>>>(S.pk_rows, main_blocks, S.pk_heavy.p,
-            (int)S.pk_n_heavy, S.pk_prow_src.p, S.pk_has_ext ? S.pk_ext_ptr.p : nullptr, S.pk_ext_dep.p, S.pk_ext_val.p, rhs, x,
-            S.pk_w.p, done);
+        pdl_launch(pk_gather_kernel, (unsigned)(main_blocks + (S.pk_n_heavy + 7) / 8), 256, 0, st, pdl_next(pdl_chain),
+            S.pk_rows, main_blocks, (const int32_t*)S.pk_heavy.p, (int)S.pk_n_heavy, (const int32_t*)S.pk_prow_src.p,
+            (const int64_t*)(S.pk_has_ext ? S.pk_ext_ptr.p : nullptr), (const int32_t*)S.pk_ext_dep.p,
+            (const double*)S.pk_ext_val.p, rhs, (const double*)x, S.pk_w.p, done);
         ++launches;
     }
     const bool fork = S.n_sub_warp > 0 && (S.n_sub_pack > 0 || S.n_sub_cta > 0);
@@ -554,8 +571,11 @@
         wst = ss.side;
     }
     if (S.n_sub_pack > 0) {
-        tri_packed_kernel<<<(unsigned)S.n_sub_pack, kPkThreads, S.pk_smem, st>>>(S.pk_chunk_off.p, S.pk_row_off.p, S.pk_stream.p,
-            S.pk_prow_u.p, S.pk_prow_out.p, S.pk_w.p, x, out_scatter, done, S.pk_timeline.n ? S.pk_timeline.p : nullptr);
+        pdl_launch_prio(tri_packed_kernel, (unsigned)S.n_sub_pack, kPkThreads, S.pk_smem, st, pdl_next(pdl_chain),
+            (CUADMM_EXP_PK && fork) ? high_priority() : 0,
+            (const int64_t*)S.pk_chunk_off.p, (const int64_t*)S.pk_row_off.p, (const unsigned char*)S.pk_stream.p,
+            (const int32_t*)S.pk_prow_u.p, (const int32_t*)S.pk_prow_out.p, (const double*)S.pk_w.p, x, out_scatter, done,
+            S.pk_timeline.n ? S.pk_timeline.p : nullptr);
         ++launches;
     }
     if (S.n_sub_warp > 0) {
@@ -566,6 +586,7 @@
         ++launches;
     }
     if (S.n_sub_cta > 0) {
+        if (pdl_chain) *pdl_chain = true;
         tri_subtree_kernel<<<(unsigned)S.n_sub_cta, kTriThreads, 0, st>>>(S.sub_off.p, S.sub_lvl_ptr.p, S.slot_rows.p, S.slot_info.p,
             S.ptr.p, S.dep.p, S.val.p, S.inv_diag.p, rhs, gather, x, out_scatter, out_perm, done);
         ++launches;
@@ -573,27 +594,30 @@
     if (fork) {
         CUADMM_CUDA(cudaEventRecord(ss.join, ss.side));
         CUADMM_CUDA(cudaStreamWaitEvent(st, ss.join, 0));
+        if (pdl_chain) *pdl_chain = false;
     }
     return launches;
 }
 
-static int launch_sweep(const TriSweep& S, const double* rhs, const int32_t* gather, double* x,
-                        double* out_scatter, const int32_t* out_perm, const int* done, cudaStream_t st, const SweepStreams& ss) {
+static int launch_sweep(const TriSweep& S, const double* rhs, const int32_t* gather, double* x, double* out_scatter,
+                        const int32_t* out_perm, const int* done, cudaStream_t st, const SweepStreams& ss, bool* pdl_chain) {
     int launches = 0;
-    if (S.subtrees_first && S.n_sub) launches += launch_subtrees(S, rhs, gather, x, out_scatter, out_perm, done, st, ss);
+    if (S.subtrees_first && S.n_sub) launches += launch_subtrees(S, rhs, gather, x, out_scatter, out_perm, done, st, ss, pdl_chain);
     for (const TriSweep::Phase& ph : S.phases) {
         if (ph.narrow) {
+            if (pdl_chain) *pdl_chain = true;
             tri_narrow_kernel<<<1, kNarrowThreads, 0, st>>>(ph.level0, ph.level1, S.level_ptr.p, S.slot_rows.p, S.slot_info.p,
                 S.ptr.p, S.dep.p, S.val.p, S.inv_diag.p, rhs, gather, x, out_scatter, out_perm, done);
         } else {
             const int64_t s0 = S.h_level_ptr[ph.level0], s1 = S.h_level_ptr[ph.level1];
             const int grid = (int)(((s1 - s0) * 32 + kTriThreads - 1) / kTriThreads);
-            tri_wide_kernel<<<grid, kTriThreads, 0, st>>>(s0, s1, S.slot_rows.p, S.slot_info.p, S.ptr.p, S.dep.p, S.val.p,
-                S.inv_diag.p, rhs, gather, x, out_scatter, out_perm, done);
+            pdl_launch(tri_wide_kernel, grid, kTriThreads, 0, st, pdl_next(pdl_chain), s0, s1, (const int32_t*)S.slot_rows.p,
+                (const int32_t*)S.slot_info.p, (const int64_t*)S.ptr.p, (const int32_t*)S.dep.p, (const double*)S.val.p,
+                (const double*)S.inv_diag.p, rhs, gather, x, out_scatter, out_perm, done);
         }
         ++launches;
     }
-    if (!S.subtrees_first && S.n_sub) launches += launch_subtrees(S, rhs, gather, x, out_scatter, out_perm, done, st, ss);
+    if (!S.subtrees_first && S.n_sub) launches += launch_subtrees(S, rhs, gather, x, out_scatter, out_perm, done, st, ss, pdl_chain);
     CUADMM_CUDA(cudaGetLastError());
     return launches;
 }
@@ -1261,13 +1285,14 @@
     CUADMM_CUDA(cudaDeviceSynchronize());
 }
 
-void cuadmm_ysolve_s::solve(const double* d_rhs_, double* d_y_, cudaStream_t st) {
+void cuadmm_ysolve_s::solve(const double* d_rhs_, double* d_y_, cudaStream_t st, bool* pdl_chain) {
     if (m == 0) return;
     double* xv = x_p ? x_p : x.p;
     double* tmpv = tail_tmp_p ? tail_tmp_p : tail_tmp.p;
-    launch_sweep(fwd, d_rhs_, perm.p, z.p, nullptr, nullptr, done_flag, st, streams);
+    launch_sweep(fwd, d_rhs_, perm.p, z.p, nullptr, nullptr, done_flag, st, streams, pdl_chain);
     auto mark = [&](int tag) {
         if (!prof_ev) return;
+        if (pdl_chain) *pdl_chain = false;
         cudaEvent_t ev;
         CUADMM_CUDA(cudaEventCreate(&ev));
         CUADMM_CUDA(cudaEventRecord(ev, st));
@@ -1285,10 +1310,12 @@
         mark(20);
         if (!peer || peer->world == 1) {
             const int blocks = (int)((n_tail + 7) / 8);
-            tail_gemv_row_kernel<<<blocks, 256, 0, st>>>(n_tail, tail_inv.p, z.p + n_lead, tmpv, tail_tptr.p, tail_tcol.p,
-                                                         nullptr, nullptr, 0, done_flag, 1);
-            tail_gemv_row_kernel<<<blocks, 256, 0, st>>>(n_tail, tail_inv_t.p, tmpv, xv + n_lead, tail_tptr_t.p, tail_tcol_t.p,
-                                                         d_y_, perm.p, n_lead, done_flag, 0);
+            pdl_launch(tail_gemv_row_kernel, blocks, 256, 0, st, pdl_next(pdl_chain), n_tail, (const double*)tail_inv.p,
+                       (const double*)(z.p + n_lead), tmpv, (const int32_t*)tail_tptr.p, (const int32_t*)tail_tcol.p,
+                       (double*)nullptr, (const int32_t*)nullptr, (int64_t)0, done_flag, 1);
+            pdl_launch(tail_gemv_row_kernel, blocks, 256, 0, st, pdl_next(pdl_chain), n_tail, (const double*)tail_inv_t.p,
+                       (const double*)tmpv, xv + n_lead, (const int32_t*)tail_tptr_t.p, (const int32_t*)tail_tcol_t.p,
+                       d_y_, (const int32_t*)perm.p, n_lead, done_flag, 0);
         } else {
             PeerPtrs pxt = peer_x;
             for (int q = 0; q < peer->world; ++q) pxt.p[q] += n_lead;
@@ -1297,11 +1324,12 @@
             gemv_split(tail_inv.p, z.p + n_lead, tmpv, tail_tptr.p, tail_tcol.p, 1, tail_row0[0], n0, peer->world, pv, peer_tmp);
             gemv_split(tail_inv_t.p, tmpv, xv + n_lead, tail_tptr_t.p, tail_tcol_t.p, 0, tail_row0[1], n1, peer->world, pv, pxt);
             tail_scatter_kernel<<<(int)((n_tail + 255) / 256), 256, 0, st>>>(n_tail, xv + n_lead, perm.p, n_lead, d_y_, done_flag);
+            if (pdl_chain) *pdl_chain = true;
         }
         CUADMM_CUDA(cudaGetLastError());
         mark(21);
     }
-    launch_sweep(bwd, z.p, nullptr, xv, d_y_, perm.p, done_flag, st, streams);
+    launch_sweep(bwd, z.p, nullptr, xv, d_y_, perm.p, done_flag, st, streams, pdl_chain);
 }
 
 extern "C" {
diff --git a/cuadmm_b200/csrc/ysolve.h b/cuadmm_b200/csrc/ysolve.h
--- a/cuadmm_b200/csrc/ysolve.h
+++ b/cuadmm_b200/csrc/ysolve.h
@@ -74,7 +74,7 @@
     ~cuadmm_ysolve_s();
     int launches_per_solve = 0;
     int64_t alg_bytes = 0;
-    void solve(const double* d_rhs, double* d_y, cudaStream_t stream);
+    void solve(const double* d_rhs, double* d_y, cudaStream_t stream, bool* pdl_chain = nullptr);
 };
 
 namespace cuadmm {
```

New measurement: 831.3, median of 6. No clear change (+0.3%).
